# aleflabo/COSKAD

Measured on AMD Instinct MI355X. Metric: pose_clips_per_sec_fwd_bwd, higher is better.
Workload: dtype f32; 1 GPU; euclidean_encoder_dynamicCenter train step (fwd+mse-to-centre+L2 reg+bwd+Adam), synthetic clips B=4096/GPU T=12 V=17 C=2, channels 2-32-16-32-64, latent 16; clips_per_gpu=4096, global_batch=4096, head=euclidean, parallelism=dp1, hip_graph=False

## Files before the change

### coskad_amd/csrc/bottleneck.hip

```cpp
#include "tile_ops.h"
#include "layer_launch.h"

namespace coskad {

constexpr int kBtlBlock = 256;
constexpr int kBtlWaves = kBtlBlock / 64;
constexpr int kBtlFwdWaves = 8;

__global__ __launch_bounds__(64 * kBtlFwdWaves) void k_btlnk_fwd(const float* __restrict__ U,
                                                     const float* __restrict__ W,
                                                     const float* __restrict__ bias,
                                                     const float* __restrict__ slope,
                                                     float* __restrict__ z, int B, int K, int L) {
  __shared__ float red[kBtlFwdWaves][256];
  const int lane = threadIdx.x & 63, wave = threadIdx.x >> 6;
  const int i = lane & 15, kk = lane >> 4;
  const int n = blockIdx.x * 16 + i;
  const bool pre = slope != nullptr;
  const float a = pre ? slope[0] : 0.f;
  const bool rowok = n < B, colok = i < L;
  const float* up = U + (size_t)(rowok ? n : 0) * K;
  const float* wp = W + (size_t)(colok ? i : 0) * K;
  const int nsteps = ceil_div(K, 16);
  const int per = ceil_div(nsteps, kBtlFwdWaves);
  const int s0 = wave * per, s1 = min(nsteps, s0 + per);
  f32x4 acc = {0.f, 0.f, 0.f, 0.f};
  constexpr int UB = 4;
  for (int sb = s0; sb < s1; sb += UB) {
    float4 x[UB], w[UB];
#pragma unroll
    for (int u = 0; u < UB; ++u) {
      const int k = (sb + u) * 16 + 4 * kk;
      const bool ok = sb + u < s1 && k < K;
      x[u] = (ok && rowok) ? *reinterpret_cast<const float4*>(up + k) : float4{0.f, 0.f, 0.f, 0.f};
      w[u] = (ok && colok) ? *reinterpret_cast<const float4*>(wp + k) : float4{0.f, 0.f, 0.f, 0.f};
    }
#pragma unroll
    for (int u = 0; u < UB; ++u) {
      float4 xv = x[u];
      if (pre) { xv.x = prelu_f(xv.x, a); xv.y = prelu_f(xv.y, a); xv.z = prelu_f(xv.z, a); xv.w = prelu_f(xv.w, a); }
      acc = __builtin_amdgcn_mfma_f32_16x16x4f32(xv.x, w[u].x, acc, 0, 0, 0);
      acc = __builtin_amdgcn_mfma_f32_16x16x4f32(xv.y, w[u].y, acc, 0, 0, 0);
      acc = __builtin_amdgcn_mfma_f32_16x16x4f32(xv.z, w[u].z, acc, 0, 0, 0);
      acc = __builtin_amdgcn_mfma_f32_16x16x4f32(xv.w, w[u].w, acc, 0, 0, 0);
    }
  }
#pragma unroll
  for (int r = 0; r < 4; ++r) red[wave][(4 * (lane >> 4) + r) * 16 + (lane & 15)] = acc[r];
  __syncthreads();
  const int e = threadIdx.x, row = (e >> 4) & 15, col = e & 15;
  const int nn = blockIdx.x * 16 + row;
  if (e < 256 && nn < B && col < L) {
    float s = 0.f;
#pragma unroll
// ... 124 lines not shown
#pragma unroll
    for (int g = 0; g < 4; ++g) {
      const int nn = n0 + c, j = 4 * g + q;
      const float av = (nn < nend && j < L) ? dz[(size_t)nn * L + j] : 0.f;
      dx[0] = __builtin_amdgcn_mfma_f32_16x16x4f32(av, wf[g].x, dx[0], 0, 0, 0);
      dx[1] = __builtin_amdgcn_mfma_f32_16x16x4f32(av, wf[g].y, dx[1], 0, 0, 0);
      dx[2] = __builtin_amdgcn_mfma_f32_16x16x4f32(av, wf[g].z, dx[2], 0, 0, 0);
      dx[3] = __builtin_amdgcn_mfma_f32_16x16x4f32(av, wf[g].w, dx[3], 0, 0, 0);
    }
#pragma unroll
    for (int s = 0; s < 4; ++s) {
      const int nn = n0 + 4 * q + s;
      const bool ok = kok && nn < nend;
      const float4 u = ucur[s];
      float4 x = u;
      if (pre) { x.x = prelu_f(u.x, a); x.y = prelu_f(u.y, a); x.z = prelu_f(u.z, a); x.w = prelu_f(u.w, a); }
      const float dzv = (nn < nend && c < L) ? dz[(size_t)nn * L + c] : 0.f;
      dw[0] = __builtin_amdgcn_mfma_f32_16x16x4f32(dzv, x.x, dw[0], 0, 0, 0);
      dw[1] = __builtin_amdgcn_mfma_f32_16x16x4f32(dzv, x.y, dw[1], 0, 0, 0);
      dw[2] = __builtin_amdgcn_mfma_f32_16x16x4f32(dzv, x.z, dw[2], 0, 0, 0);
      dw[3] = __builtin_amdgcn_mfma_f32_16x16x4f32(dzv, x.w, dw[3], 0, 0, 0);
      float4 g = {dx[0][s], dx[1][s], dx[2][s], dx[3][s]};
      if (pre) {
        da += (u.x < 0.f ? g.x * u.x : 0.f) + (u.y < 0.f ? g.y * u.y : 0.f) +
              (u.z < 0.f ? g.z * u.z : 0.f) + (u.w < 0.f ? g.w * u.w : 0.f);
        g.x = u.x > 0.f ? g.x : a * g.x; g.y = u.y > 0.f ? g.y : a * g.y;
        g.z = u.z > 0.f ? g.z : a * g.z; g.w = u.w > 0.f ? g.w : a * g.w;
      }
      if (ok) *reinterpret_cast<float4*>(dU + (size_t)nn * K + kc) = g;
    }
#pragma unroll
    for (int s = 0; s < 4; ++s) ucur[s] = unext[s];
  }
  if (kok) {
    float* dst = dWp + (size_t)blockIdx.y * L * K;
#pragma unroll
    for (int r = 0; r < 4; ++r) {
      const int j = 4 * q + r;
      if (j < L) *reinterpret_cast<float4*>(dst + (size_t)j * K + kc) = float4{dw[0][r], dw[1][r], dw[2][r], dw[3][r]};
    }
  }
  da = wave_sum(da);
  if (lane == 0) sred[wave] = da;
  __syncthreads();
  if (threadIdx.x == 0) dap[blockIdx.y * gridDim.x + blockIdx.x] = (sred[0] + sred[1]) + (sred[2] + sred[3]);
}

__global__ __launch_bounds__(256) void k_btlnk_reduce(const float* __restrict__ partials, int P, size_t E,
                                                       float* __restrict__ out, const float* __restrict__ dz,
                                                       int B, int L, float* __restrict__ db,
                                                       const float* __restrict__ dap, int nda,
                                                       float* __restrict__ dslope, int accumulate,
                                                       const float* __restrict__ rows, int RP, int RE,
                                                       double* __restrict__ rsum) {
  __shared__ double sh[256];
  const unsigned nE = (unsigned)((E + 255) / 256);
  if (blockIdx.x > nE + L) {
    const int col = threadIdx.x & 15, slice = threadIdx.x >> 4;
    const int e = (int)(blockIdx.x - (nE + L + 1)) * 16 + col;
    double s = 0.0;
    if (e < RE) {
      const float* base = rows + e;
      int p = slice;
      for (; p + 7 * 16 < RP; p += 8 * 16) {
        float v[8];
#pragma unroll
        for (int u = 0; u < 8; ++u) v[u] = base[(size_t)(p + 16 * u) * RE];
#pragma unroll
        for (int u = 0; u < 8; ++u) s += (double)v[u];
      }
      for (; p < RP; p += 16) s += (double)base[(size_t)p * RE];
    }
    sh[threadIdx.x] = s;
    __syncthreads();
    if (slice == 0 && e < RE) {
      double t = 0.0;
#pragma unroll
      for (int k = 0; k < 16; ++k) t += sh[col + 16 * k];
      rsum[e] = t;
    }
    return;
  }
  if (blockIdx.x < nE) {
    const size_t e = (size_t)blockIdx.x * 256 + threadIdx.x;
    if (e >= E) return;
    double s = 0.0;
    int p = 0;
    for (; p + 8 <= P; p += 8) {
      float v[8];
#pragma unroll
      for (int u = 0; u < 8; ++u) v[u] = partials[(size_t)(p + u) * E + e];
#pragma unroll
      for (int u = 0; u < 8; ++u) s += (double)v[u];
    }
    for (; p < P; ++p) s += (double)partials[(size_t)p * E + e];
    out[e] = accumulate ? out[e] + (float)s : (float)s;
    return;
  }
  const int r = (int)(blockIdx.x - nE);
  double s = 0.0;
  if (r < L) {
    if (!db) return;
    for (int n = threadIdx.x; n < B; n += 256) s += (double)dz[(size_t)n * L + r];
  } else {
    if (!dslope) return;
    for (int i = threadIdx.x; i < nda; i += 256) s += (double)dap[i];
  }
  sh[threadIdx.x] = s;
  __syncthreads();
  for (int w = 128; w > 0; w >>= 1) {
    if ((int)threadIdx.x < w) sh[threadIdx.x] += sh[threadIdx.x + w];
    __syncthreads();
  }
  if (threadIdx.x == 0) {
    float* o = r < L ? db + r : dslope;
    o[0] = accumulate ? o[0] + (float)sh[0] : (float)sh[0];
  }
}

static int btl_chunks(int B, int K) {
  const int gx = ceil_div(K, 256);
  int s = (1024 + gx / 2) / gx;
  const int smax = ceil_div(B, 16);
  if (s > smax) s = smax;
  if (s > 64) s = 64;
  return s < 1 ? 1 : s;
}

int launch_btlnk_reduce(const float* partials, int P, size_t E, float* out, const float* dz, int B, int L, float* db,
                        const float* dap, int nda, float* dslope, int accumulate, hipStream_t stream, const float* rows,
                        int RP, int RE, double* rsum) {
  const unsigned extra = rows ? (unsigned)ceil_div(RE, 16) : 0u;
  hipLaunchKernelGGL(k_btlnk_reduce, dim3((unsigned)((E + 255) / 256) + L + 1 + extra), dim3(256), 0, stream, partials, P, E, out, dz,
                     B, L, db, dap, nda, dslope, accumulate, rows, RP, RE, rsum);
  return check_launch("btlnk_bwd_reduce");
}

constexpr int kBtlWideMax = 512;

}

using namespace coskad;

extern "C" {

int coskad_btlnk_fwd_f32(const float* U, const float* W, const float* bias, const float* slope, float* z,
                         int B, int K, int L, hipStream_t stream) {
  if (!U || !W || !z) return fail(COSKAD_ERR_ARG, "btlnk_fwd: null pointer");
  if (B <= 0 || K <= 0 || L <= 0) return fail(COSKAD_ERR_ARG, "btlnk_fwd: B=%d K=%d L=%d", B, K, L);
  if (L > 16) return fail(COSKAD_ERR_SHAPE, "btlnk_fwd: latent_dim=%d > 16 needs the workspace entry point coskad_btlnk_fwd_ws_f32", L);
  if (K % 4) return fail(COSKAD_ERR_SHAPE, "btlnk_fwd: K=%d must be a multiple of 4", K);
  hipLaunchKernelGGL(k_btlnk_fwd, dim3(ceil_div(B, 16)), dim3(64 * kBtlFwdWaves), 0, stream, U, W, bias, slope, z, B, K, L);
  return check_launch("btlnk_fwd");
}

size_t coskad_btlnk_fwd_ws_bytes(int B) { return (size_t)kBtlKS * (size_t)(B > 0 ? B : 0) * 16 * sizeof(float); }

size_t coskad_btlnk_fwd_ws_bytes_l(int B, int K, int L) {
  if (L > 16 && L <= kBtlWideMax) return wide_btlnk_fwd_ws_bytes(B, K, L);
  return coskad_btlnk_fwd_ws_bytes(B);
}

int coskad_btlnk_fwd_ws_f32(const float* U, const float* W, const float* bias, const float* slope, float* z, void* ws,
                            size_t ws_bytes, int B, int K, int L, hipStream_t stream) {
  if (!U || !W || !z || !ws) return fail(COSKAD_ERR_ARG, "btlnk_fwd_ws: null pointer");
  if (B <= 0 || K <= 0 || L <= 0) return fail(COSKAD_ERR_ARG, "btlnk_fwd_ws: B=%d K=%d L=%d", B, K, L);
  if (L > kBtlWideMax) return fail(COSKAD_ERR_SHAPE, "btlnk_fwd_ws: latent_dim=%d > %d not supported", L, kBtlWideMax);
  if (L > 16) {
    if (ws_bytes < wide_btlnk_fwd_ws_bytes(B, K, L)) return fail(COSKAD_ERR_WORKSPACE, "btlnk_fwd_ws: workspace too small");
    return wide_btlnk_fwd(U, W, bias, slope, z, ws, B, K, L, stream);
  }
  if (K % 16) return fail(COSKAD_ERR_SHAPE, "btlnk_fwd_ws: K=%d must be a multiple of 16", K);
  if (ws_bytes < coskad_btlnk_fwd_ws_bytes(B)) return fail(COSKAD_ERR_WORKSPACE, "btlnk_fwd_ws: workspace too small");
  float* part = reinterpret_cast<float*>(ws);
  hipLaunchKernelGGL(k_btlnk_fwd_t, dim3(ceil_div(B, 64), kBtlKS), dim3(256), 0, stream, U, W, slope, part, B, K, L);
  int rc;
  if ((rc = check_launch("btlnk_fwd_t"))) return rc;
  hipLaunchKernelGGL(k_btlnk_fwd_sum, dim3(ceil_div(B * 16, 256)), dim3(256), 0, stream, part, bias, z, B, L, kBtlKS);
  return check_launch("btlnk_fwd_sum");
}

size_t coskad_btlnk_bwd_ws_bytes(int B, int K, int L) {
  if (L > 16 && L <= kBtlWideMax) return wide_btlnk_bwd_ws_bytes(B, K, L);
  const int S = btl_chunks(B, K);
  return ((size_t)S * L * K + (size_t)S * ceil_div(K, 256) + 64) * sizeof(float);
}

int coskad_btlnk_bwd_f32(const float* U, const float* W, const float* dz, const float* slope, float* dU,
                         float* dW, float* db, float* dslope, void* ws, size_t ws_bytes, int accumulate,
                         int B, int K, int L, hipStream_t stream) {
  if (!U || !W || !dz || !dU || !dW || !ws) return fail(COSKAD_ERR_ARG, "btlnk_bwd: null pointer");
  if (B <= 0 || K <= 0 || L <= 0) return fail(COSKAD_ERR_ARG, "btlnk_bwd: B=%d K=%d L=%d", B, K, L);
  if (L > kBtlWideMax) return fail(COSKAD_ERR_SHAPE, "btlnk_bwd: latent_dim=%d > %d not supported", L, kBtlWideMax);
  if (ws_bytes < coskad_btlnk_bwd_ws_bytes(B, K, L)) return fail(COSKAD_ERR_WORKSPACE, "btlnk_bwd: workspace too small");
  if (L > 16) return wide_btlnk_bwd(U, W, dz, slope, dU, dW, db, dslope, ws, accumulate, B, K, L, stream);
  if (K % 4) return fail(COSKAD_ERR_SHAPE, "btlnk_bwd: K=%d must be a multiple of 4", K);
  const int S = btl_chunks(B, K);
  const int chunk = round_up(ceil_div(B, S), 16);
  const int gx = ceil_div(K, 256);
  float* dWp = reinterpret_cast<float*>(ws);
  float* dap = dWp + (size_t)S * L * K;
  {
    ProbeScope probe(KID_BTLNK_BWD, 0, L, stream);
    hipLaunchKernelGGL(k_btlnk_bwd, dim3(gx, S), dim3(kBtlBlock), 0, stream, U, W, dz, slope, dU, dWp, dap, B, K, L, chunk);
  }
  int rc = check_launch("btlnk_bwd");
  if (rc) return rc;
  return launch_btlnk_reduce(dWp, S, (size_t)L * K, dW, dz, B, L, db, dap, gx * S, (dslope && slope) ? dslope : nullptr, accumulate, stream,
                             nullptr, 0, 0, nullptr);
}

}
```

### coskad_amd/csrc/btlnk_chain.hip

```cpp
#include "fused_ops.h"
#include "layer_launch.h"

namespace coskad {
namespace bc {

using ff::f32x4; using ff::mfma; using ff::BufRes; using ff::make_res; using ff::buf_load4; using ff::buf_load1;
__device__ __forceinline__ void buf_store1(BufRes r, int voff, int soff, float v) {
  __builtin_amdgcn_raw_buffer_store_b32(__float_as_uint(v), r, voff, soff, 0);
}

constexpr int HID = 64;
constexpr int PT = 16;
constexpr int NCL = 16;
constexpr int RSTR = 17;
constexpr int kThreads = 512;
#ifndef BC_XCD
#define BC_XCD 1
#endif
#ifndef BC_PF
#define BC_PF 1
#endif
#ifndef BC_SKIP
#define BC_SKIP 0
#endif

template <int CT>
__global__ __launch_bounds__(kThreads, 1) void k_btlnk_bwd_stats(
    const float* __restrict__ U, const float* __restrict__ W, const float* __restrict__ dz, const float* __restrict__ slope,
    float* __restrict__ dU, float* __restrict__ dWp, float* __restrict__ dap, const float* __restrict__ xin,
    const float* __restrict__ Zg, const float* __restrict__ in_slope, float* __restrict__ prow, int B, int TV, int L, int chunk) {
  constexpr int Ci = 16 * CT, NR = 2 * Ci;
  constexpr int GCS = HID * RSTR + 4, ZCS = NR * RSTR + 4;
  constexpr int NL = NR * NCL * (PT / 4) / kThreads;
  constexpr int E = 2 * HID * Ci + HID;
  extern __shared__ __attribute__((aligned(16))) float lds[];
  float* G = lds;
  float* ZX = lds + NCL * GCS;
  const int tid = threadIdx.x, lane = tid & 63;
  const int wave = __builtin_amdgcn_readfirstlane(tid >> 6);
  const int wc = wave & 3, h = wave >> 2;
  const int c = lane & 15, q = lane >> 4;
  const int K = HID * TV;
  const int nwg = gridDim.x, npt = (TV + PT - 1) / PT;
  int wg = blockIdx.x;
  if (BC_XCD) {
    const int xq = nwg / 8, xr = nwg % 8, xcd = wg % 8;
    wg = (xcd < xr ? xcd * (xq + 1) : xr * (xq + 1) + (xcd - xr) * xq) + wg / 8;
  }
  const int ychunk = wg / npt;
  const int p0 = (wg - ychunk * npt) * PT;
  const int nbeg = ychunk * chunk, nend = min(B, nbeg + chunk);
  const bool pre = slope != nullptr;
  const float a = pre ? slope[0] : 0.f;
  const bool xact = in_slope != nullptr;
  const float a_in = xact ? in_slope[0] : 0.f;
  const int ch0 = 16 * wc + 8 * h;
  const bool pok = p0 + c < TV;
  constexpr int MASK = 0x7ffffff0;

  float wf[8][4];
#pragma unroll
  for (int i = 0; i < 8; ++i)
#pragma unroll
    for (int g = 0; g < 4; ++g) {
      const int j = 4 * g + q;
      wf[i][g] = (j < L && pok) ? W[(size_t)j * K + (ch0 + i) * TV + p0 + c] : 0.f;
    }

  f32x4 dw[8], pacc[CT], qacc[CT];
#pragma unroll
  for (int i = 0; i < 8; ++i) dw[i] = f32x4{0.f, 0.f, 0.f, 0.f};
#pragma unroll
  for (int t = 0; t < CT; ++t) pacc[t] = qacc[t] = f32x4{0.f, 0.f, 0.f, 0.f};
  float ssum = 0.f, da = 0.f;

  auto tile_res = [&](const float* base, int n0, int rowfloats) {
    const int left = nend - n0;
    return make_res(base + (size_t)(left > 0 ? n0 : 0) * rowfloats, left > 0 ? (unsigned)left * (unsigned)rowfloats * 4u : 0u);
  };
  const int zx_p4 = lane & 3, zx_row = lane >> 2;
  const int zx_voff = (p0 + 4 * zx_p4 < TV) ? (zx_row * TV + p0 + 4 * zx_p4) * 4 : MASK;
  auto zx_load = [&](int n0, float4 (&v)[NL]) {
    const BufRes rz = tile_res(Zg, n0, Ci * TV), rx = tile_res(xin, n0, Ci * TV);
#pragma unroll
    for (int i = 0; i < NL; ++i) {
      const int cl = wave + 8 * (i & 1), rb = i >> 1;
      v[i] = (BC_SKIP & 4) ? float4{0.f, 0.f, 0.f, 0.f} : buf_load4(rb < CT ? rz : rx, zx_voff, (cl * Ci + 16 * (rb % CT)) * TV * 4);
    }
  };
  auto zx_store = [&](const float4 (&v)[NL]) {
    if (BC_SKIP & 8) return;
#pragma unroll
    for (int i = 0; i < NL; ++i) {
      const int cl = wave + 8 * (i & 1), rb = i >> 1;
      float4 x = v[i];
      if (xact && rb >= CT) { x.x = prelu_f(x.x, a_in); x.y = prelu_f(x.y, a_in); x.z = prelu_f(x.z, a_in); x.w = prelu_f(x.w, a_in); }
      float* d = ZX + cl * ZCS + (16 * rb + zx_row) * RSTR + 4 * zx_p4;
      d[0] = x.x; d[1] = x.y; d[2] = x.z; d[3] = x.w;
    }
  };
  const int u_voff = pok ? (4 * q * K + p0 + c) * 4 : MASK;
  auto u_load = [&](int n0, float (&u)[8][4]) {
    const BufRes ru = tile_res(U, n0, K);
#pragma unroll
    for (int i = 0; i < 8; ++i)
#pragma unroll
      for (int r = 0; r < 4; ++r) u[i][r] = (BC_SKIP & 1) ? ((i + r) & 1 ? 1.f : -1.f) : buf_load1(ru, u_voff, (r * K + (ch0 + i) * TV) * 4);
  };
  const int dza_voff = (c * L + q) * 4, dzb_voff = (4 * q * L + c) * 4;
  auto dz_load = [&](int n0, float (&da_)[4], float (&db_)[4]) {
    const BufRes rd = tile_res(dz, n0, L);
#pragma unroll
    for (int g = 0; g < 4; ++g) {
      const float v = buf_load1(rd, dza_voff, 16 * g);
      da_[g] = 4 * g + q < L ? v : 0.f;
    }
#pragma unroll
    for (int r = 0; r < 4; ++r) {
      const float v = buf_load1(rd, dzb_voff, r * L * 4);
      db_[r] = c < L ? v : 0.f;
    }
  };

  float4 zx[NL];
  float ucur[8][4], dza[4], dzb[4];
  u_load(nbeg, ucur);
  dz_load(nbeg, dza, dzb);
  zx_load(nbeg, zx);

  float* gw = G + 4 * q * GCS + ch0 * RSTR + c;
  const float* ga = G + 4 * q * GCS + (16 * wc + c) * RSTR + 8 * h;
  const float* zb = ZX + 4 * q * ZCS + c * RSTR + 8 * h;

  for (int n0 = nbeg; n0 < nend; n0 += NCL) {
    float unext[8][4];
    if (BC_PF == 2) { zx_store(zx); zx_load(n0 + NCL, zx); }
    if (BC_PF) u_load(n0 + NCL, unext);
    {
      const BufRes rdu = tile_res(dU, n0, K);
      f32x4 dx[8];
#pragma unroll
      for (int i = 0; i < 8; ++i) dx[i] = f32x4{0.f, 0.f, 0.f, 0.f};
#pragma unroll
      for (int g = 0; g < 4; ++g)
#pragma unroll
        for (int i = 0; i < 8; ++i) dx[i] = mfma(dza[g], wf[i][g], dx[i]);
#pragma unroll
      for (int r = 0; r < 4; ++r)
#pragma unroll
        for (int i = 0; i < 8; ++i) {
          const float u = ucur[i][r];
          float g = dx[i][r], x = u;
          if (pre) {
            da += u < 0.f ? g * u : 0.f;
            g = u > 0.f ? g : a * g;
            x = prelu_f(u, a);
          }
          if (!(BC_SKIP & 32)) dw[i] = mfma(dzb[r], x, dw[i]);
          if (!(BC_SKIP & 64)) gw[r * GCS + i * RSTR] = g;
          if (!(BC_SKIP & 2) || g == 123.456f) buf_store1(rdu, u_voff, (r * K + (ch0 + i) * TV) * 4, g);
        }
    }
    if (BC_PF != 2) zx_store(zx);
    lds_barrier();
    if (BC_PF) {
#pragma unroll
      for (int i = 0; i < 8; ++i)
#pragma unroll
        for (int r = 0; r < 4; ++r) ucur[i][r] = unext[i][r];
    } else {
      u_load(n0 + NCL, ucur);
    }
    dz_load(n0 + NCL, dza, dzb);
    if (BC_PF != 2) zx_load(n0 + NCL, zx);
#pragma unroll
    for (int pl = 0; pl < 8; ++pl)
#pragma unroll
      for (int r = 0; r < 4; ++r) {
        const float av = (BC_SKIP & 64) ? 1.f : ga[r * GCS + pl];
        ssum += av;
        if (BC_SKIP & 16) continue;
#pragma unroll
        for (int t = 0; t < CT; ++t) {
          pacc[t] = mfma(av, zb[r * ZCS + (16 * t) * RSTR + pl], pacc[t]);
          qacc[t] = mfma(av, zb[r * ZCS + (Ci + 16 * t) * RSTR + pl], qacc[t]);
        }
      }
    lds_barrier();
  }

  {
    float* dst = dWp + (size_t)ychunk * L * K + p0 + c;
#pragma unroll
    for (int i = 0; i < 8; ++i)
#pragma unroll
      for (int r = 0; r < 4; ++r) {
        const int j = 4 * q + r;
        if (j < L && pok) dst[(size_t)j * K + (ch0 + i) * TV] = dw[i][r];
      }
  }
  float* row = lds;
  float* red = lds + E;
  const float s4 = ssum + __shfl_xor(ssum, 16, 64);
  const float sch = s4 + __shfl_xor(s4, 32, 64);
  da = wave_sum(da);
  for (int hh = 0; hh < 2; ++hh) {
    if (h == hh) {
#pragma unroll
      for (int t = 0; t < CT; ++t)
#pragma unroll
        for (int r = 0; r < 4; ++r) {
          const int o = 16 * wc + 4 * q + r, cc = 16 * t + c;
          float* p = row + o * Ci + cc;
          p[0] = (hh ? p[0] : 0.f) + pacc[t][r];
          p[HID * Ci] = (hh ? p[HID * Ci] : 0.f) + qacc[t][r];
        }
      if (q == 0) {
        float* p = row + 2 * HID * Ci + 16 * wc + c;
        p[0] = (hh ? p[0] : 0.f) + sch;
      }
      if (lane == 0) red[wave] = da;
    }
    __syncthreads();
  }
  float* dstrow = prow + (size_t)wg * E;
  for (int e = tid; e < E; e += kThreads) dstrow[e] = row[e];
  if (tid == 0) dap[wg] = ((red[0] + red[1]) + (red[2] + red[3])) + ((red[4] + red[5]) + (red[6] + red[7]));
}

struct Plan {
  int npt, S, chunk;
};
static Plan plan(int B, int TV) {
  Plan p;
  p.npt = ceil_div(TV, PT);
  int s = 256 / p.npt;
  const int smax = ceil_div(B, NCL);
  if (s > smax) s = smax;
  if (s < 1) s = 1;
  p.chunk = round_up(ceil_div(B, s), NCL);
  p.S = ceil_div(B, p.chunk);
  return p;
}
static inline size_t sums_offset(int rows, int E) { return ((size_t)rows * E + 1) / 2 * 2; }

}

}

using namespace coskad;

extern "C" {

int coskad_btlnk_bwd_chain_ok(int K, int TV, int below_Ci) {
  return TV > 0 && TV % 4 == 0 && K == bc::HID * TV && (below_Ci == 16 || below_Ci == 32);
}

int coskad_btlnk_bwd_chain_rows(int B, int TV) {
  if (B <= 0 || TV <= 0) return 0;
  const bc::Plan p = bc::plan(B, TV);
  return p.npt * p.S;
}

size_t coskad_btlnk_bwd_chain_floats(int B, int TV, int below_Ci) {
  const size_t E = 2 * (size_t)bc::HID * below_Ci + bc::HID;
  return bc::sums_offset(coskad_btlnk_bwd_chain_rows(B, TV), (int)E) + 2 * E;
}

size_t coskad_btlnk_bwd_chain_ws_bytes(int B, int K, int L, int TV) {
  if (B <= 0 || TV <= 0) return 0;
  const bc::Plan p = bc::plan(B, TV);
  return ((size_t)p.S * L * K + (size_t)p.S * p.npt + 64) * sizeof(float);
}

int coskad_btlnk_bwd_chain_f32(const float* U, const float* W, const float* dz, const float* slope, float* dU, float* dW,
                               float* db, float* dslope, void* ws, size_t ws_bytes, int accumulate, int B, int K, int L,
                               const float* below_in, const float* below_Z, const float* below_in_slope, int below_Ci, int TV,
                               float* stats_out, size_t stats_out_bytes, int* stats_rows, hipStream_t stream) {
  if (!U || !W || !dz || !dU || !dW || !ws || !below_in || !below_Z || !stats_out || !stats_rows)
    return fail(COSKAD_ERR_ARG, "btlnk_bwd_chain: null pointer");
  if (B <= 0 || K <= 0 || L <= 0) return fail(COSKAD_ERR_ARG, "btlnk_bwd_chain: B=%d K=%d L=%d", B, K, L);
  if (L > 16) return fail(COSKAD_ERR_SHAPE, "btlnk_bwd_chain: latent_dim=%d > 16 not supported", L);
  if (!coskad_btlnk_bwd_chain_ok(K, TV, below_Ci))
    return fail(COSKAD_ERR_SHAPE, "btlnk_bwd_chain: K=%d TV=%d below_Ci=%d (needs K = 64 TV, TV %% 4 == 0, 16 / 32 channels below)", K, TV, below_Ci);
  if ((size_t)stats_out & 7) return fail(COSKAD_ERR_ARG, "btlnk_bwd_chain: stats_out must be 8-byte aligned");
  if (ws_bytes < coskad_btlnk_bwd_chain_ws_bytes(B, K, L, TV)) return fail(COSKAD_ERR_WORKSPACE, "btlnk_bwd_chain: workspace too small");
  if (stats_out_bytes < coskad_btlnk_bwd_chain_floats(B, TV, below_Ci) * sizeof(float))
    return fail(COSKAD_ERR_WORKSPACE, "btlnk_bwd_chain: stats_out %zu bytes too small", stats_out_bytes);
  const bc::Plan p = bc::plan(B, TV);
  const int rows = p.npt * p.S;
  const int E = 2 * bc::HID * below_Ci + bc::HID;
  float* dWp = reinterpret_cast<float*>(ws);
  float* dap = dWp + (size_t)p.S * L * K;
  const size_t lds = (size_t)bc::NCL * ((bc::HID * bc::RSTR + 4) + (2 * below_Ci * bc::RSTR + 4)) * sizeof(float);
  int rc;
  {
  ProbeScope probe(KID_BTLNK_BWD, below_Ci, L, stream);
  if (below_Ci == 32) {
    auto k = bc::k_btlnk_bwd_stats<2>;
    (void)hipFuncSetAttribute((const void*)k, hipFuncAttributeMaxDynamicSharedMemorySize, (int)lds);
    hipLaunchKernelGGL(k, dim3(p.npt * p.S), dim3(bc::kThreads), lds, stream, U, W, dz, slope, dU, dWp, dap, below_in, below_Z,
                       below_in_slope, stats_out, B, TV, L, p.chunk);
  } else {
    auto k = bc::k_btlnk_bwd_stats<1>;
    (void)hipFuncSetAttribute((const void*)k, hipFuncAttributeMaxDynamicSharedMemorySize, (int)lds);
    hipLaunchKernelGGL(k, dim3(p.npt * p.S), dim3(bc::kThreads), lds, stream, U, W, dz, slope, dU, dWp, dap, below_in, below_Z,
                       below_in_slope, stats_out, B, TV, L, p.chunk);
  }
  }
  if ((rc = check_launch("btlnk_bwd_stats"))) return rc;
  *stats_rows = rows;
  return launch_btlnk_reduce(dWp, p.S, (size_t)L * K, dW, dz, B, L, db, dap, rows, (dslope && slope) ? dslope : nullptr, accumulate, stream,
                             stats_out, rows, E, reinterpret_cast<double*>(stats_out + bc::sums_offset(rows, E)));
}

}
```

### coskad_amd/csrc/first_layer.hip

```cpp
#include "mfma_ops.h"
#include "layer_launch.h"

namespace coskad {
namespace fl {

__device__ __forceinline__ float act(float x, bool pre, float a) { return (pre && x < 0.f) ? a * x : x; }
__device__ __forceinline__ float4 act4(float4 v, bool pre, float a) {
  return float4{act(v.x, pre, a), act(v.y, pre, a), act(v.z, pre, a), act(v.w, pre, a)};
}
__device__ __forceinline__ float dot4(const float4& a, const float4& b) { return (a.x * b.x + a.y * b.y) + (a.z * b.z + a.w * b.w); }

constexpr int NW = 4;
template <int CI, int RW>
__global__ __launch_bounds__(64 * NW, 4) void k_first_stats(const float* __restrict__ in, const float* __restrict__ Zg,
                                                           const float* __restrict__ dU, const float* __restrict__ in_slope,
                                                           float* __restrict__ partials, int B, int Co, int TVr, int need_q) {
  const int lane = threadIdx.x & 63;
  const int wave = uniform(threadIdx.x >> 6);
  const bool pre = in_slope != nullptr;
  const float a_in = pre ? in_slope[0] : 0.f;
  const int n4 = TVr >> 2;
  float pP[RW][CI], pQ[RW][CI], pS[RW];
#pragma unroll
  for (int k = 0; k < RW; ++k) {
    pS[k] = 0.f;
#pragma unroll
    for (int c = 0; c < CI; ++c) { pP[k][c] = 0.f; pQ[k][c] = 0.f; }
  }
  for (int clip = blockIdx.x; clip < B; clip += gridDim.x) {
    const float* gz = Zg + (size_t)clip * CI * TVr;
    const float* gx = in + (size_t)clip * CI * TVr;
    const float* gd = dU + ((size_t)clip * Co + (size_t)wave * RW) * TVr;
    for (int l = lane; l < n4; l += 64) {
      float4 z[CI], x[CI];
#pragma unroll
      for (int c = 0; c < CI; ++c) {
        z[c] = *reinterpret_cast<const float4*>(gz + c * TVr + 4 * l);
        x[c] = need_q ? act4(*reinterpret_cast<const float4*>(gx + c * TVr + 4 * l), pre, a_in) : float4{0.f, 0.f, 0.f, 0.f};
      }
      float4 d[RW];
#pragma unroll
      for (int k = 0; k < RW; ++k)
        d[k] = (wave * RW + k < Co) ? *reinterpret_cast<const float4*>(gd + (size_t)k * TVr + 4 * l) : float4{0.f, 0.f, 0.f, 0.f};
#pragma unroll
      for (int k = 0; k < RW; ++k) {
        pS[k] += (d[k].x + d[k].y) + (d[k].z + d[k].w);
#pragma unroll
        for (int c = 0; c < CI; ++c) {
          pP[k][c] += dot4(d[k], z[c]);
          pQ[k][c] += dot4(d[k], x[c]);
        }
      }
    }
  }
// ... 90 lines not shown
      }
#pragma unroll
      for (int c = 0; c < CI; ++c) *reinterpret_cast<float4*>(part + (wave * CI + c) * TV + 4 * l) = dz[c];
    }
    __syncthreads();
    for (int e = tid; e < CI * TV; e += NTH) {
      const int c = e / TV, p = e - c * TV;
      float v = kt[c];
#pragma unroll
      for (int c2 = 0; c2 < CI; ++c2) v = fmaf(Kt[c2 * CiP + c], Zg[((size_t)clip * CI + c2) * TV + p], v);
#pragma unroll
      for (int w = 0; w < NW; ++w) v += part[(w * CI + c) * TV + p];
      dZl[e] = v;
      Xl[e] = act(in[(size_t)clip * CI * TV + e], pre, a_in);
    }
    __syncthreads();
    for (int e = tid; e < CI * TV; e += NTH) {
      const int c = e / TV, p = e - c * TV, q = p / V, v = p - q * V;
      float y = 0.f, dy = 0.f;
#pragma unroll
      for (int t = 0; t < T; ++t) y = fmaf(Xl[c * TV + t * V + v], TwL[(t * T + q) * V + v], y);
#pragma unroll
      for (int w = 0; w < V; ++w) dy = fmaf(AwL[q * V * V + v * V + w], dZl[c * TV + q * V + w], dy);
      Yl[e] = y;
      dYl[e] = dy;
    }
    __syncthreads();
#pragma unroll
    for (int k = 0; k < KA; ++k) {
      float s = 0.f;
#pragma unroll
      for (int c = 0; c < CI; ++c) s = fmaf(Yl[c * TV + ya[k]], dZl[c * TV + za[k]], s);
      accA[k] += s;
    }
#pragma unroll
    for (int k = 0; k < KT; ++k) {
      float s = 0.f;
#pragma unroll
      for (int c = 0; c < CI; ++c) s = fmaf(Xl[c * TV + xt[k]], dYl[c * TV + yt[k]], s);
      accT[k] += s;
    }
  }
  float* dst = partials + (size_t)blockIdx.x * (NA + NT);
#pragma unroll
  for (int k = 0; k < KA; ++k)
    if (tid + NTH * k < NA) dst[tid + NTH * k] = accA[k];
#pragma unroll
  for (int k = 0; k < KT; ++k)
    if (tid + NTH * k < NT) dst[NA + tid + NTH * k] = accT[k];
}


constexpr int NWM = 8;
template <int T, int V, int CI>
__global__ __launch_bounds__(64 * NWM, 4) void k_first_moments(const float* __restrict__ in, const float* __restrict__ Aw,
                                                          const float* __restrict__ Tw, const float* __restrict__ in_slope,
                                                          float* __restrict__ partials, int B, float* __restrict__ Zout) {
  constexpr int TV = T * V, NA = T * V * V, NT = V * T * T, KP = (TV + 63) / 64;
  extern __shared__ __attribute__((aligned(16))) float lds[];
  float* AwL = lds;
  float* TwL = AwL + NA;
  const int tid = threadIdx.x, lane = tid & 63;
  const int wave = uniform(tid >> 6);
  float* Xl = TwL + NT + wave * 2 * CI * TV;
  float* Yl = Xl + CI * TV;
  const bool pre = in_slope != nullptr;
  const float a_in = pre ? in_slope[0] : 0.f;
  for (int e = tid; e < NA; e += 64 * NWM) AwL[e] = Aw[e];
  for (int e = tid; e < NT; e += 64 * NWM) {
    const int v = e / (T * T), tq = e - v * T * T;
    TwL[tq * V + v] = Tw[e];
  }
  float mx[CI][CI], mz[CI][CI], sx[CI], sz[CI];
#pragma unroll
  for (int a = 0; a < CI; ++a) {
    sx[a] = 0.f; sz[a] = 0.f;
#pragma unroll
    for (int b = 0; b < CI; ++b) { mx[a][b] = 0.f; mz[a][b] = 0.f; }
  }
  __syncthreads();
  const int rounds = (B + gridDim.x * NWM - 1) / (gridDim.x * NWM);
  for (int r = 0; r < rounds; ++r) {
    const int clip = (r * gridDim.x + blockIdx.x) * NWM + wave;
    const bool live = clip < B;
    const float* gx = in + (size_t)(live ? clip : 0) * CI * TV;
#pragma unroll
    for (int k = 0; k < KP; ++k) {
      const int p = lane + 64 * k;
      if (p < TV) {
        float x[CI];
#pragma unroll
        for (int c = 0; c < CI; ++c) {
          x[c] = live ? act(gx[c * TV + p], pre, a_in) : 0.f;
          Xl[c * TV + p] = x[c];
          sx[c] += x[c];
        }
#pragma unroll
        for (int a = 0; a < CI; ++a)
#pragma unroll
          for (int b = 0; b < CI; ++b) mx[a][b] = fmaf(x[a], x[b], mx[a][b]);
      }
    }
    __syncthreads();
#pragma unroll
    for (int k = 0; k < KP; ++k) {
      const int p = lane + 64 * k;
      if (p < TV) {
        const int q = p / V, v = p - q * V;
#pragma unroll
        for (int c = 0; c < CI; ++c) {
          float y = 0.f;
#pragma unroll
          for (int t = 0; t < T; ++t) y = fmaf(Xl[c * TV + t * V + v], TwL[(t * T + q) * V + v], y);
          Yl[c * TV + p] = y;
        }
      }
    }
    __syncthreads();
    float* gz = Zout + (size_t)(live ? clip : 0) * CI * TV;
#pragma unroll
    for (int k = 0; k < KP; ++k) {
      const int p = lane + 64 * k;
      if (p < TV) {
        const int t = p / V, w = p - t * V;
        float z[CI];
#pragma unroll
        for (int c = 0; c < CI; ++c) {
          float acc = 0.f;
#pragma unroll
          for (int v = 0; v < V; ++v) acc = fmaf(Yl[c * TV + t * V + v], AwL[t * V * V + v * V + w], acc);
          z[c] = acc;
          if (live) gz[c * TV + p] = acc;
          sz[c] += acc;
        }
#pragma unroll
        for (int a = 0; a < CI; ++a)
// ... 81 lines not shown
    else if (Ci == 2) LAUNCH_FS_C(2);
    else if (Ci == 3) LAUNCH_FS_C(3);
    else LAUNCH_FS_C(4);
  }
#undef LAUNCH_FS_C
#undef LAUNCH_FS
  return check_launch("first_stats");
}

template <int T, int V>
static int launch_first_bwd_tv(const float* in, const float* Zg, const float* dU, const float* Aw, const float* Tw, const float* coef,
                               const float* in_slope, float* partials, int B, int Ci, int Co, int max_rows, hipStream_t st,
                               int* rows_out) {
  constexpr int NWB = fl::first_bwd_waves<T, V>();
  int grid = B < 512 ? B : 512;
  if (grid > max_rows) grid = max_rows;
  *rows_out = grid;
  const int rw = ceil_div(Co, NWB);
  const size_t lds = ((size_t)T * V * V + (size_t)V * T * T + (4 + NWB) * (size_t)Ci * T * V) * sizeof(float);
#define LAUNCH_FB1(CI, RW)                                                                                              \
  do {                                                                                                                  \
    auto k = fl::k_first_bwd<T, V, CI, RW>;                                                                             \
    if (lds > 64 * 1024) (void)hipFuncSetAttribute((const void*)k, hipFuncAttributeMaxDynamicSharedMemorySize, (int)lds); \
    hipLaunchKernelGGL(k, dim3(grid), dim3(64 * NWB), lds, st, in, Zg, dU, Aw, Tw, coef, in_slope, partials, B, Co);             \
  } while (0)
#define LAUNCH_FB1_C(CI)                        \
  do {                                          \
    if (rw <= 4) LAUNCH_FB1(CI, 4);             \
    else if (rw <= 8) LAUNCH_FB1(CI, 8);        \
    else LAUNCH_FB1(CI, 16);                    \
  } while (0)
  {
    ProbeScope probe(KID_BWD_DATA, Ci, Co, st);
    if (Ci == 1) LAUNCH_FB1_C(1);
    else if (Ci == 2) LAUNCH_FB1_C(2);
    else if (Ci == 3) LAUNCH_FB1_C(3);
    else LAUNCH_FB1_C(4);
  }
#undef LAUNCH_FB1_C
#undef LAUNCH_FB1
  return check_launch("first_bwd");
}

int launch_first_bwd(const float* in, const float* Zg, const float* dU, const float* Aw, const float* Tw, const float* coef,
                     const float* in_slope, float* partials, int B, int Ci, int Co, int T, int V, int max_rows, hipStream_t st,
                     int* rows_out) {
#define CALL(T_, V_) return launch_first_bwd_tv<T_, V_>(in, Zg, dU, Aw, Tw, coef, in_slope, partials, B, Ci, Co, max_rows, st, rows_out)
  COSKAD_DISPATCH_TV(T, V, CALL);
#undef CALL
}

template <int T, int V>
static int launch_first_moments_tv(const float* in, const float* Aw, const float* Tw, const float* in_slope, float* partials, int B,
                                   int Ci, float* Zout, int max_rows, hipStream_t st, int* rows_out) {
  int grid = (B + fl::NWM - 1) / fl::NWM;
  if (grid > 512) grid = 512;
  if (grid > max_rows) grid = max_rows;
  *rows_out = grid;
  const size_t lds = ((size_t)T * V * V + (size_t)V * T * T + 2 * fl::NWM * (size_t)Ci * T * V) * sizeof(float);
#define LAUNCH_FM(CI)                                                                                                   \
  do {                                                                                                                  \
    auto k = fl::k_first_moments<T, V, CI>;                                                                             \
    if (lds > 64 * 1024) (void)hipFuncSetAttribute((const void*)k, hipFuncAttributeMaxDynamicSharedMemorySize, (int)lds); \
    hipLaunchKernelGGL(k, dim3(grid), dim3(64 * fl::NWM), lds, st, in, Aw, Tw, in_slope, partials, B, Zout);                    \
  } while (0)
  {
    ProbeScope probe(KID_FWD_MOMENTS, Ci, 0, st);
    if (Ci == 1) LAUNCH_FM(1);
    else if (Ci == 2) LAUNCH_FM(2);
    else if (Ci == 3) LAUNCH_FM(3);
    else LAUNCH_FM(4);
  }
#undef LAUNCH_FM
  return check_launch("first_moments");
}

int launch_first_moments(const float* in, const float* Aw, const float* Tw, const float* in_slope, float* partials, int B, int Ci,
                         int T, int V, float* Zout, int max_rows, hipStream_t st, int* rows_out) {
#define CALL(T_, V_) return launch_first_moments_tv<T_, V_>(in, Aw, Tw, in_slope, partials, B, Ci, Zout, max_rows, st, rows_out)
  COSKAD_DISPATCH_TV(T, V, CALL);
#undef CALL
}

int launch_first_apply(const float* Z, const float* in, float* out, const float* wfold, const float* bias, const float* in_slope,
                       int B, int Ci, int Co, int TVr, hipStream_t st) {
  const int grid = B < 2048 ? B : 2048;
  const size_t lds = 2 * (size_t)Ci * TVr * sizeof(float);
  const int CoP = round_up(Co, 16);
#define LAUNCH_FAP(CI) hipLaunchKernelGGL((fl::k_first_apply<CI>), dim3(grid), dim3(256), lds, st, Z, in, out, wfold, bias, in_slope, B, Co, CoP, TVr)
  {
    ProbeScope probe(KID_LAYER_APPLY, Ci, Co, st);
    if (Ci == 1) LAUNCH_FAP(1);
    else if (Ci == 2) LAUNCH_FAP(2);
    else if (Ci == 3) LAUNCH_FAP(3);
    else LAUNCH_FAP(4);
  }
#undef LAUNCH_FAP
  return check_launch("first_apply");
}

}
```

### coskad_amd/csrc/fused_apply_next.hip

```cpp
#include "fused_ops.h"
#include "layer_launch.h"

#ifndef FN_ABLATE
#define FN_ABLATE 0
#endif

namespace coskad {
namespace fn {

using namespace ff;

struct FtabArgs {
  const float* A[4];
  const float* Tm[4];
  float* tab[4];
};
__global__ void k_build_ftab(FtabArgs args) {
  const int layer = blockIdx.y;
  const float* __restrict__ Aw = args.A[layer];
  const float* __restrict__ Tw = args.Tm[layer];
  const int e = blockIdx.x * blockDim.x + threadIdx.x;
  if (e >= LAYER_F4 * 4) return;
  float val = 0.f;
  if (e < TEMP_F4 * 4) {
    const int v = e / 256, l = (e >> 2) & 63, s = e & 3, j = l & 15, q = l >> 4;
    if (s < 3 && j < T) val = Tw[v * T * T + (4 * s + q) * T + j];
  } else {
    const int r = e - TEMP_F4 * 4;
    const int t = r / (3 * 256), c = (r / 256) % 3, l = (r >> 2) & 63, k = 4 * c + (r & 3), j = l & 15, q = l >> 4;
    if (k < 10) {
      const int s = k < 5 ? k : k - 5, w = 4 * s + q;
      if (w < V) val = Aw[t * V * V + w * V + (k < 5 ? j : 16)];
    }
  }
  args.tab[layer][e] = val;
}

template <int CT, int OTP>
__global__ __launch_bounds__(256, 1) void k_layer_apply_next(const float* __restrict__ in, const float* __restrict__ Zg,
                                                            const float* __restrict__ wfold, const float* __restrict__ bias,
                                                            const float* __restrict__ in_slope, const float* __restrict__ out_slope,
                                                            const float* __restrict__ ftab, float* __restrict__ out,
                                                            float* __restrict__ Znext, float* __restrict__ partials, int B) {
  constexpr int Ci = CT ? 16 * CT : 2, Co = 16 * OTP, CoP = Co, NG = 2 * CT;
  constexpr int NACC = OTP == 1 ? 2 : 3;
  constexpr int E = 2 * (Co * Co + Co);
  static_assert(OTP == 1 || OTP == 2, "the 32-row image holds the whole output");
  extern __shared__ __attribute__((aligned(16))) float lds_all[];
  const int lane = threadIdx.x & 63;
  const int wave = __builtin_amdgcn_readfirstlane(threadIdx.x >> 6);
  float* lds = lds_all + wave * WAVE_LDS_W;
  float* r1 = lds + R1;
  float* r2 = lds + R2;
  auto geo = [&]() {
    int l = lane;
    asm volatile("" : "+v"(l));
    return Lane{l & 15, l >> 4};
  };
  auto olane = [&]() {
    int l = lane;
    asm volatile("" : "+v"(l));
    return l;
  };
  const bool pre = in_slope != nullptr;
  const float a_in = pre ? in_slope[0] : 0.f;
  const float a_out = out_slope[0];
  const int l16 = lane * 16;
  const BufRes wres = make_res(wfold, 2 * Ci * CoP * 4u);
  const BufRes bres = make_res(bias, CoP * 4u);
  const BufRes tabres = make_res(ftab, LAYER_F4 * 16u);
  const int nwaves = gridDim.x * 4;
  auto clip_res = [&](const float* base, int c, int rows) {
    const bool in_range = c < B;
#ifdef COSKAD_HOT
    return make_res(base + (size_t)(in_range ? (c & 63) : 0) * rows * TV, in_range ? rows * TV * 4u : 0u);
#else
    return make_res(base + (size_t)(in_range ? c : 0) * rows * TV, in_range ? rows * TV * 4u : 0u);
#endif
  };
  constexpr int QTAIL = 4 * (TV / 4) - 192;
  const int l16t = lane < QTAIL ? l16 : 0x7ffffff0;
  float4 gb[16];
  auto qload = [&](const BufRes& res, int row0, int q) {
#pragma unroll
    for (int c = 0; c < 4; ++c) gb[4 * q + c] = buf_load4(res, c < 3 ? l16 : l16t, ((row0 + 4 * q) * (TV / 4) + 64 * c) * 16);
  };
  auto qstore = [&](int q, bool act) {
    const int ln = olane();
// ... 202 lines not shown
  }

  float* row = lds_all;
  __syncthreads();
  const Lane L = geo();
  auto put = [&](int w, float* base, const f32x4 (&g)[NACC], const float (&s)[OTP]) {
#pragma unroll
    for (int r = 0; r < 4; ++r) {
      const int i = 4 * L.q + r, j = L.j;
      if constexpr (OTP == 1) {
        float* p = base + i * Co + j;
        p[0] = (w ? p[0] : 0.f) + (g[0][r] + g[1][r]);
      } else {
        float* p00 = base + i * Co + j;
        float* p01 = base + i * Co + 16 + j;
        float* p10 = base + (16 + j) * Co + i;
        float* p11 = base + (16 + i) * Co + 16 + j;
        p00[0] = (w ? p00[0] : 0.f) + g[0][r];
        p01[0] = (w ? p01[0] : 0.f) + g[1][r];
        p10[0] = (w ? p10[0] : 0.f) + g[1][r];
        p11[0] = (w ? p11[0] : 0.f) + g[2][r];
      }
    }
#pragma unroll
    for (int rt = 0; rt < OTP; ++rt) {
      const float t = quad_sum(s[rt]);
      if (L.q == 0) {
        float* p = base + Co * Co + 16 * rt + L.j;
        p[0] = (w ? p[0] : 0.f) + t;
      }
    }
  };
  for (int w = 0; w < 4; ++w) {
    if (wave == w) {
      put(w, row, gx, sx);
      put(w, row + Co * Co + Co, gz, sz);
    }
    __syncthreads();
  }
  float* dst = partials + (size_t)blockIdx.x * E;
  for (int e = threadIdx.x; e < E; e += 256) dst[e] = row[e];
}

}

bool layer_apply_next_ok(int T_, int V_, int Ci, int Co) {
  return T_ == ff::T && V_ == ff::V && (Ci == 2 || Ci == 16 || Ci == 32) && (Co == 16 || Co == 32);
}

int ftab_floats() { return ff::LAYER_F4 * 4; }

int launch_build_ftab(const float* const* A, const float* const* Tm, float* const* tab, int n, hipStream_t st) {
  if (n < 1 || n > 4) return fail(COSKAD_ERR_ARG, "build_ftab: 1..4 layers per launch, got %d", n);
  fn::FtabArgs args{};
  for (int i = 0; i < n; ++i) {
    if (!A[i] || !Tm[i] || !tab[i]) return fail(COSKAD_ERR_ARG, "build_ftab: null pointer (layer %d)", i);
    args.A[i] = A[i]; args.Tm[i] = Tm[i]; args.tab[i] = tab[i];
  }
  hipLaunchKernelGGL(fn::k_build_ftab, dim3(ceil_div(ff::LAYER_F4 * 4, 256), n), dim3(256), 0, st, args);
  return check_launch("build_ftab");
}

static bool apply_next_bpc_on(int Ci, int Co) { return (Ci == 2 && Co == 32) || (Ci == 32 && Co == 16) || (Ci == 16 && Co == 32); }
int layer_apply_next_rows(int B, int Ci, int Co) {
  if (apply_next_bpc_on(Ci, Co)) return apply_next_bpc_rows(B);
  const int nblk = (B + 3) / 4;
  return nblk < 256 ? nblk : 256;
}

int launch_layer_apply_next(const float* Z, const float* in, float* out, const float* wfold, const float* bias,
                            const float* in_slope, const float* out_slope, const float* ftab, float* Znext, float* partials,
                            int B, int Ci, int Co, hipStream_t st, int* rows_out) {
  const size_t lds = (size_t)4 * ff::WAVE_LDS_W * sizeof(float);
  const int grid = layer_apply_next_rows(B, Ci, Co);
  *rows_out = grid;
  if (apply_next_bpc_on(Ci, Co))
    return launch_layer_apply_next_bpc(Z, in, out, wfold, bias, in_slope, out_slope, ftab, Znext, partials, B, Ci, Co, st);
#define LAUNCH_FN(CT, OTP)                                                                                            \
  do {                                                                                                                \
    auto k = fn::k_layer_apply_next<CT, OTP>;                                                                         \
    (void)hipFuncSetAttribute((const void*)k, hipFuncAttributeMaxDynamicSharedMemorySize, (int)lds);                  \
    hipLaunchKernelGGL(k, dim3(grid), dim3(256), lds, st, in, Z, wfold, bias, in_slope, out_slope, ftab, out, Znext,  \
                       partials, B);                                                                                  \
  } while (0)
  {
    ProbeScope probe(KID_LAYER_APPLY, Ci, Co, st);
    if (Ci == 2 && Co == 16) LAUNCH_FN(0, 1);
    else if (Ci == 2 && Co == 32) LAUNCH_FN(0, 2);
    else if (Ci == 16 && Co == 16) LAUNCH_FN(1, 1);
    else if (Ci == 16 && Co == 32) LAUNCH_FN(1, 2);
    else if (Ci == 32 && Co == 16) LAUNCH_FN(2, 1);
    else if (Ci == 32 && Co == 32) LAUNCH_FN(2, 2);
    else return fail(COSKAD_ERR_SHAPE, "apply_next: unsupported channels (%d, %d)", Ci, Co);
  }
#undef LAUNCH_FN
  return check_launch("layer_apply_next");
}

}

using namespace coskad;
extern "C" {

int coskad_layer_apply_next_ok(int Ci, int Co, int T, int V) { return layer_apply_next_ok(T, V, Ci, Co) ? 1 : 0; }
int coskad_ftab_floats(void) { return ftab_floats(); }
int coskad_layer_apply_next_rows(int B, int Ci, int Co) { return layer_apply_next_rows(B, Ci, Co); }

// ... 24 lines not shown
```

### coskad_amd/csrc/heads.hip

```cpp
#include "tile_ops.h"
#include "heads_common.h"

namespace coskad {

struct Vec {
  float v[LMAX];
};

__device__ __forceinline__ Vec load_vec(const float* p, int L) {
  Vec r;
#pragma unroll
  for (int j = 0; j < LMAX; ++j) r.v[j] = j < L ? p[j] : 0.f;
  return r;
}
__device__ __forceinline__ void store_vec(float* p, const Vec& a, int L) {
#pragma unroll
  for (int j = 0; j < LMAX; ++j)
    if (j < L) p[j] = a.v[j];
}
__device__ __forceinline__ float dot(const Vec& a, const Vec& b) {
  float s = 0.f;
#pragma unroll
  for (int j = 0; j < LMAX; ++j) s = fmaf(a.v[j], b.v[j], s);
  return s;
}

struct Embed {
  Vec p;
  float un_raw, un, tn, en_raw;
  bool clamped;
};
__device__ __forceinline__ Embed hyp_embed(const Vec& u) {
  Embed r;
  r.un_raw = sqrtf(dot(u, u));
  r.un = fmaxf(r.un_raw, kMinNorm);
  r.tn = tanhf(fminf(fmaxf(r.un, -kTanhClamp), kTanhClamp));
  const float f = r.tn / r.un;
  Vec e;
#pragma unroll
  for (int j = 0; j < LMAX; ++j) e.v[j] = f * u.v[j];
  r.en_raw = sqrtf(dot(e, e));
  const float en = fmaxf(r.en_raw, kMinNorm);
  const float maxnorm = 1.f - kBallEps;
  r.clamped = en > maxnorm;
  const float s = r.clamped ? maxnorm / en : 1.f;
#pragma unroll
  for (int j = 0; j < LMAX; ++j) r.p.v[j] = r.clamped ? e.v[j] / en * maxnorm : e.v[j];
  (void)s;
  return r;
}

__device__ __forceinline__ float poincare_dist(const Vec& c, const Vec& p, Vec* gp) {
  const float x2 = dot(c, c), y2 = dot(p, p), xy = -dot(c, p);
  const float alpha = 1.f + 2.f * xy + y2, beta = 1.f - x2;
  const float den = 1.f + 2.f * xy + x2 * y2;
  const float D = den + kMobiusEps;
  Vec m;
#pragma unroll
  for (int j = 0; j < LMAX; ++j) m.v[j] = (alpha * (-c.v[j]) + beta * p.v[j]) / D;
  const float mn = sqrtf(dot(m, m));
  const float mc = fminf(fmaxf(mn, -1.f + kArtanhEps), 1.f - kArtanhEps);
  const float d = (log1pf(mc) - log1pf(-mc));
  if (gp) {
    const float gmn = 2.f / (1.f - mc * mc);
    const float inv = mn > 0.f ? gmn / mn : 0.f;
    Vec gm;
#pragma unroll
    for (int j = 0; j < LMAX; ++j) gm.v[j] = inv * m.v[j];
    const float gD = -dot(gm, m) / D;
    float galpha = 0.f;
#pragma unroll
    for (int j = 0; j < LMAX; ++j) galpha = fmaf(gm.v[j] / D, -c.v[j], galpha);
#pragma unroll
    for (int j = 0; j < LMAX; ++j) {
      const float x = -c.v[j], y = p.v[j];
      gp->v[j] = beta * gm.v[j] / D + galpha * (2.f * x + 2.f * y) + gD * (2.f * x + 2.f * x2 * y);
    }
  }
  return d;
}

__device__ __forceinline__ Vec hyp_embed_bwd(const Vec& u, const Embed& em, const Vec& gp) {
  const float f = em.tn / em.un;
  Vec ge;
  if (em.clamped) {
    const float maxnorm = 1.f - kBallEps;
    const float en = em.en_raw;
    float egp = 0.f;
#pragma unroll
    for (int j = 0; j < LMAX; ++j) egp = fmaf(f * u.v[j], gp.v[j], egp);
#pragma unroll
    for (int j = 0; j < LMAX; ++j) ge.v[j] = maxnorm * (gp.v[j] / en - f * u.v[j] * egp / (en * en * en));
  } else {
    ge = gp;
  }
  Vec gu;
  float gf = dot(ge, u);
  float coef = 0.f;
  if (em.un_raw > kMinNorm) {
    const float sech2 = em.un < kTanhClamp ? 1.f - em.tn * em.tn : 0.f;
    const float df = (sech2 * em.un - em.tn) / (em.un * em.un);
    coef = gf * df / em.un_raw;
  }
#pragma unroll
  for (int j = 0; j < LMAX; ++j) gu.v[j] = f * ge.v[j] + coef * u.v[j];
  return gu;
}

constexpr int kHeadSlots = LMAX + 3;

constexpr int kHeadSingleRows = kFlatBlock;
__host__ __device__ inline int head_blocks(int B) { return B <= kHeadSingleRows ? 1 : ceil_div(B, kFlatBlock); }

__device__ __forceinline__ void block_partials(const float (&vals)[kHeadSlots], float* partials, float scale0, float* stats,
                                               float* acc) {
  __shared__ float sh[kFlatBlock / 64][kHeadSlots];
  const int lane = threadIdx.x & 63, wave = threadIdx.x >> 6;
#pragma unroll
  for (int k = 0; k < kHeadSlots; ++k) {
    const float s = wave_sum(vals[k]);
    if (lane == 0) sh[wave][k] = s;
  }
  __syncthreads();
  if (threadIdx.x < kHeadSlots) {
    float s = 0.f;
    for (int w = 0; w < kFlatBlock / 64; ++w) s += sh[w][threadIdx.x];
    if (gridDim.x == 1) {
      if (stats) stats[threadIdx.x] = threadIdx.x == 0 ? s * scale0 : s;
      if (acc) acc[threadIdx.x] += s;
    } else {
      partials[blockIdx.x * kHeadSlots + threadIdx.x] = s;
    }
  }
}

__global__ __launch_bounds__(kFlatBlock) void k_mse_head(const float* __restrict__ z,
                                                    const float* __restrict__ cvec,
                                                    float* __restrict__ dz, float* __restrict__ score,
                                                    float* __restrict__ partials, int B, int L,
                                                    float gscale, float scale0, float* __restrict__ stats,
                                                    float* __restrict__ acc) {
  float vals[kHeadSlots];
#pragma unroll
  for (int k = 0; k < kHeadSlots; ++k) vals[k] = 0.f;
  const Vec c = load_vec(cvec, L);
#pragma unroll 4
  for (int n = blockIdx.x * kFlatBlock + threadIdx.x; n < B; n += gridDim.x * kFlatBlock) {
    const Vec u = load_vec(z + (size_t)n * L, L);
    Vec g;
    float sq = 0.f;
#pragma unroll
    for (int j = 0; j < LMAX; ++j) {
      const float d = j < L ? u.v[j] - c.v[j] : 0.f;
      sq = fmaf(d, d, sq);
      g.v[j] = 2.f * d * gscale;
      vals[1 + j] += u.v[j];
    }
    vals[0] += sq;
    vals[LMAX + 1] += 1.f;
    vals[LMAX + 2] += sqrtf(dot(u, u));
    if (dz) store_vec(dz + (size_t)n * L, g, L);
    if (score) score[n] = sq / (float)L;
  }
  block_partials(vals, partials, scale0, stats, acc);
}

__global__ __launch_bounds__(kFlatBlock) void k_mahalanobis_head(const float* __restrict__ z,
                                                            const float* __restrict__ cvec,
                                                            const float* __restrict__ VI,
                                                            float* __restrict__ dz, float* __restrict__ score,
                                                            float* __restrict__ partials, int B, int L,
                                                            float gscale, float scale0, float* __restrict__ stats,
                                                            float* __restrict__ acc) {
  __shared__ float vi[LMAX * LMAX];
  for (int e = threadIdx.x; e < LMAX * LMAX; e += kFlatBlock) {
    const int r = e / LMAX, q = e - r * LMAX;
    vi[e] = (r < L && q < L) ? VI[r * L + q] : 0.f;
  }
  __syncthreads();
  float vals[kHeadSlots];
#pragma unroll
  for (int k = 0; k < kHeadSlots; ++k) vals[k] = 0.f;
  const Vec c = load_vec(cvec, L);
  for (int n = blockIdx.x * kFlatBlock + threadIdx.x; n < B; n += gridDim.x * kFlatBlock) {
    const Vec u = load_vec(z + (size_t)n * L, L);
    Vec d, w, wt;
#pragma unroll
    for (int j = 0; j < LMAX; ++j) { d.v[j] = j < L ? u.v[j] - c.v[j] : 0.f; w.v[j] = 0.f; wt.v[j] = 0.f; }
#pragma unroll
    for (int r = 0; r < LMAX; ++r)
#pragma unroll
      for (int q = 0; q < LMAX; ++q) {
        const float a = vi[r * LMAX + q];
        w.v[r] = fmaf(a, d.v[q], w.v[r]);
        wt.v[q] = fmaf(a, d.v[r], wt.v[q]);
      }
    const float dist = sqrtf(dot(d, w));
    vals[0] += dist;
#pragma unroll
    for (int j = 0; j < LMAX; ++j) vals[1 + j] += u.v[j];
    vals[LMAX + 1] += 1.f;
    vals[LMAX + 2] += sqrtf(dot(u, u));
    if (score) score[n] = dist;
    if (dz) {
      Vec g;
      const float inv = gscale / (2.f * dist);
#pragma unroll
      for (int j = 0; j < LMAX; ++j) g.v[j] = (w.v[j] + wt.v[j]) * inv;
      store_vec(dz + (size_t)n * L, g, L);
    }
  }
  block_partials(vals, partials, scale0, stats, acc);
}

__global__ __launch_bounds__(LMAX * LMAX) void k_gram(const float* __restrict__ z, float* __restrict__ gram, int B,
                                                     int L, int accumulate) {
  constexpr int CH = 256;
  __shared__ float zs[CH * LMAX];
  const int i = threadIdx.x / LMAX, j = threadIdx.x % LMAX;
  float s = 0.f;
  for (int n0 = 0; n0 < B; n0 += CH) {
    const int nc = min(CH, B - n0);
    __syncthreads();
    for (int e = threadIdx.x; e < nc * L; e += LMAX * LMAX) {
      const int r = e / L, q = e - r * L;
      zs[r * LMAX + q] = z[(size_t)(n0 + r) * L + q];
    }
    __syncthreads();
    if (i < L && j < L)
      for (int r = 0; r < nc; ++r) s = fmaf(zs[r * LMAX + i], zs[r * LMAX + j], s);
  }
  if (i < L && j < L) gram[i * L + j] = accumulate ? gram[i * L + j] + s : s;
}

__global__ __launch_bounds__(kFlatBlock) void k_poincare_head(const float* __restrict__ z,
                                                         const float* __restrict__ cvec,
                                                         float* __restrict__ dz, float* __restrict__ zh,
                                                         float* __restrict__ score,
                                                         float* __restrict__ partials, int B, int L,
                                                         float gscale, float scale0, float* __restrict__ stats,
                                                         float* __restrict__ acc) {
  float vals[kHeadSlots];
#pragma unroll
  for (int k = 0; k < kHeadSlots; ++k) vals[k] = 0.f;
  for (int n = blockIdx.x * kFlatBlock + threadIdx.x; n < B; n += gridDim.x * kFlatBlock) {
    const Vec u = load_vec(z + (size_t)n * L, L);
    const Embed em = hyp_embed(u);
    if (zh) store_vec(zh + (size_t)n * L, em.p, L);
    const float y2 = dot(em.p, em.p);
    const float gamma = 2.f / (1.f - y2);
#pragma unroll
    for (int j = 0; j < LMAX; ++j) vals[1 + j] += gamma * em.p.v[j];
    vals[LMAX + 1] += gamma - 1.f;
    vals[LMAX + 2] += sqrtf(y2);
    if (cvec) {
      const Vec c = load_vec(cvec, L);
      Vec gp;
      const float d = poincare_dist(c, em.p, dz ? &gp : nullptr);
      vals[0] += d;
      if (score) score[n] = d;
      if (dz) {
#pragma unroll
        for (int j = 0; j < LMAX; ++j) gp.v[j] *= gscale;
        store_vec(dz + (size_t)n * L, hyp_embed_bwd(u, em, gp), L);
      }
    }
  }
  block_partials(vals, partials, scale0, stats, acc);
}

__global__ __launch_bounds__(64) void k_head_finalize(const float* __restrict__ partials, int P,
                                                       float scale0, float* __restrict__ stats,
                                                       float* __restrict__ acc) {
  const int k = threadIdx.x;
  if (k >= kHeadSlots) return;
  double s = 0.0;
  for (int p = 0; p < P; ++p) s += (double)partials[p * kHeadSlots + k];
  if (stats) stats[k] = (float)(k == 0 ? s * (double)scale0 : s);
  if (acc) acc[k] += (float)s;
}

__global__ __launch_bounds__(kFlatBlock) void k_poincare_dist(const float* __restrict__ zh,
                                                         const float* __restrict__ cvec,
                                                         float* __restrict__ score, int B, int L) {
  const int n = blockIdx.x * kFlatBlock + threadIdx.x;
  if (n >= B) return;
  const Vec p = load_vec(zh + (size_t)n * L, L), c = load_vec(cvec, L);
  score[n] = poincare_dist(c, p, nullptr);
}

__global__ __launch_bounds__(kFlatBlock) void k_poincare_logmap0(const float* __restrict__ y, float* __restrict__ out, int B, int L) {
  const int n = blockIdx.x * kFlatBlock + threadIdx.x;
  if (n >= B) return;
  const Vec p = load_vec(y + (size_t)n * L, L);
  const float yn = fmaxf(sqrtf(dot(p, p)), kMinNorm);
  const float yc = fminf(fmaxf(yn, -1.f + kArtanhEps), 1.f - kArtanhEps);
  const float at = 0.5f * (log1pf(yc) - log1pf(-yc));
  Vec o;
#pragma unroll
  for (int j = 0; j < LMAX; ++j) o.v[j] = p.v[j] / yn * at;
  store_vec(out + (size_t)n * L, o, L);
}

__global__ void k_midpoint_finalize(const float* __restrict__ acc, float* __restrict__ cvec, int L) {
  if (threadIdx.x != 0 || blockIdx.x != 0) return;
  const double s = fmax((double)acc[LMAX + 1], 1e-10);
  double m[LMAX], mn2 = 0.0;
  for (int j = 0; j < L; ++j) { m[j] = (double)acc[1 + j] / s; mn2 += m[j] * m[j]; }
  const double mn = fmax(sqrt(mn2), 1e-15);
  const double mc = fmin(mn, 1.0 - 1e-7);
  const double at = 0.5 * log((1.0 + mc) / (1.0 - mc));
  const double sc = tanh(0.5 * at) / mn;
  for (int j = 0; j < L; ++j) cvec[j] = (float)(sc * m[j]);
}

__global__ void k_center_finalize(const float* __restrict__ acc, float eps, float* __restrict__ cvec,
                                  int L) {
  const int j = threadIdx.x;
  if (j >= L || blockIdx.x != 0) return;
  float c = acc[1 + j] / acc[LMAX + 1];
  if (fabsf(c) < eps && c < 0.f) c = -eps;
  if (fabsf(c) < eps && c > 0.f) c = eps;
  cvec[j] = c;
}

__global__ __launch_bounds__(256) void k_sqnorm_masked(const float* __restrict__ p,
                                                        const float* __restrict__ mask, size_t n,
                                                        float* __restrict__ partials) {
  __shared__ float sh[4];
  float s = 0.f;
  for (size_t i = (size_t)blockIdx.x * 256 + threadIdx.x; i < n; i += (size_t)gridDim.x * 256) {
    const float v = p[i];
// ... 191 lines not shown
```

### coskad_amd/csrc/heads_common.h

```cpp
#pragma once
#include "common.h"

namespace coskad {

constexpr int LMAX = 16;
constexpr int kWideLMax = 512;
constexpr float kMinNorm = 1e-5f;
constexpr float kBallEps = 1e-3f;
constexpr float kArtanhEps = 1e-5f;
constexpr float kMobiusEps = 1e-5f;
constexpr float kTanhClamp = 15.f;

__host__ __device__ inline int head_lp(int L) { return L > LMAX ? L : LMAX; }
__host__ __device__ inline int head_slots_for(int L) { return head_lp(L) + 3; }

size_t wide_head_ws_floats(int B, int L);
int wide_mse_head(const float* z, const float* c, float* dz, float* score, float* stats, float* acc, float upstream, float* ws,
                  int B, int L, hipStream_t stream);
int wide_mahalanobis_head(const float* z, const float* c, const float* VI, float* dz, float* score, float* stats, float* acc,
                          float* gram, int gram_accumulate, float upstream, float* ws, int B, int L, hipStream_t stream);
int wide_poincare_head(const float* z, const float* c, float* dz, float* zh, float* score, float* stats, float* acc,
                       float upstream, float* ws, int B, int L, hipStream_t stream);
int wide_poincare_dist(const float* zh, const float* c, float* score, int B, int L, hipStream_t stream);
int wide_poincare_logmap0(const float* y, float* out, int B, int L, hipStream_t stream);
int wide_center_finalize(const float* acc, float* c, float eps, int L, hipStream_t stream);
int wide_midpoint_finalize(const float* acc, float* c, int L, hipStream_t stream);

}
```

### coskad_amd/csrc/layer_launch.h

```cpp
#pragma once
#include "common.h"
#include <cstdlib>
#include <type_traits>

extern "C" int coskad_window_ok(int T, int V);
extern "C" int coskad_layer_train_window_ok(int T, int V, int Ci, int Co);
extern "C" int coskad_layer_train_window_narrow_ok(int T, int V, int Ci, int Co);

namespace coskad {

#ifdef COSKAD_ABLATE
inline int ablate_env(const char* name, int dflt) {
  const char* e = getenv(name);
  return e ? atoi(e) : dflt;
}
#else
constexpr int ablate_env(const char*, int dflt) { return dflt; }
#endif

template <class F>
inline void with_tiles(int n, F&& f) {
  if (n == 1) f(std::integral_constant<int, 1>{});
  else if (n == 2) f(std::integral_constant<int, 2>{});
  else if (n == 3) f(std::integral_constant<int, 3>{});
// ... 26 lines not shown
  float* stats = nullptr;
};
struct StatsOnly {
  float* out = nullptr;
  int* rows_out = nullptr;
};
struct LayerBwdArgs {
  const float* in = nullptr;
  const float* dU = nullptr;
  const float* A = nullptr;
  const float* Tm = nullptr;
  const float* in_slope = nullptr;
  const float* stat = nullptr;
  const float* Wt = nullptr;
  const float* gt = nullptr;
  const float* Wr = nullptr;
  const float* gr = nullptr;
  const float* Z = nullptr;
  LayerGrads g;
  void* ws = nullptr;
  size_t ws_bytes = 0;
  int accumulate = 0;
  int B = 0, Ci = 0, Co = 0;
  hipStream_t stream = nullptr;
  ChainIn chain;
  double stats_count = 0.0;
  Below below;
  StatsOnly stats_only;
  float* dz_ext = nullptr;
};

struct BnConvParams {
  const float* Wt = nullptr;
  const float* bt = nullptr;
  const float* gt = nullptr;
  const float* bet = nullptr;
  float* rm_t = nullptr;
  float* rv_t = nullptr;
  long long* nbt_t = nullptr;
  const float* Wr = nullptr;
  const float* br = nullptr;
  const float* gr = nullptr;
  const float* ber = nullptr;
  float* rm_r = nullptr;
  float* rv_r = nullptr;
  long long* nbt_r = nullptr;
  float momentum = 0.f;
};
struct FoldOut {
  float* wfold = nullptr;
  float* bias = nullptr;
  float* stat = nullptr;
};
struct LayerStatsArgs {
  const float* in = nullptr;
  const float* A = nullptr;
  const float* Tm = nullptr;
  const float* in_slope = nullptr;
  const float* partials = nullptr;
  int rows = 0;
  BnConvParams p;
  FoldOut out;
  float* Zout = nullptr;
  double* sums = nullptr;
  void* ws = nullptr;
  size_t ws_bytes = 0;
  int B = 0, Ci = 0, Co = 0;
  hipStream_t stream = nullptr;
};

void launch_reduce_partials(const float* partials, int rows, int E, double* out, hipStream_t st);

int launch_window_gcn(const float* in, float* out, const float* Aw, const float* Tw, int rows, int T, int V, int adjoint,
                      hipStream_t st);
int launch_window_params(const float* x, const float* dZ, const float* Aw, const float* Tw, float* dA, float* dT, void* ws,
                         int accumulate, int rows, int T, int V, hipStream_t st, float* dX, const float* add,
                         const float* in_slope = nullptr, float* dap = nullptr, int* rows_out = nullptr);
size_t window_params_ws_bytes(int T, int V);

bool window_moments_ok(int T, int V, int Ci);
int launch_window_moments(const float* in, const float* Aw, const float* Tw, const float* in_slope, float* partials, int B, int Ci,
                          int T, int V, int need_x, float* Zout, hipStream_t st, int* rows_out);
bool window_flat_ok(int TV, int Ci, int Co);
int launch_window_apply(const float* Z, const float* in, float* out, const float* wfold, const float* bias, const float* in_slope,
                        int B, int Ci, int Co, int TV, hipStream_t st);
int launch_window_stats(const float* in, const float* Zg, const float* dU, const float* in_slope, float* partials, int B, int Ci, int Co,
                        int TV, int need_q, hipStream_t st, int* rows_out);
int launch_window_data(const float* in, const float* Z, const float* dU, const float* coef, const float* in_slope, float* dZ, float* dXr,
                       int B, int Ci, int Co, int TV, hipStream_t st);

int layer_bwd_below_rows(int T_, int V_, int B, int Ci, int Co, int below_Ci);
int launch_layer_bwd_bpc(const float* in, const float* Zg, const float* dU, const float* coef, const float* in_slope, float* dIn,
                         float* btab, float* partials, float* dap, int B, int Ci, int Co, hipStream_t st, int* rows_out,
                         const float* below_z, const float* below_x, const float* below_slope, int below_Ci, float* below_stats);
bool layer_bwd_fused_ok(int T_, int V_, int Ci, int Co);
int launch_reduce_fused(const float* partials, int rows, float* dA, float* dT, const float* dap, float* dslope, int accumulate,
                        hipStream_t st, const float* brows, int bE, double* bout);
bool bwd_stats_ring_ok(int T_, int V_, int Ci, int Co);
int launch_bwd_stats_ring(const float* in, const float* Zg, const float* dU, const float* in_slope, float* partials, int B,
                          int Ci, int Co, hipStream_t st, int* rows_out);
bool bwd_stats_bpc_ok(int T_, int V_, int Ci, int Co);
bool bwd_stats_flat_ok(int TV_, int Ci, int Co);
int launch_bwd_stats_flat(const float* in, const float* Zg, const float* dU, const float* in_slope, float* partials, int B,
                          int Ci, int Co, int TV_, hipStream_t st, int* rows_out);
int launch_bwd_stats_bpc(const float* in, const float* Zg, const float* dU, const float* in_slope, float* partials, int B,
                         int Ci, int Co, hipStream_t st, int* rows_out);
bool bwd_data_bpc_ok(int T_, int V_, int Ci, int Co);
int launch_bwd_data_bpc(const float* in, const float* Zg, const float* dU, const float* Aw, const float* Tw, const float* coef,
                        const float* in_slope, float* dIn, float* dZout, float* dap, int B, int Ci, int Co, int T_, int V_,
                        hipStream_t st, int* rows_out, float* gpart);
bool gcn_params_bpc_ok(int T_, int V_);
int launch_gcn_params_bpc(const float* in, const float* in_slope, const float* dz, const float* Aw, const float* Tw, float* partials,
                          int rows_total, int T_, int V_, hipStream_t st, int* rows_out);
bool first_layer_ok(int T_, int V_, int Ci, int Co);
int launch_first_stats(const float* in, const float* Zg, const float* dU, const float* in_slope, float* partials, int B, int Ci,
                       int Co, int TVr, int need_q, int max_rows, hipStream_t st, int* rows_out);
int launch_first_bwd(const float* in, const float* Zg, const float* dU, const float* Aw, const float* Tw, const float* coef,
                     const float* in_slope, float* partials, int B, int Ci, int Co, int T, int V, int max_rows, hipStream_t st,
                     int* rows_out);
int launch_first_moments(const float* in, const float* Aw, const float* Tw, const float* in_slope, float* partials, int B, int Ci,
                         int T, int V, float* Zout, int max_rows, hipStream_t st, int* rows_out);
int launch_first_apply(const float* Z, const float* in, float* out, const float* wfold, const float* bias, const float* in_slope,
                       int B, int Ci, int Co, int TVr, hipStream_t st);
bool fwd_moments_bpc_ok(int T_, int V_, int Ci);
int launch_fwd_moments_bpc(const float* in, const float* Aw, const float* Tw, const float* in_slope, float* partials, int B, int Ci,
                           int T_, int V_, int need_x, float* Zout, hipStream_t st, int* rows_out);
int launch_combine_moments_bpc(const float* Zy, const float* YR, const float* stat, float* U, const float* Aw, const float* Tw,
                               const float* slope, float* partials, int B, int T_, int V_, float* Zout, hipStream_t st, int* rows_out);
template <int T, int V>
int launch_layer_apply_m(const float* in, float* out, const float* Aw, const float* Tw, const float* wfold,
                         const float* bias, const float* in_slope, const float* out_slope, int B, int Ci,
                         int Co, hipStream_t st, const float* Zg);
bool eval_layer_clip_ok(int T_, int V_, int Ci, int Co);
int launch_eval_layer_clip(const float* in, float* out, const float* Aw, const float* Tw, const float* wfold, const float* bias,
                           const float* in_slope, const float* out_slope, int B, int Ci, int Co, int T_, int V_, hipStream_t st);
bool eval_first_pair_clip_ok(int T_, int V_, int Ci, int Cm, int Co);
int launch_eval_first_pair_clip(const float* x, float* out, const float* A1, const float* T1, const float* wfold1,
                                const float* bias1, const float* A2, const float* T2, const float* wfold2, const float* bias2,
                                const float* mid_slope, const float* out_slope, int B, int Co, int T_, int V_, hipStream_t st);
bool layer_apply_ring_ok(int T_, int V_, int Ci, int Co);
int launch_layer_apply_ring(const float* Z, const float* in, float* out, const float* wfold, const float* bias,
                            const float* in_slope, int B, int Ci, int Co, hipStream_t st);
int launch_layer_apply_bpc(const float* Z, const float* in, float* out, const float* wfold, const float* bias,
                           const float* in_slope, int B, int Ci, int Co, hipStream_t st);
bool layer_apply_flat_ok(int TV_, int Ci, int Co);
int launch_layer_apply_flat(const float* Z, const float* in, float* out, const float* wfold, const float* bias,
                            const float* in_slope, int B, int Ci, int Co, int TV_, hipStream_t st);
int launch_commute_apply_mix(const float* in, float* out, const float* wt, const float* wr, const float* in_slope, const float* Aw,
                             const float* Tw, float* zy, float* mixpart, int B, int Ci, int Jo, int TV_, hipStream_t st, int* rows_out);
int apply_next_bpc_rows(int B);
int launch_layer_apply_next_bpc(const float* Z, const float* in, float* out, const float* wfold, const float* bias,
                                const float* in_slope, const float* out_slope, const float* ftab, float* Znext, float* partials,
                                int B, int Ci, int Co, hipStream_t st);
int launch_btlnk_reduce(const float* partials, int P, size_t E, float* out, const float* dz, int B, int L, float* db,
                        const float* dap, int nda, float* dslope, int accumulate, hipStream_t stream, const float* rows,
                        int RP, int RE, double* rsum);
size_t wide_btlnk_fwd_ws_bytes(int B, int K, int L);
size_t wide_btlnk_bwd_ws_bytes(int B, int K, int L);
int wide_btlnk_fwd(const float* U, const float* W, const float* bias, const float* slope, float* z, void* ws, int B, int K, int L,
                   hipStream_t stream);
int wide_btlnk_bwd(const float* U, const float* W, const float* dz, const float* slope, float* dU, float* dW, float* db,
                   float* dslope, void* ws, int accumulate, int B, int K, int L, hipStream_t stream);
bool wide_rev_btlnk_ok(int N, int L);
size_t wide_rev_btlnk_ws_floats(int B, int N, int L);
int wide_rev_btlnk_fwd(const float* z, const float* W, const float* bias, float* H, int B, int N, int L, hipStream_t stream);
int wide_rev_btlnk_bwd(const float* dH, const float* z, const float* W, float* dz, int dz_accumulate, float* dW, float* db, int accumulate,
                       float* ws, int B, int N, int L, hipStream_t stream);

}
```

### coskad_amd/csrc/stsgcn_train.hip

```cpp
#include "mfma_ops.h"
#include "layer_launch.h"

namespace coskad {

constexpr int kMaxGrid = 768;

template <int T, int V, int NTC>
__global__ __launch_bounds__((Geo<T, V>::Block), (Geo<T, V>::Block <= 512 && NTC <= 2 ? 6 : 4)) void k_fwd_moments(const float* __restrict__ in,
                                                       const float* __restrict__ Aw,
                                                       const float* __restrict__ Tw,
                                                       const float* __restrict__ in_slope,
                                                       float* __restrict__ partials, int B, int Ci,
                                                       int NB, int need_x, float* __restrict__ Zout) {
  constexpr int kScratchFloats = Geo<T, V>::Scratch;
  constexpr int TV = Geo<T, V>::TV, LD = TV + 2;
  extern __shared__ __attribute__((aligned(16))) float lds[];
  float* scratch = lds;
  float* AwL = lds + max(NB * Ci * LD, kScratchFloats);
  float* TwL = AwL + T * V * V;
  copy_to_lds(AwL, Aw, T * V * V);
  copy_to_lds(TwL, Tw, V * T * T);
  const bool pre = in_slope != nullptr;
  const float a_in = pre ? in_slope[0] : 0.f;
  f32x4 mx[NTC][NTC], mz[NTC][NTC];
  float sx[NTC], sz[NTC];
  zero_acc(mx); zero_acc(mz);
#pragma unroll
  for (int t = 0; t < NTC; ++t) { sx[t] = 0.f; sz[t] = 0.f; }

  const int ntiles = ceil_div(B, NB);
  for (int tile = blockIdx.x; tile < ntiles; tile += gridDim.x) {
    const int clip0 = tile * NB;
    const int nb = min(NB, B - clip0);
    const int rows = nb * Ci;
    lds_barrier();
    stage_rows<T, V, LD>(in + (size_t)clip0 * Ci * TV, lds, rows * TV, pre, a_in);
    lds_barrier();
    if (need_x) {
      for (int n = 0; n < nb; ++n) moment_accum<T, V, NTC, LD>(lds + n * Ci * LD, Ci, mx, sx);
      lds_barrier();
    }
    gcn_mfma<T, V, false, LD>(lds, rows, AwL, TwL);
    lds_barrier();
    if (Zout) unstage_rows<T, V, LD>(Zout + (size_t)clip0 * Ci * TV, lds, rows * TV);
    for (int n = 0; n < nb; ++n) moment_accum<T, V, NTC, LD>(lds + n * Ci * LD, Ci, mz, sz);
  }
  float* dst = partials + (size_t)blockIdx.x * (2 * (Ci * Ci + Ci));
  store_moments<NTC>(mx, sx, scratch, dst, Ci, dst + Ci * Ci, Ci);
  store_moments<NTC>(mz, sz, scratch, dst + Ci * Ci + Ci, Ci, dst + 2 * Ci * Ci + Ci, Ci);
}

constexpr int kRedCols = 16;
__global__ __launch_bounds__(1024) void k_reduce_partials(const float* __restrict__ partials, int P, int E,
                                                           double* __restrict__ out) {
// ... 188 lines not shown

size_t train_stats_ws_bytes(int Ci) {
  const size_t E = 2 * ((size_t)Ci * Ci + Ci);
  return kMaxGrid * E * sizeof(float) + round_up((int)(E * sizeof(double)), 256) + 256;
}

void launch_reduce_partials(const float* partials, int rows, int E, double* out, hipStream_t st) {
  hipLaunchKernelGGL(k_reduce_partials, dim3(ceil_div(E, kRedCols)), dim3(1024), 0, st, partials, rows, E, out);
}

static int launch_reduce_fold(const float* partials, int rows, double* red, double npos, const BnConvParams& p, const FoldOut& o,
                              int Ci, int Co, hipStream_t st) {
  const int E = 2 * (Ci * Ci + Ci);
  int rc = 0;
  const bool self_sum = partials && p.Wt && E <= kFoldSelfSum;
  if (partials && !self_sum) {
    launch_reduce_partials(partials, rows, E, red, st);
    if ((rc = check_launch("reduce_partials"))) return rc;
  }
  if (!p.Wt) return 0;
  const size_t fold_lds = (2 * (size_t)Ci * Ci + 2 * Ci) * sizeof(double) + (4 * (size_t)Co * Ci + 4 * Co) * sizeof(float);
  if (fold_lds > 64 * 1024) (void)hipFuncSetAttribute((const void*)k_train_fold, hipFuncAttributeMaxDynamicSharedMemorySize, (int)fold_lds);
  const int fold_blocks = Co >= 32 ? 8 : (Co >= 16 ? 4 : 1);
  hipLaunchKernelGGL(k_train_fold, dim3(fold_blocks), dim3(1024), fold_lds, st, red, npos, p.Wt, p.bt, p.gt, p.bet, p.rm_t,
                     p.rv_t, p.nbt_t, p.Wr, p.br, p.gr, p.ber, p.rm_r, p.rv_r, p.nbt_r, p.momentum, o.wfold, o.bias, o.stat, Ci,
                     Co, round_up(Co, 16), self_sum ? partials : (const float*)nullptr, rows);
  return check_launch("train_fold");
}

template <int T, int V>
static int launch_train_stats(const LayerStatsArgs& a) {
  constexpr int kBlock = Geo<T, V>::Block;
  constexpr int kScratchFloats = Geo<T, V>::Scratch;
  constexpr int TV = Geo<T, V>::TV, LD = TV + 2;
  static_assert(TV % 4 == 0, "the moments kernel stages with float4 and needs TV + 2 == 2 (mod 4)");
  const int B = a.B, Ci = a.Ci, Co = a.Co;
  hipStream_t st = a.stream;
  if (Ci > 64) return fail(COSKAD_ERR_SHAPE, "train_stats: C_in=%d > 64 not supported", Ci);
  if (a.ws_bytes < train_stats_ws_bytes(Ci))
    return fail(COSKAD_ERR_WORKSPACE, "train_stats: workspace %zu < %zu bytes", a.ws_bytes, train_stats_ws_bytes(Ci));
  const int E = 2 * (Ci * Ci + Ci);
  int NB = Ci >= 32 ? 1 : 32 / Ci;
  if (NB > B) NB = B;
  const size_t img = (size_t)NB * Ci * LD > (size_t)kScratchFloats ? (size_t)NB * Ci * LD : (size_t)kScratchFloats;
  const size_t lds = (img + (size_t)T * V * V + (size_t)V * T * T) * sizeof(float);
  if (lds > (size_t)kMaxLdsBytes) return fail(COSKAD_ERR_SHAPE, "train_stats: LDS %zu too large", lds);
  const int ntiles = ceil_div(B, NB);
  const int per_cu = lds <= (size_t)52 * 1024 && Ci <= 32 && kBlock <= 512 ? 3 : (lds <= (size_t)80 * 1024 ? 2 : 1);
  const int grid = ntiles < 256 * per_cu ? ntiles : 256 * per_cu;
  float* partials = reinterpret_cast<float*>(a.ws);
  double* red = reinterpret_cast<double*>(reinterpret_cast<char*>(a.ws) + round_up((int)(kMaxGrid * (size_t)E * sizeof(float)), 256));
  const int need_x = a.sums ? 1 : (a.p.Wr != nullptr);
  int rows = grid;
  if (a.Zout && Ci <= 4 && TV % 4 == 0) {
    int rc1 = launch_first_moments(a.in, a.A, a.Tm, a.in_slope, partials, B, Ci, T, V, a.Zout, kMaxGrid, st, &rows);
    if (rc1) return rc1;
  } else if (a.Zout && fwd_moments_bpc_ok(T, V, Ci)) {
    ProbeScope probe(KID_FWD_MOMENTS, Ci, Co, st);
    int rc1 = launch_fwd_moments_bpc(a.in, a.A, a.Tm, a.in_slope, partials, B, Ci, T, V, need_x, a.Zout, st, &rows);
    if (rc1) return rc1;
  } else {
    ProbeScope probe(KID_FWD_MOMENTS, Ci, Co, st);
    with_tiles(ceil_div(Ci, 16), [&](auto NTC) {
      auto k = k_fwd_moments<T, V, decltype(NTC)::value>;
      if (lds > 64 * 1024) (void)hipFuncSetAttribute((const void*)k, hipFuncAttributeMaxDynamicSharedMemorySize, (int)lds);
      hipLaunchKernelGGL(k, dim3(grid), dim3(kBlock), lds, st, a.in, a.A, a.Tm, a.in_slope, partials, B, Ci, NB, need_x, a.Zout);
    });
  }
  int rc = check_launch("fwd_moments");
  if (rc) return rc;
  if (a.sums) return launch_reduce_fold(partials, rows, a.sums, 0.0, BnConvParams{}, FoldOut{}, Ci, Co, st);
  return launch_reduce_fold(partials, rows, red, (double)B * TV, a.p, a.out, Ci, Co, st);
}

enum : unsigned {
  kNeedInput = 1,
  kNeedPartials = 2,
  kNeedSums = 4,
  kNeedFold = 8,
  kNeedWs = 16,
};
static int check_layer_stats(const char* who, const LayerStatsArgs& a, unsigned need) {
  bool null = false;
  if (need & kNeedInput) null = null || !a.in || !a.A || !a.Tm;
  if (need & kNeedPartials) null = null || !a.partials;
  if (need & kNeedSums) null = null || !a.sums;
  if (need & kNeedFold) null = null || !a.p.Wt || !a.p.gt || !a.p.bet || !a.out.wfold || !a.out.bias || !a.out.stat;
  if (need & kNeedWs) null = null || !a.ws;
  if (null) return fail(COSKAD_ERR_ARG, "%s: null pointer", who);
  if (need & kNeedFold) {
    if (a.p.Wr && (!a.p.gr || !a.p.ber)) return fail(COSKAD_ERR_ARG, "%s: residual BN missing", who);
    if (!a.p.Wr && a.Ci != a.Co) return fail(COSKAD_ERR_ARG, "%s: identity residual needs Ci == Co", who);
  }
  return COSKAD_OK;
}

static int launch_train_stats_window(const LayerStatsArgs& a, int T, int V) {
  const int B = a.B, Ci = a.Ci, Co = a.Co;
  if (a.ws_bytes < train_stats_ws_bytes(Ci))
    return fail(COSKAD_ERR_WORKSPACE, "train_stats: workspace %zu < %zu bytes", a.ws_bytes, train_stats_ws_bytes(Ci));
  const int E = 2 * (Ci * Ci + Ci);
  float* partials = reinterpret_cast<float*>(a.ws);
  double* red = reinterpret_cast<double*>(reinterpret_cast<char*>(a.ws) + round_up((int)(kMaxGrid * (size_t)E * sizeof(float)), 256));
  const int need_x = a.sums ? 1 : (a.p.Wr != nullptr);
  int rows = 0;
  if (int rc = launch_window_moments(a.in, a.A, a.Tm, a.in_slope, partials, B, Ci, T, V, need_x, a.Zout, a.stream, &rows)) return rc;
  if (a.sums) return launch_reduce_fold(partials, rows, a.sums, 0.0, BnConvParams{}, FoldOut{}, Ci, Co, a.stream);
  return launch_reduce_fold(partials, rows, red, (double)B * T * V, a.p, a.out, Ci, Co, a.stream);
}

static int dispatch_train_stats(const char* who, const LayerStatsArgs& a, int T, int V, bool full) {
  if (coskad_window_ok(T, V)) {
    if ((size_t)a.in & 15) return fail(COSKAD_ERR_ARG, "%s: `in` must be 16-byte aligned at window lengths 8, 16 and 24", who);
    if ((size_t)a.Zout & 15) return fail(COSKAD_ERR_ARG, "%s: `Z` must be 16-byte aligned at window lengths 8, 16 and 24", who);
    if (full ? (coskad_layer_train_window_ok(T, V, a.Ci, a.Co) || coskad_layer_train_window_narrow_ok(T, V, a.Ci, a.Co))
             : window_moments_ok(T, V, a.Ci))
      return launch_train_stats_window(a, T, V);
  }
#define CALL(T_, V_) return launch_train_stats<T_, V_>(a)
  COSKAD_DISPATCH_TV(T, V, CALL);
#undef CALL
}

}

using namespace coskad;

extern "C" {

size_t coskad_train_stats_ws_bytes(int Ci) { return train_stats_ws_bytes(Ci); }
int coskad_stat_floats(int Ci, int Co) { return stat_floats(Ci, Co); }

int coskad_layer_train_stats_z_f32(const float* in, const float* A, const float* Tm, const float* in_slope,
                                 const float* Wt, const float* bt, const float* gamma_t,
                                 const float* beta_t, float* rmean_t, float* rvar_t, long long* nbt_t,
                                 const float* Wr, const float* br, const float* gamma_r,
                                 const float* beta_r, float* rmean_r, float* rvar_r, long long* nbt_r,
                                 float momentum, float* wfold, float* bias, float* stat, void* ws,
                                 size_t ws_bytes, int B, int Ci, int Co, int T, int V,
                                 hipStream_t stream, float* Z) {
  const LayerStatsArgs a{
      .in = in, .A = A, .Tm = Tm, .in_slope = in_slope,
      .p = {.Wt = Wt, .bt = bt, .gt = gamma_t, .bet = beta_t, .rm_t = rmean_t, .rv_t = rvar_t, .nbt_t = nbt_t, .Wr = Wr, .br = br,
            .gr = gamma_r, .ber = beta_r, .rm_r = rmean_r, .rv_r = rvar_r, .nbt_r = nbt_r, .momentum = momentum},
      .out = {.wfold = wfold, .bias = bias, .stat = stat},
      .Zout = Z, .ws = ws, .ws_bytes = ws_bytes, .B = B, .Ci = Ci, .Co = Co, .stream = stream};
  if (int rc = check_layer_stats("layer_train_stats", a, kNeedInput | kNeedFold | kNeedWs)) return rc;
  if (B <= 0 || Ci <= 0 || Co <= 0) return fail(COSKAD_ERR_ARG, "layer_train_stats: B=%d Ci=%d Co=%d", B, Ci, Co);
  return dispatch_train_stats("layer_train_stats", a, T, V, true);
}

int coskad_layer_train_stats_f32(const float* in, const float* A, const float* Tm, const float* in_slope,
                                 const float* Wt, const float* bt, const float* gamma_t,
                                 const float* beta_t, float* rmean_t, float* rvar_t, long long* nbt_t,
                                 const float* Wr, const float* br, const float* gamma_r,
                                 const float* beta_r, float* rmean_r, float* rvar_r, long long* nbt_r,
                                 float momentum, float* wfold, float* bias, float* stat, void* ws,
                                 size_t ws_bytes, int B, int Ci, int Co, int T, int V,
                                 hipStream_t stream) {
  return coskad_layer_train_stats_z_f32(in, A, Tm, in_slope, Wt, bt, gamma_t, beta_t, rmean_t, rvar_t, nbt_t, Wr, br, gamma_r, beta_r,
                                        rmean_r, rvar_r, nbt_r, momentum, wfold, bias, stat, ws, ws_bytes, B, Ci, Co, T, V, stream,
                                        nullptr);
}

int coskad_layer_train_fold_f32(const float* partials, int rows, const float* Wt, const float* bt, const float* gamma_t,
                                const float* beta_t, float* rmean_t, float* rvar_t, long long* nbt_t,
                                const float* Wr, const float* br, const float* gamma_r,
                                const float* beta_r, float* rmean_r, float* rvar_r, long long* nbt_r,
                                float momentum, float* wfold, float* bias, float* stat, void* ws,
                                size_t ws_bytes, int B, int Ci, int Co, int T, int V, hipStream_t stream) {
  const LayerStatsArgs a{
      .partials = partials, .rows = rows,
      .p = {.Wt = Wt, .bt = bt, .gt = gamma_t, .bet = beta_t, .rm_t = rmean_t, .rv_t = rvar_t, .nbt_t = nbt_t, .Wr = Wr, .br = br,
            .gr = gamma_r, .ber = beta_r, .rm_r = rmean_r, .rv_r = rvar_r, .nbt_r = nbt_r, .momentum = momentum},
      .out = {.wfold = wfold, .bias = bias, .stat = stat},
      .ws = ws, .ws_bytes = ws_bytes, .B = B, .Ci = Ci, .Co = Co, .stream = stream};
  if (int rc = check_layer_stats("layer_train_fold", a, kNeedPartials | kNeedFold | kNeedWs)) return rc;
  if (B <= 0 || Ci <= 0 || Co <= 0 || Ci > 64 || rows <= 0) return fail(COSKAD_ERR_ARG, "layer_train_fold: B=%d Ci=%d Co=%d rows=%d", B, Ci, Co, rows);
  const size_t E = 2 * ((size_t)Ci * Ci + Ci);
  if (ws_bytes < round_up((int)(E * sizeof(double)), 256)) return fail(COSKAD_ERR_WORKSPACE, "layer_train_fold: workspace %zu too small", ws_bytes);
  return launch_reduce_fold(partials, rows, reinterpret_cast<double*>(ws), (double)B * T * V, a.p, a.out, Ci, Co, stream);
}


int coskad_layer_train_moments_f32(const float* in, const float* A, const float* Tm, const float* in_slope, float* Z, double* sums,
                                   void* ws, size_t ws_bytes, int B, int Ci, int T, int V, hipStream_t stream) {
  const LayerStatsArgs a{.in = in, .A = A, .Tm = Tm, .in_slope = in_slope, .Zout = Z, .sums = sums, .ws = ws, .ws_bytes = ws_bytes,
                         .B = B, .Ci = Ci, .Co = Ci, .stream = stream};
  if (int rc = check_layer_stats("layer_train_moments", a, kNeedInput | kNeedSums | kNeedWs)) return rc;
  if (B <= 0 || Ci <= 0) return fail(COSKAD_ERR_ARG, "layer_train_moments: B=%d Ci=%d", B, Ci);
  if ((size_t)sums & 7) return fail(COSKAD_ERR_ARG, "layer_train_moments: sums must be 8-byte aligned");
  return dispatch_train_stats("layer_train_moments", a, T, V, false);
}

int coskad_layer_moment_sums_f32(const float* partials, int rows, int Ci, double* sums, hipStream_t stream) {
  if (!partials || !sums || rows <= 0 || Ci <= 0 || Ci > 64) return fail(COSKAD_ERR_ARG, "layer_moment_sums: bad argument");
  if ((size_t)sums & 7) return fail(COSKAD_ERR_ARG, "layer_moment_sums: sums must be 8-byte aligned");
  return launch_reduce_fold(partials, rows, sums, 0.0, BnConvParams{}, FoldOut{}, Ci, Ci, stream);
}

int coskad_layer_train_fold_sums_f32(const double* sums, double count, const float* Wt, const float* bt, const float* gamma_t,
                                     const float* beta_t, float* rmean_t, float* rvar_t, long long* nbt_t,
                                     const float* Wr, const float* br, const float* gamma_r,
                                     const float* beta_r, float* rmean_r, float* rvar_r, long long* nbt_r,
// ... 18 lines not shown
```

### coskad_amd/engine.py

```python
from __future__ import annotations

import os
from dataclasses import dataclass, field
from typing import Dict, List, Optional

import torch

from . import ops

Tensor = torch.Tensor


@dataclass
class LayerTensors:
    A: Tensor
    T: Tensor
    Wt: Tensor
    bt: Optional[Tensor]
    gt: Tensor
    bet: Tensor
    rm_t: Tensor
    rv_t: Tensor
    nbt_t: Tensor
    Wr: Optional[Tensor]
# ... 57 lines not shown

    def __init__(self) -> None:
        self.buf: Optional[Tensor] = None

    def get(self, nbytes: int, device) -> Tensor:
        if self.buf is None or self.buf.numel() < nbytes or self.buf.device != device:
            self.buf = torch.empty(int(nbytes), dtype=torch.uint8, device=device)
        return self.buf


@dataclass
class ChainCtx:
    inputs: List[Tensor] = field(default_factory=list)
    stats: List[Tensor] = field(default_factory=list)
    zs: List[Optional[Tensor]] = field(default_factory=list)
    in_slope: Optional[Tensor] = None
    sync: object = None
    sync_count: float = 0.0


EVAL_FIRST_PAIR = True
EVAL_WINDOW = True
EVAL_TAIL = True


def eval_fold(L: LayerTensors):
    key = L.fold_key() if L.cache is not None else None
    if key is not None and L.cache.get("key") == key:
        return L.cache["fold"]
    wb = ops.bn_fold(L.w2(L.Wt), L.bt, L.gt, L.bet, L.rm_t, L.rv_t, L.w2(L.Wr), L.br, L.gr, L.ber, L.rm_r, L.rv_r)
    if key is not None:
        L.cache["key"], L.cache["fold"] = key, wb
    return wb


def chain_forward(x: Tensor, layers: List[LayerTensors], training: bool, ws: Workspace,
                  in_slope: Optional[Tensor] = None, want_ctx: bool = False, sync=None, pending0=None):
    B, C, T, V = x.shape
    ctx = ChainCtx(in_slope=in_slope) if want_ctx else None
    sync_count = None
    batch_stats = [training or L.rm_t is None for L in layers]
    if sync is not None and training:
        import torch.distributed as dist
        if not STORE_Z:
            raise ValueError("SyncBN runs on the stored-Z training path")
        cnt = torch.tensor([float(B * T * V)], device=x.device, dtype=torch.float64)
        dist.all_reduce(cnt, group=sync)
        sync_count = float(cnt.item())
        if ctx is not None:
            ctx.sync, ctx.sync_count = sync, sync_count
    h, slope = x, in_slope
    n = len(layers)
    fuse = [False] * n
    ftab = None
    if all(batch_stats) and STORE_Z and FUSE_NEXT:
        for i in range(n - 1):
            fuse[i] = layers[i + 1].Ci == layers[i].Co and ops.layer_apply_next_ok(layers[i].Ci, layers[i].Co, T, V)
        nxt = [i + 1 for i in range(n - 1) if fuse[i]]
        if nxt:
            ftab = torch.empty(n, ops.ftab_floats(), device=x.device, dtype=torch.float32)
            for k in range(0, len(nxt), 4):
                grp = nxt[k:k + 4]
                ops.build_ftabs([layers[i].A for i in grp], [layers[i].T for i in grp], [ftab[i] for i in grp])
    fuse_flat = [False] * n
    if all(batch_stats) and STORE_Z and FUSE_NEXT and sync is None:
        for i in range(n - 1):
            fuse_flat[i] = (not fuse[i] and layers[i + 1].Ci == layers[i].Co and layers[i].Wr is not None
                            and ops.layer_apply_next_flat_ok(layers[i].Ci, layers[i].Co, T, V))
    skip = -1
    pending = pending0
    if pending0 is not None and not (batch_stats[0] and STORE_Z and sync is None):
        raise ValueError("chain_forward: pending0 is for the stored-Z training path without SyncBN")
    for i, L in enumerate(layers):
        if i == skip:
            continue
        if h.shape[1] != L.Ci:
            raise ValueError(f"layer expects {L.Ci} input channels, got {h.shape[1]}")
        Z = None
        if batch_stats[i]:
            buf = ws.get(ops.train_stats_ws_bytes(L.Ci), x.device)
            if sync_count is not None:
                if pending is not None:
                    Z, partials, rows = pending
                    sums = ops.layer_moment_sums(partials, rows, L.Ci)
                else:
                    Z = torch.empty_like(h)
                    sums = ops.layer_train_moments(h, L.A, L.T, slope, buf, Z=Z)
                dist.all_reduce(sums, group=sync)
                wfold, bias, stat = ops.layer_train_fold_sums(
                    sums, sync_count, L.w2(L.Wt), L.bt, L.gt, L.bet, L.rm_t, L.rv_t, L.nbt_t,
                    L.w2(L.Wr), L.br, L.gr, L.ber, L.rm_r, L.rv_r, L.nbt_r, momentum=L.step_momentum())
            elif pending is not None:
                Z, partials, rows = pending
                wfold, bias, stat = ops.layer_train_fold(
                    partials, rows, B, T, V, L.w2(L.Wt), L.bt, L.gt, L.bet, L.rm_t, L.rv_t, L.nbt_t,
                    L.w2(L.Wr), L.br, L.gr, L.ber, L.rm_r, L.rv_r, L.nbt_r, buf, momentum=L.step_momentum())
            else:
                if STORE_Z:
                    Z = torch.empty_like(h)
                wfold, bias, stat = ops.layer_train_stats(
                    h, L.A, L.T, slope, L.w2(L.Wt), L.bt, L.gt, L.bet, L.rm_t, L.rv_t, L.nbt_t,
                    L.w2(L.Wr), L.br, L.gr, L.ber, L.rm_r, L.rv_r, L.nbt_r, buf, momentum=L.step_momentum(), Z=Z)
        else:
            wfold, bias = eval_fold(L)
            stat = None
            if (EVAL_FIRST_PAIR and i == 0 and ctx is None and slope is None and n > 1 and not batch_stats[1] and layers[1].Ci == L.Co
                    and L.Wr is not None and wfold.shape[1] == L.Co
                    and ops.layer_first_pair_ok(L.Ci, L.Co, layers[1].Co, T, V)):
                N = layers[1]
                wf2, b2 = eval_fold(N)
                if wf2.shape[1] == N.Co:
                    h = ops.layer_first_pair_apply(h, L.A, L.T, wfold, bias, N.A, N.T, wf2, b2, L.Co, N.Co, L.slope)
                    slope, skip = N.slope, 1
                    continue
        pending = None
        if fuse[i]:
            rows_max = ops.layer_apply_next_rows(B, h.shape[1], L.Co)
            partials = torch.empty(rows_max * 2 * (L.Co * L.Co + L.Co), device=x.device, dtype=torch.float32)
            u, Zn, rows = ops.layer_apply_next(Z, h, wfold, bias, L.Co, slope, L.slope, ftab[i + 1], partials, T, V)
            pending = (Zn, partials, rows)
        elif fuse_flat[i] and Z is not None:
            u, Zn, partials, rows = ops.layer_apply_next_flat(Z, h, wfold, bias, L.Co, slope, L.slope, layers[i + 1].A, layers[i + 1].T)
            pending = (Zn, partials, rows)
        elif Z is not None:
            u = ops.layer_apply_z(Z, h, L.A, L.T, wfold, bias, L.Co, in_slope=slope)
        else:
            u = ops.layer_apply(h, L.A, L.T, wfold, bias, L.Co, in_slope=slope)
        if ctx is not None:
            ctx.inputs.append(h)
            ctx.stats.append(stat)
            ctx.zs.append(Z)
        h, slope = u, L.slope
    return h, ctx


STORE_Z = True
FUSE_BELOW = True
CHAIN_SKIP = frozenset()
FUSE_TOP = True
FUSE_NEXT = True


class SideStream:

    def __init__(self) -> None:
        self.stream: Optional[torch.cuda.Stream] = None
        self.dz = [None, None]
        self.ws = None
        self.done = [None, None]

    def ensure(self, nfloats: int, ws_bytes: int, device) -> None:
        if self.stream is None:
            self.stream = torch.cuda.Stream(device=device)
        for k in range(2):
            if self.dz[k] is None or self.dz[k].numel() < nfloats:
                self.dz[k] = torch.empty(nfloats, device=device, dtype=torch.float32)
        if self.ws is None or self.ws.numel() < ws_bytes:
            self.ws = torch.empty(ws_bytes, device=device, dtype=torch.uint8)


def btlnk_backward(ctx: Optional[ChainCtx], layers: List[LayerTensors], U: Tensor, W: Tensor, dz: Tensor, slope: Optional[Tensor],
                   dW: Tensor, db: Optional[Tensor], dslope: Optional[Tensor], ws: Workspace):
    B = U.shape[0]
    K, L = U.numel() // B, W.shape[0]
    i = len(layers) - 1 if layers else -1
    Z = ctx.zs[i] if (ctx is not None and ctx.zs and i >= 0) else None
    if (FUSE_TOP and Z is not None and U.dim() == 4 and layers[i].Wr is not None and L <= 16
            and ops.btlnk_bwd_chain_ok(K, U.shape[2] * U.shape[3], layers[i].Ci)):
        in_slope = layers[i - 1].slope if i > 0 else ctx.in_slope
        return ops.btlnk_bwd_chain(U, W, dz, slope, dW, db, dslope, ws, ctx.inputs[i], Z, in_slope)
    buf = ws.get(ops.btlnk_bwd_ws_bytes(B, K, L), U.device)
    return ops.btlnk_bwd(U, W, dz, slope, dW, db, dslope, buf), None


def chain_backward(ctx: ChainCtx, layers: List[LayerTensors], dU: Tensor, ws: Workspace,
                   grads: List[Dict[str, Tensor]], need_dx: bool, accumulate: bool = False,
                   side: Optional[SideStream] = None, stats_in=None, in_slope_grad: Optional[Tensor] = None) -> Optional[Tensor]:
    n = len(layers)
    if side is not None and stats_in is not None:
        raise ValueError("chain_backward: the side-stream path runs its own batch reductions (stats_in must be None)")
    if ctx.sync is not None and side is not None:
        raise ValueError("SyncBN runs on the main stream (side=None)")
    main = torch.cuda.current_stream() if side is not None else None
    if side is not None:
        side.done = [None, None]
    for i in range(n - 1, -1, -1):
        L = layers[i]
        x_in = ctx.inputs[i]
        B, Ci, T, V = x_in.shape
        in_slope = layers[i - 1].slope if i > 0 else ctx.in_slope
        g = dict(grads[i])
        g.pop("slope", None)
        if i > 0:
            g["slope_in"] = grads[i - 1]["slope"]
        elif in_slope_grad is not None and in_slope is not None:
            g["slope_in"] = in_slope_grad
        want_dx = need_dx or i > 0
        buf = ws.get(ops.layer_bwd_ws_bytes(B, Ci, L.Co, T, V), x_in.device)
        args = (x_in, dU, L.A, L.T, in_slope, ctx.stats[i], L.w2(L.Wt), L.gt, L.w2(L.Wr), L.gr, _as2d(g), buf)
        if side is None:
            sync = ctx.sync
            if sync is not None:
                import torch.distributed as dist
                if stats_in is None:
                    stats_in = ops.layer_bwd_stats(x_in, dU, L.A, L.T, in_slope, L.Wr is not None, buf, Z=ctx.zs[i])
                dist.all_reduce(ops.chain_sums(stats_in[0], stats_in[1], Ci, L.Co), group=sync)
            below = None
            Zi = ctx.zs[i] if ctx.zs else None
            if (FUSE_BELOW and i not in CHAIN_SKIP and Zi is not None and i > 0 and ctx.zs[i - 1] is not None
                    and in_slope is not None and layers[i - 1].Wr is not None):
                cb = ctx.inputs[i - 1].shape[1]
                rows = ops.layer_bwd_below_rows(B, Ci, L.Co, cb, T, V)
                if rows:
                    below = (ctx.inputs[i - 1], ctx.zs[i - 1], layers[i - 2].slope if i > 1 else ctx.in_slope,
                             torch.empty(ops.layer_bwd_below_floats(B, Ci, L.Co, cb, T, V), device=x_in.device, dtype=torch.float32))
            dIn = ops.layer_bwd(*args, need_dx=want_dx, accumulate=accumulate, Z=Zi,
                                stats_in=stats_in, below=below, stats_count=ctx.sync_count if sync is not None else 0.0)
            stats_in = (below[3], rows) if below is not None else None
        else:
            k = i & 1
            side.ensure(max(x.numel() for x in ctx.inputs), ops.layer_gcn_params_ws_bytes(T, V), x_in.device)
            if side.done[k] is not None:
                main.wait_event(side.done[k])
            dz = side.dz[k][:x_in.numel()].view(B, Ci, T, V)
            dIn = ops.layer_bwd_data(*args, dZ=dz, need_dx=want_dx, accumulate=accumulate, Z=ctx.zs[i] if ctx.zs else None)
# ... 64 lines not shown
```

### coskad_amd/ops.py

```python
from __future__ import annotations

import ctypes
from typing import Optional

import torch

from . import _lib
from ._lib import call

Tensor = torch.Tensor


def _stream() -> ctypes.c_void_p:
    return ctypes.c_void_p(torch.cuda.current_stream().cuda_stream)


def _chk(t: Optional[Tensor], name: str, shape=None, dtype=torch.float32, optional=False) -> None:
    if t is None:
        if optional:
            return
        raise ValueError(f"{name}: tensor required")
    if not t.is_cuda:
        raise _lib.CoskadHipError(f"{name}: expected a CUDA (ROCm) tensor, got device {t.device}; "
                                  "the COSKAD hot path runs only on the HIP extension (no CPU fallback)")
# ... 104 lines not shown
               out: Optional[Tensor] = None, score: Optional[Tensor] = None):
    B, Ci, T, V = x_in.shape
    _chk(x_in, "x_in"); _chk(A, "A", (T, V, V)); _chk(Tm, "T", (V, T, T))
    _chk(wfold, "wfold", (2 * Ci, cop(Co))); _chk(bias, "bias", (cop(Co),))
    _chk(in_slope, "in_slope", (1,), optional=True); _chk(out_slope, "out_slope", (1,), optional=True)
    if not (want_out or want_score):
        raise ValueError("layer_tail: neither the reconstruction nor the score asked for")
    if want_score:
        _chk(x, "x", (B, Co, T, V))
        if score is None:
            score = torch.empty(B, device=x_in.device, dtype=torch.float32)
        else:
            _chk(score, "score", (B,))
    if want_out:
        if out is None:
            out = torch.empty(B, Co, T, V, device=x_in.device, dtype=torch.float32)
        else:
            _chk(out, "out", (B, Co, T, V))
    out, score = (out if want_out else None), (score if want_score else None)
    call("coskad_layer_tail_f32", x_in, x if want_score else None, out, score, A, Tm, wfold, bias, in_slope, out_slope, B, Ci, Co, T, V,
         _stream(), tag=(Ci, Co))
    return out, score


def layer_first_pair_ok(Ci: int, Cm: int, Co: int, T: int, V: int) -> bool:
    return bool(_lib.lib().coskad_layer_first_pair_ok(T, V, Ci, Cm, Co))


def layer_first_pair_apply(x: Tensor, A1: Tensor, T1: Tensor, wfold1: Tensor, bias1: Tensor, A2: Tensor, T2: Tensor, wfold2: Tensor,
                           bias2: Tensor, Cm: int, Co: int, mid_slope: Tensor, out_slope: Optional[Tensor] = None) -> Tensor:
    B, Ci, T, V = x.shape
    _chk(x, "x", (B, 2, T, V)); _chk(A1, "A1", (T, V, V)); _chk(T1, "T1", (V, T, T)); _chk(A2, "A2", (T, V, V)); _chk(T2, "T2", (V, T, T))
    _chk(wfold1, "wfold1", (4, Cm)); _chk(bias1, "bias1", (Cm,)); _chk(wfold2, "wfold2", (2 * Cm, Co)); _chk(bias2, "bias2", (Co,))
    _chk(mid_slope, "mid_slope", (1,)); _chk(out_slope, "out_slope", (1,), optional=True)
    out = torch.empty(B, Co, T, V, device=x.device, dtype=torch.float32)
    call("coskad_layer_first_pair_apply_f32", x, out, A1, T1, wfold1, bias1, A2, T2, wfold2, bias2, mid_slope, out_slope, B, Cm, Co, T, V,
         _stream())
    return out


def layer_fits(Ci: int, Co: int, T: int, V: int) -> bool:
    return bool(_lib.lib().coskad_layer_fits(Ci, Co, T, V))


def stat_floats(Ci: int, Co: int) -> int:
    return _lib.lib().coskad_stat_floats(Ci, Co)


def train_stats_ws_bytes(Ci: int) -> int:
    return _lib.lib().coskad_train_stats_ws_bytes(Ci)


def layer_train_stats(x, A, Tm, in_slope, Wt, bt, gt, bet, rm_t, rv_t, nbt_t,
                      Wr, br, gr, ber, rm_r, rv_r, nbt_r, ws, momentum: float = 0.1, Z: Optional[Tensor] = None):
    B, Ci, T, V = x.shape
    Co = Wt.shape[0]
    _chk(x, "x"); _chk(A, "A", (T, V, V)); _chk(Tm, "T", (V, T, T))
    _chk(Wt, "Wt", (Co, Ci)); _chk(gt, "gamma_t", (Co,)); _chk(bet, "beta_t", (Co,))
    for n, t in (("bt", bt), ("rm_t", rm_t), ("rv_t", rv_t), ("br", br), ("gamma_r", gr), ("beta_r", ber),
                 ("rm_r", rm_r), ("rv_r", rv_r)):
        _chk(t, n, (Co,), optional=True)
    _chk(Wr, "Wr", (Co, Ci), optional=True)
    _chk(in_slope, "in_slope", (1,), optional=True)
    _chk(nbt_t, "nbt_t", (), dtype=torch.int64, optional=True)
    _chk(nbt_r, "nbt_r", (), dtype=torch.int64, optional=True)
    need = train_stats_ws_bytes(Ci)
    if ws is None or ws.numel() * ws.element_size() < need:
        raise ValueError(f"workspace too small: need {need} bytes")
    wfold = torch.empty(2 * Ci, cop(Co), device=x.device, dtype=torch.float32)
    bias = torch.empty(cop(Co), device=x.device, dtype=torch.float32)
    stat = torch.empty(stat_floats(Ci, Co), device=x.device, dtype=torch.float32)
    _chk(Z, "Z", tuple(x.shape), optional=True)
    args = (x, A, Tm, in_slope, Wt, bt, gt, bet, rm_t, rv_t, nbt_t, Wr, br, gr, ber, rm_r, rv_r, nbt_r, momentum, wfold, bias, stat, ws,
            ws.numel() * ws.element_size(), B, Ci, Co, T, V, _stream())
    note_raw_write()
    if Z is None:
        call("coskad_layer_train_stats_f32", *args)
    else:
        call("coskad_layer_train_stats_z_f32", *args, Z)
    return wfold, bias, stat


def layer_train_moments(x, A, Tm, in_slope, ws, Z: Optional[Tensor] = None) -> Tensor:
    B, Ci, T, V = x.shape
    _chk(x, "x"); _chk(A, "A", (T, V, V)); _chk(Tm, "T", (V, T, T)); _chk(in_slope, "in_slope", (1,), optional=True)
    _chk(Z, "Z", tuple(x.shape), optional=True)
    need = train_stats_ws_bytes(Ci)
    if ws is None or _bytes(ws) < need:
        raise ValueError(f"workspace too small: need {need} bytes")
    sums = torch.empty(2 * (Ci * Ci + Ci), device=x.device, dtype=torch.float64)
    call("coskad_layer_train_moments_f32", x, A, Tm, in_slope, Z, sums, ws, _bytes(ws), B, Ci, T, V, _stream())
    return sums


def layer_moment_sums(partials: Tensor, rows: int, Ci: int) -> Tensor:
    _chk(partials, "partials")
    if partials.numel() < rows * 2 * (Ci * Ci + Ci):
        raise ValueError("layer_moment_sums: partials smaller than rows x 2 (Ci^2 + Ci)")
    sums = torch.empty(2 * (Ci * Ci + Ci), device=partials.device, dtype=torch.float64)
    call("coskad_layer_moment_sums_f32", partials, rows, Ci, sums, _stream())
    return sums


def layer_train_fold_sums(sums, count, Wt, bt, gt, bet, rm_t, rv_t, nbt_t, Wr, br, gr, ber, rm_r, rv_r, nbt_r, momentum: float = 0.1):
    Co, Ci = Wt.shape
    _chk(sums, "sums", (2 * (Ci * Ci + Ci),), dtype=torch.float64); _chk(Wt, "Wt", (Co, Ci)); _chk(gt, "gamma_t", (Co,)); _chk(bet, "beta_t", (Co,))
    for n, t in (("bt", bt), ("rm_t", rm_t), ("rv_t", rv_t), ("br", br), ("gamma_r", gr), ("beta_r", ber), ("rm_r", rm_r), ("rv_r", rv_r)):
        _chk(t, n, (Co,), optional=True)
    _chk(Wr, "Wr", (Co, Ci), optional=True)
    _chk(nbt_t, "nbt_t", (), dtype=torch.int64, optional=True); _chk(nbt_r, "nbt_r", (), dtype=torch.int64, optional=True)
    wfold = torch.empty(2 * Ci, cop(Co), device=Wt.device, dtype=torch.float32)
    bias = torch.empty(cop(Co), device=Wt.device, dtype=torch.float32)
    stat = torch.empty(stat_floats(Ci, Co), device=Wt.device, dtype=torch.float32)
    note_raw_write()
    call("coskad_layer_train_fold_sums_f32", sums, float(count), Wt, bt, gt, bet, rm_t, rv_t, nbt_t, Wr, br, gr, ber, rm_r, rv_r, nbt_r,
         momentum, wfold, bias, stat, Ci, Co, _stream())
    return wfold, bias, stat


def layer_bwd_stats(x_in, dU, A, Tm, in_slope, has_residual: bool, ws, Z=None):
    B, Ci, T, V = x_in.shape
    Co = dU.shape[1]
    _chk(x_in, "x_in"); _chk(dU, "dU", (B, Co, T, V)); _chk(A, "A", (T, V, V)); _chk(Tm, "T", (V, T, T))
    _chk(in_slope, "in_slope", (1,), optional=True); _chk(Z, "Z", (B, Ci, T, V), optional=True)
    need = layer_bwd_ws_bytes(B, Ci, Co, T, V)
    if ws is None or _bytes(ws) < need:
        raise ValueError(f"workspace too small: need {need} bytes")
    buf = torch.empty(_lib.lib().coskad_layer_bwd_stats_floats(B, Ci, Co, T, V), device=x_in.device, dtype=torch.float32)
    rows = ctypes.c_int(0)
    call("coskad_layer_bwd_stats_f32", x_in, dU, A, Tm, in_slope, 1 if has_residual else 0, buf, _bytes(buf), ctypes.byref(rows), ws,
         _bytes(ws), B, Ci, Co, T, V, _stream(), Z)
    return buf, rows.value


def chain_sums(buf: Tensor, rows: int, Ci: int, Co: int) -> Tensor:
    off = _lib.lib().coskad_layer_bwd_sums_offset(rows, Ci, Co)
    E = 2 * Co * Ci + Co
    return buf[off:off + 2 * E].view(torch.float64)


def layer_apply_z(Z, x, A, Tm, wfold, bias, Co, in_slope=None, out_slope=None, out=None):
    B, Ci, T, V = x.shape
    _chk(x, "x"); _chk(Z, "Z", (B, Ci, T, V)); _chk(wfold, "wfold", (2 * Ci, cop(Co))); _chk(bias, "bias", (cop(Co),))
    _chk(in_slope, "in_slope", (1,), optional=True); _chk(out_slope, "out_slope", (1,), optional=True)
    if out is None:
        out = torch.empty(B, Co, T, V, device=x.device, dtype=torch.float32)
    _chk(A, "A", (T, V, V)); _chk(Tm, "T", (V, T, T))
    call("coskad_layer_apply_z_f32", Z, x, out, A, Tm, wfold, bias, in_slope, out_slope, B, Ci, Co, T, V, _stream())
    return out


def layer_apply_next_ok(Ci: int, Co: int, T: int, V: int) -> bool:
    return bool(_lib.lib().coskad_layer_apply_next_ok(Ci, Co, T, V))


def layer_apply_next_rows(B: int, Ci: int, Co: int) -> int:
    return _lib.lib().coskad_layer_apply_next_rows(B, Ci, Co)


def ftab_floats() -> int:
    return _lib.lib().coskad_ftab_floats()


def build_ftabs(As, Ts, tabs) -> None:
    n = len(As)
    if not (1 <= n <= 4) or len(Ts) != n or len(tabs) != n:
        raise ValueError("build_ftabs: 1..4 layers, equal list lengths")
    T, V = As[0].shape[0], As[0].shape[1]
    nf = ftab_floats()
    for A, Tm, tab in zip(As, Ts, tabs):
        _chk(A, "A", (T, V, V)); _chk(Tm, "T", (V, T, T)); _chk(tab, "tab", (nf,))
    arr = ctypes.c_void_p * n
    call("coskad_build_ftab_f32", arr(*[t.data_ptr() for t in As]), arr(*[t.data_ptr() for t in Ts]),
         arr(*[t.data_ptr() for t in tabs]), n, T, V, _stream())


def layer_apply_next(Z, x, wfold, bias, Co, in_slope, out_slope, ftab_next, partials, T, V, out=None, Z_next=None):
    B, Ci = x.shape[0], x.shape[1]
    _chk(x, "x", (B, Ci, T, V)); _chk(Z, "Z", (B, Ci, T, V)); _chk(wfold, "wfold", (2 * Ci, cop(Co))); _chk(bias, "bias", (cop(Co),))
    _chk(in_slope, "in_slope", (1,), optional=True); _chk(out_slope, "out_slope", (1,)); _chk(ftab_next, "ftab_next", (ftab_floats(),))
    _chk(partials, "partials")
    if out is None:
        out = torch.empty(B, Co, T, V, device=x.device, dtype=torch.float32)
    if Z_next is None:
        Z_next = torch.empty(B, Co, T, V, device=x.device, dtype=torch.float32)
    _chk(out, "out", (B, Co, T, V)); _chk(Z_next, "Z_next", (B, Co, T, V))
    rows = layer_apply_next_rows(B, Ci, Co)
    call("coskad_layer_apply_next_f32", Z, x, out, wfold, bias, in_slope, out_slope, ftab_next, Z_next, partials, _bytes(partials), B, Ci,
         Co, T, V, _stream(), tag=(Ci, Co))
    return out, Z_next, rows


def layer_apply_next_flat_ok(Ci: int, Co: int, T: int, V: int) -> bool:
    return bool(_lib.lib().coskad_layer_apply_next_flat_ok(Ci, Co, T, V))


def layer_apply_next_flat(Z, x, wfold, bias, Co, in_slope, out_slope, A_next, T_next):
    B, Ci, T, V = x.shape
    _chk(x, "x"); _chk(Z, "Z", (B, Ci, T, V)); _chk(wfold, "wfold", (2 * Ci, cop(Co))); _chk(bias, "bias", (cop(Co),))
    _chk(in_slope, "in_slope", (1,), optional=True); _chk(out_slope, "out_slope", (1,))
    _chk(A_next, "A_next", (T, V, V)); _chk(T_next, "T_next", (V, T, T))
    rows = int(_lib.lib().coskad_layer_apply_next_flat_rows(B))
    out = torch.empty(B, Co, T, V, device=x.device, dtype=torch.float32)
    Zn = torch.empty(B, Co, T, V, device=x.device, dtype=torch.float32)
    partials = torch.empty(rows * 2 * (Co * Co + Co), device=x.device, dtype=torch.float32)
    call("coskad_layer_apply_next_flat_f32", Z, x, out, wfold, bias, in_slope, out_slope, A_next, T_next, Zn, partials, _bytes(partials), B,
         Ci, Co, T, V, _stream(), tag=(Ci, Co))
    return out, Zn, partials, rows


def layer_train_fold(partials, rows, B, T, V, Wt, bt, gt, bet, rm_t, rv_t, nbt_t, Wr, br, gr, ber, rm_r, rv_r, nbt_r, ws,
                     momentum: float = 0.1):
    Co, Ci = Wt.shape
    _chk(partials, "partials"); _chk(Wt, "Wt", (Co, Ci)); _chk(gt, "gamma_t", (Co,)); _chk(bet, "beta_t", (Co,))
    for n, t in (("bt", bt), ("rm_t", rm_t), ("rv_t", rv_t), ("br", br), ("gamma_r", gr), ("beta_r", ber),
                 ("rm_r", rm_r), ("rv_r", rv_r)):
        _chk(t, n, (Co,), optional=True)
    _chk(Wr, "Wr", (Co, Ci), optional=True)
    _chk(nbt_t, "nbt_t", (), dtype=torch.int64, optional=True)
    _chk(nbt_r, "nbt_r", (), dtype=torch.int64, optional=True)
    if partials.numel() < rows * 2 * (Ci * Ci + Ci):
        raise ValueError("layer_train_fold: partials smaller than rows x 2 (Ci^2 + Ci)")
    need = train_stats_ws_bytes(Ci)
    if ws is None or _bytes(ws) < need:
        raise ValueError(f"workspace too small: need {need} bytes")
    wfold = torch.empty(2 * Ci, cop(Co), device=Wt.device, dtype=torch.float32)
    bias = torch.empty(cop(Co), device=Wt.device, dtype=torch.float32)
# ... 138 lines not shown
    return z


BTLNK_SPLITK_MIN_B = 1
BTLNK_LMAX = 512


def btlnk_bwd_ws_bytes(B, K, L) -> int:
    return _lib.lib().coskad_btlnk_bwd_ws_bytes(B, K, L)


def btlnk_bwd(U, W, dz, slope, dW, db, dslope, ws, dU=None, accumulate=False):
    B = U.shape[0]
    K = U.numel() // B
    L = W.shape[0]
    _chk(U, "U"); _chk(W, "W", (L, K)); _chk(dz, "dz", (B, L)); _chk(dW, "dW", (L, K))
    _chk(db, "db", (L,), optional=True); _chk(dslope, "dslope", (1,), optional=True); _chk(slope, "slope", (1,), optional=True)
    need = btlnk_bwd_ws_bytes(B, K, L)
    if ws is None or _bytes(ws) < need:
        raise ValueError(f"workspace too small: need {need} bytes")
    if dU is None:
        dU = torch.empty_like(U)
    call("coskad_btlnk_bwd_f32", U, W, dz, slope, dU, dW, db, dslope, ws, _bytes(ws), 1 if accumulate else 0, B, K, L, _stream())
    return dU


def btlnk_bwd_chain_ok(K: int, TV: int, below_Ci: int) -> bool:
    return bool(_lib.lib().coskad_btlnk_bwd_chain_ok(K, TV, below_Ci))


def btlnk_bwd_chain(U, W, dz, slope, dW, db, dslope, ws, below_in, below_Z, below_in_slope, dU=None, accumulate=False):
    B, Ch, T, V = U.shape
    TV = T * V
    K = Ch * TV
    L = W.shape[0]
    Ci = below_in.shape[1]
    _chk(U, "U"); _chk(W, "W", (L, K)); _chk(dz, "dz", (B, L)); _chk(dW, "dW", (L, K))
    _chk(db, "db", (L,), optional=True); _chk(dslope, "dslope", (1,), optional=True); _chk(slope, "slope", (1,), optional=True)
    _chk(below_in, "below_in", (B, Ci, T, V)); _chk(below_Z, "below_Z", (B, Ci, T, V)); _chk(below_in_slope, "below_in_slope", (1,), optional=True)
    if not btlnk_bwd_chain_ok(K, TV, Ci):
        raise ValueError(f"btlnk_bwd_chain: shape K={K} TV={TV} Ci={Ci} not supported")
    lib = _lib.lib()
    need = lib.coskad_btlnk_bwd_chain_ws_bytes(B, K, L, TV)
    buf = ws.get(need, U.device)
    stats = torch.empty(lib.coskad_btlnk_bwd_chain_floats(B, TV, Ci), device=U.device, dtype=torch.float32)
    if dU is None:
        dU = torch.empty_like(U)
    rows = ctypes.c_int(0)
    call("coskad_btlnk_bwd_chain_f32", U, W, dz, slope, dU, dW, db, dslope, buf, _bytes(buf), 1 if accumulate else 0, B, K, L, below_in,
         below_Z, below_in_slope, Ci, TV, stats, _bytes(stats), ctypes.byref(rows), _stream())
    return dU, (stats, rows.value)


def _cuda_f32(t: Tensor, name: str) -> None:
    if not t.is_cuda:
        raise _lib.CoskadHipError(f"{name}: expected a CUDA (ROCm) tensor, got device {t.device}; no CPU fallback")
    if t.dtype != torch.float32:
        raise TypeError(f"{name}: expected float32, got {t.dtype}")


def _b3(t: Tensor):
    if t.dim() == 2:
        return 1, t.shape[0], t.shape[1], 0, t.stride(0), t.stride(1)
    if t.dim() == 3:
        return t.shape[0], t.shape[1], t.shape[2], t.stride(0), t.stride(1), t.stride(2)
    raise ValueError("gemm operands are 2-D or 3-D")


def gemm(A: Tensor, B: Tensor, out: Optional[Tensor] = None, bias: Optional[Tensor] = None, bias_mode: int = 0,
         bias_mod: int = 1, relu: bool = False, accumulate: bool = False) -> Tensor:
    _cuda_f32(A, "A"); _cuda_f32(B, "B")
    ba, M, K, sab, sam, sak = _b3(A)
    bb, K2, N, sbb, sbk, sbn = _b3(B)
    if K != K2:
        raise ValueError(f"gemm: inner sizes differ ({K} vs {K2})")
    batch = max(ba, bb)
    if ba not in (1, batch) or bb not in (1, batch):
        raise ValueError("gemm: batch sizes do not broadcast")
    if ba == 1:
        sab = 0
    if bb == 1:
        sbb = 0
    if out is None:
        out = torch.empty((batch, M, N) if (A.dim() == 3 or B.dim() == 3) else (M, N), device=A.device, dtype=torch.float32)
    _cuda_f32(out, "out")
    bc, Mc, Nc, scb, scm, scn = _b3(out)
    if (Mc, Nc) != (M, N) or bc != batch:
        raise ValueError(f"gemm: out has shape {tuple(out.shape)}, expected batch {batch} x {M} x {N}")
    _chk(bias, "bias", optional=True)
    call("coskad_gemm_f32", A, B, out, bias, sab, sam, sak, sbb, sbk, sbn, scb, scm, scn, M, N, K, batch, bias_mode, bias_mod,
         1 if relu else 0, 0, 0, 0, 1 if accumulate else 0, _stream())
    return out


def gemm_reduce(A: Tensor, B: Tensor, out: Tensor, target_chunks: int = 64, ktotal: int = 0, accumulate: bool = False) -> Tensor:
    _cuda_f32(A, "A"); _cuda_f32(B, "B"); _chk(out, "out")
    ba, M, K, sab, sam, sak = _b3(A)
    bb, K2, N, sbb, sbk, sbn = _b3(B)
    if K != K2 or ba != bb or tuple(out.shape) != (M, N):
        raise ValueError("gemm_reduce: shape mismatch")
    chunk = max(1, (ba + target_chunks - 1) // target_chunks)
    chunks = (ba + chunk - 1) // chunk
    part = torch.empty(chunks, M, N, device=A.device, dtype=torch.float32)
    call("coskad_gemm_f32", A, B, part, None, sab, sam, sak, sbb, sbk, sbn, 0, 0, 0, M, N, K, ba, 0, 1, 0, 1, chunk, ktotal, 0, _stream())
    call("coskad_gemm_sum_f32", part, chunks, M * N, out, 1 if accumulate else 0, _stream())
    return out
# ... 769 lines not shown
```

### coskad_amd/trainer.py

```python
from __future__ import annotations

from typing import Dict, List, Optional

import torch
import torch.distributed as dist

from . import engine, ops, parallel
from .models.graph_layers.stsgcn import layer_tensors

Tensor = torch.Tensor


class FlatParams:

    def __init__(self, module: torch.nn.Module) -> None:
        named = [(n, p) for n, p in module.named_parameters()]
        self.names = [n for n, _ in named]
        al = lambda k: (k + 3) // 4 * 4
        total = sum(al(p.numel()) for _, p in named)
        dev = named[0][1].device
        self.flat = torch.zeros(total, device=dev, dtype=torch.float32)
        self.grad = torch.zeros(total, device=dev, dtype=torch.float32)
        self.reg_mask = torch.zeros(total, device=dev, dtype=torch.float32)
        self.views: Dict[str, Tensor] = {}
# ... 373 lines not shown


class _OneClassHead:

    def _head(self, z: Tensor):
        m = self.model
        if self.head == 'euclidean':
            return ops.mse_head(z, m.c, acc=self.center_acc)[:2]
        if self.head == 'poincare':
            return ops.poincare_head(z, m.c, acc=self.center_acc)[:2]
        if self.head == 'mahalanobis':
            return ops.mahalanobis_head(z, m.c, m.inv_cov_matrix, acc=self.center_acc, gram=self.gram_acc)[:2]
        raise ValueError(f"unknown head {self.head}")

    def refresh_center(self, eps: float = 1e-3) -> Tensor:
        parallel.allreduce_sum_(self.center_acc, self.pg)
        L = self.model.latent_dim
        c = ops.center_finalize(self.center_acc, eps, L) if self.head != 'poincare' else ops.midpoint_finalize(self.center_acc, L)
        self.model.c.copy_(c)
        self.center_acc.zero_()
        return self.model.c

    def refresh_inv_cov(self, mu: Tensor, reset: bool = True) -> Tensor:
        parallel.allreduce_sum_(self.gram_acc, self.pg)
        acc = self.center_acc.clone()
        parallel.allreduce_sum_(acc, self.pg)
        self.model.inv_cov_matrix.copy_(inv_cov_from_moments(self.gram_acc, acc, mu, self.model.latent_dim))
        if reset:
            self.gram_acc.zero_()
        return self.model.inv_cov_matrix


def _stacked_heads(m):
    return torch.cat([m.fc_mean.weight, m.fc_var.weight], 0), torch.cat([m.fc_mean.bias, m.fc_var.bias], 0)


def _unstack_head_grads(gv: Dict[str, Tensor], L: int, gW: Tensor, gb: Tensor) -> None:
    gv["fc_mean.weight"].copy_(gW[:L]); gv["fc_var.weight"].copy_(gW[L:])
    gv["fc_mean.bias"].copy_(gb[:L]); gv["fc_var.bias"].copy_(gb[L:])


class _LinearProjector:

    def __init__(self, lin, fp: "FlatParams", ws: engine.Workspace, wname: str = "btlnk.") -> None:
        self.lin, self.ws = lin, ws
        self.gW, self.gb = fp.gviews[wname + "weight"], fp.gviews.get(wname + "bias")

    def forward(self, U: Tensor, slope):
        W = self.lin.weight
        return ops.btlnk_fwd(U, W, self.lin.bias, slope, ws=self.ws), W

    def backward(self, W, dy, U, slope, ctx, top_layers, last_slope_grad):
        return engine.btlnk_backward(ctx, top_layers or [], U, W, dy, slope, self.gW, self.gb, last_slope_grad, self.ws)


class _MLPProjector(_LinearProjector):

    def __init__(self, mlp, fp: "FlatParams", ws: engine.Workspace) -> None:
        super().__init__(mlp.net[0], fp, ws, "btlnk.net.0.")
        gv = fp.gviews
        self.blocks = [(bn, lin, {"gamma": gv[f"btlnk.net.{3 * i + 1}.weight"], "beta": gv[f"btlnk.net.{3 * i + 1}.bias"],
                                  "W2": gv[f"btlnk.net.{3 * i + 3}.weight"], "b2": gv.get(f"btlnk.net.{3 * i + 3}.bias")})
                       for i, (bn, lin) in enumerate(mlp.blocks())]

    def forward(self, U: Tensor, slope):
        if U.shape[0] == 1:
            raise ValueError("Expected more than 1 value per channel when training (BatchNorm1d of the mlp projector)")
        y, W = super().forward(U, slope)
        saved = []
        for bn, lin, _ in self.blocks:
            z, stat = ops.mlp_head_fwd(y, bn.weight, bn.bias, bn.running_mean, bn.running_var, bn.num_batches_tracked,
                                       lin.weight, lin.bias, True, momentum=ops.bn_momentum(bn), eps=bn.eps)
            saved.append((y, stat))
            y = z
        return y, (W, saved)

    def backward(self, saved, dy, *top):
        W, block_saved = saved
        for (bn, lin, g), (y_in, stat) in zip(reversed(self.blocks), reversed(block_saved)):
            dy = ops.mlp_head_bwd(y_in, stat, bn.weight, bn.bias, lin.weight, dy, g, True)
        return super().backward(W, dy, *top)


class _StackedHeads:

    def __init__(self, model, fp: "FlatParams", ws: engine.Workspace) -> None:
        self.model, self.ws, self.gv = model, ws, fp.gviews

    def forward(self, U: Tensor, slope):
        W, b = _stacked_heads(self.model)
        return ops.btlnk_fwd(U, W, b, slope, ws=self.ws), (W, b)

    def backward(self, saved, dy, U, slope, ctx, top_layers, last_slope_grad):
        W, b = saved
        gW, gb = torch.empty_like(W), torch.empty_like(b)
        res = engine.btlnk_backward(ctx, top_layers or [], U, W, dy, slope, gW, gb, last_slope_grad, self.ws)
        _unstack_head_grads(self.gv, self.model.latent_dim, gW, gb)
        return res


def _projector(model, fp: "FlatParams", ws: engine.Workspace):
    from .models.common.components import MLP
    if isinstance(model.btlnk, MLP):
        return _MLPProjector(model.btlnk, fp, ws)
    if isinstance(model.btlnk, torch.nn.Linear):
        return _LinearProjector(model.btlnk, fp, ws)
# ... 44 lines not shown
        from .models.sts.ae import STSE
        from .models.common.components import MLP
        mlp = isinstance(model.btlnk, MLP)
        if not isinstance(model, STSE) or not (isinstance(model.btlnk, torch.nn.Linear) or (mlp and model.btlnk.hip_ok)):
            raise TypeError("STSETrainStep drives an STSE with projector='linear' or an 'mlp' within the kernels' widths")
        super().__init__(model, lr, alpha, betas, eps, process_group)
        self.head = head
        dev = self.fp.flat.device
        self.hyper = torch.tensor([lr, 1.0, 1.0, 0.0], device=dev, dtype=torch.float32)
        L = model.latent_dim
        self.center_acc = torch.zeros(ops.head_slots(L), device=dev, dtype=torch.float32)
        self.gram_acc = torch.zeros(L, L, device=dev, dtype=torch.float32) if head == 'mahalanobis' else None
        plain_gcn = _is_plain_gcn(model.encoder)
        wide = plain_gcn or any(l.is_wide for l in model.encoder.model)
        if plain_gcn and (side_stream or use_graph):
            raise ValueError("a plain-GCN encoder runs on the main stream, outside hipGraph capture")
        if wide and (side_stream or use_graph):
            raise ValueError("an encoder with wide layers runs on the main stream, outside hipGraph capture")
        self.side = engine.SideStream() if side_stream else None
        self.sync_group = None
        if sync_bn and self.world > 1:
            if mlp or side_stream or use_graph or wide:
                raise ValueError("sync_bn: encoder BatchNorm only (STS-GCN encoder within the tile kernels, linear projector), on the "
                                 "main stream, outside hipGraph capture")
            self.sync_group = process_group if process_group is not None else dist.group.WORLD
        if plain_gcn:
            self.stack = _PlainGCNStack(model.encoder, self.fp)
        else:
            plain = not wide and (use_graph or side_stream or sync_bn or not any(_is_commute(l) for l in model.encoder.model))
            self.stack = _FlatStack(list(model.encoder.model), self.fp, "encoder.model.", plain=plain, side=self.side,
                                    sync=self.sync_group, window=fused_window)
        names = self.fp.names
        first_tail = next((i for i, n in enumerate(names) if n.startswith("btlnk.")), None)
        tail = first_tail is not None and all(n.startswith("btlnk.") for n in names[first_tail:])
        self.tail_off = self.fp.offsets[names[first_tail]] if tail else None
        if use_graph and any(isinstance(b, torch.nn.modules.batchnorm._BatchNorm) and b.momentum is None for b in model.modules()):
            raise ValueError("use_graph: BatchNorm with momentum=None changes its averaging factor every step (a launch argument here); "
                             "capture needs a fixed momentum")
        self.use_graph = use_graph
        self._graph = self._x_static = self._stats_static = None

    @property
    def layers(self) -> List[engine.LayerTensors]:
        segs = self.stack.segs
        return segs[0].layers if len(segs) == 1 and segs[0].kind == 'tile' else []

    def set_lr(self, lr: float) -> None:
        self.hyper[0] = lr
        self.lr = float(lr)

    def _body(self, x: Tensor) -> Tensor:
        U, slope, saved_stack = self.stack.forward(x, self.ws)
        ctx, top_layers = self.stack.top(saved_stack)
        z, saved = self.projector.forward(U, slope)
        stats, dz = self._head(z)
        dU, top_stats = self.projector.backward(saved, dz, U, slope, ctx if self.side is None else None, top_layers,
                                                self.stack.last_slope_grad)
        work = None
        if self.world > 1 and self.tail_off is not None:
            work = dist.all_reduce(self.fp.grad[self.tail_off:], group=self.pg, async_op=True)
        self.stack.backward(saved_stack, dU, self.ws, need_dx=False, top_stats=top_stats)
        if self.world > 1:
            head = self.fp.grad if work is None else self.fp.grad[:self.tail_off]
            dist.all_reduce(head, group=self.pg)
            if work is not None:
                work.wait()
        self._adam()
        return stats

    def step(self, x: Tensor) -> Tensor:
        self.steps += 1
        x = x.contiguous()
        if not self.use_graph:
            return self._body(x)
        if self._graph is None or self._x_static.shape != x.shape:
            self._x_static = x.clone()
            s = torch.cuda.Stream()
            s.wait_stream(torch.cuda.current_stream())
            with torch.cuda.stream(s):
                self._body(self._x_static)
            torch.cuda.current_stream().wait_stream(s)
            self.steps += 1
            self._graph = torch.cuda.CUDAGraph()
            with torch.cuda.graph(self._graph):
                self._stats_static = self._body(self._x_static)
        self._x_static.copy_(x)
        self._graph.replay()
        ops.note_raw_write()
        return self._stats_static


class _LatentHead:

    def __init__(self, step: "STSAETrainStep", heads: bool = False) -> None:
        self.model, self.acc, self.gv, self.heads = step.model, step.center_acc, step.fp.gviews, heads
        self.beta, self.gamma = step.beta, step.gamma


class _CentreLatent(_LatentHead):

    def forward(self, y: Tensor):
        stats, dz, _ = ops.mse_head(y, self.model.c, acc=self.acc)
        return y, dz, {'head': stats[0:1]}, None

    def backward(self, saved, dz: Tensor) -> Tensor:
        return dz


class _PowerSphericalLatent(_LatentHead):

# ... 264 lines not shown
```

### include/coskad_hip.h

```cpp
#ifndef COSKAD_HIP_H
#define COSKAD_HIP_H
#include <hip/hip_runtime_api.h>

#ifdef __cplusplus
extern "C" {
#endif

int coskad_abi_version(void);
const char* coskad_last_error(void);

int coskad_probe_begin(int kernel, int Ci, int Co);
int coskad_probe_stride(int n);
int coskad_probe_end(float* avg_ms, int* launches);


int coskad_window_ok(int T, int V);

int coskad_gcn_f32(const float* in, float* out, const float* A, const float* Tm, int rows, int T, int V,
                   int adjoint, hipStream_t stream);

int coskad_bn_fold_f32(const float* Wt, const float* bt, const float* gamma_t, const float* beta_t,
                       const float* mean_t, const float* var_t, const float* Wr, const float* br,
                       const float* gamma_r, const float* beta_r, const float* mean_r,
                       const float* var_r, float* wfold, float* bias, int Ci, int Co,
// ... 9 lines not shown
int coskad_layer_tail_max_grid(int T, int V, int Ci);
int coskad_layer_tail_f32(const float* in, const float* x, float* out, float* score,
                          const float* A, const float* Tm, const float* wfold, const float* bias,
                          const float* in_slope, const float* out_slope,
                          int B, int Ci, int Co, int T, int V, hipStream_t stream);

int coskad_prelu_fwd_f32(const float* u, const float* slope, float* out, size_t n, hipStream_t stream);
int coskad_prelu_bwd_f32(const float* u, const float* dout, const float* slope, float* du, float* dslope,
                         float* ws, int accumulate, size_t n, hipStream_t stream);

int coskad_rec_head_f32(const float* U, const float* x, const float* slope, float* xrec, float* dU, float* loss, float* dslope,
                        float upstream, float* ws, int accumulate, size_t n, hipStream_t stream);

size_t coskad_rev_btlnk_ws_floats(int B, int N, int L);
int coskad_rev_btlnk_wide_ok(int N, int L);
int coskad_rev_btlnk_fwd_f32(const float* z, const float* W, const float* bias, float* H, int B, int N, int L, hipStream_t stream);
int coskad_rev_btlnk_bwd_f32(const float* dH, const float* z, const float* W, float* dz, int dz_accumulate, float* dW, float* db,
                             int accumulate, float* ws, int B, int N, int L, hipStream_t stream);


size_t coskad_train_stats_ws_bytes(int Ci);
int coskad_stat_floats(int Ci, int Co);

int coskad_layer_train_stats_f32(const float* in, const float* A, const float* Tm, const float* in_slope,
                                 const float* Wt, const float* bt, const float* gamma_t,
                                 const float* beta_t, float* rmean_t, float* rvar_t, long long* nbt_t,
                                 const float* Wr, const float* br, const float* gamma_r,
                                 const float* beta_r, float* rmean_r, float* rvar_r, long long* nbt_r,
                                 float momentum, float* wfold, float* bias, float* stat, void* ws,
                                 size_t ws_bytes, int B, int Ci, int Co, int T, int V,
                                 hipStream_t stream);

int coskad_layer_train_window_ok(int T, int V, int Ci, int Co);

int coskad_layer_train_window_narrow_ok(int T, int V, int Ci, int Co);

int coskad_layer_train_stats_z_f32(const float* in, const float* A, const float* Tm, const float* in_slope,
                                   const float* Wt, const float* bt, const float* gamma_t,
                                   const float* beta_t, float* rmean_t, float* rvar_t, long long* nbt_t,
                                   const float* Wr, const float* br, const float* gamma_r,
                                   const float* beta_r, float* rmean_r, float* rvar_r, long long* nbt_r,
                                   float momentum, float* wfold, float* bias, float* stat, void* ws,
                                   size_t ws_bytes, int B, int Ci, int Co, int T, int V,
                                   hipStream_t stream, float* Z);
int coskad_layer_apply_z_f32(const float* Z, const float* in, float* out, const float* A, const float* Tm,
                             const float* wfold, const float* bias, const float* in_slope, const float* out_slope,
                             int B, int Ci, int Co, int T, int V, hipStream_t stream);

int coskad_layer_apply_next_ok(int Ci, int Co, int T, int V);
int coskad_ftab_floats(void);
int coskad_layer_apply_next_rows(int B, int Ci, int Co);
int coskad_build_ftab_f32(const float* const* A, const float* const* Tm, float* const* tab, int n, int T, int V,
                          hipStream_t stream);
int coskad_layer_apply_next_f32(const float* Z, const float* in, float* out, const float* wfold, const float* bias,
                                const float* in_slope, const float* out_slope, const float* ftab_next, float* Z_next,
                                float* partials, size_t partials_bytes, int B, int Ci, int Co, int T, int V,
                                hipStream_t stream);
int coskad_layer_train_fold_f32(const float* partials, int rows, const float* Wt, const float* bt, const float* gamma_t,
                                const float* beta_t, float* rmean_t, float* rvar_t, long long* nbt_t,
                                const float* Wr, const float* br, const float* gamma_r,
                                const float* beta_r, float* rmean_r, float* rvar_r, long long* nbt_r,
                                float momentum, float* wfold, float* bias, float* stat, void* ws,
                                size_t ws_bytes, int B, int Ci, int Co, int T, int V, hipStream_t stream);

int coskad_gather_f32(const float* src, const int* idx, float* out, size_t n, hipStream_t stream);
int coskad_fused_encoder_out_floats(void);
int coskad_fused_encoder_f32(const float* x, float* out, const float* tab, const float* wreg, const float* slopes, int B,
                             int T, int V, hipStream_t stream);

int coskad_gemm_f32(const float* A, const float* B, float* C, const float* bias, long long sa_b, long long sa_m,
                    long long sa_k, long long sb_b, long long sb_k, long long sb_n, long long sc_b, long long sc_m,
                    long long sc_n, int M, int N, int K, int batch, int bias_mode, int bias_mod, int relu, int reduce,
                    int chunk, long long ktotal, int accum, hipStream_t stream);
int coskad_gemm_sum_f32(const float* partials, int chunks, size_t E, float* out, int accumulate, hipStream_t stream);
int coskad_relu_bwd_f32(const float* out, const float* dout, float* g, float* part, int Nb, int C, int P, int slices,
                        hipStream_t stream);
int coskad_softmax_rows_f32(const float* x, float* y, int n, hipStream_t stream);
int coskad_softmax_rows_bwd_f32(const float* y, const float* dy, float* dx, int n, hipStream_t stream);

int coskad_plain_gcn_ok(int Ci, int Co, int P);
size_t coskad_plain_gcn_ws_bytes(int B, int Ci, int Co, int P, int grid_cap);
int coskad_plain_gcn_fwd_f32(const float* X, const float* W, const float* Ap, const float* bias, float* O, float* save, int B,
                             int Ci, int Co, int P, int grid_cap, hipStream_t stream);
int coskad_plain_gcn_bwd_f32(const float* X, const float* S, const float* O, const float* dO, const float* W, const float* Ap,
                             float* dX, float* dW, float* db, float* D, void* ws, size_t ws_bytes, int B, int Ci, int Co, int P,
                             int need_dx, int need_da, int accumulate, int grid_cap, hipStream_t stream);

int coskad_conv1x1_ok(int M, int K, int P);
int coskad_conv1x1_stat_rows(int M, int K, int P, int batch);
int coskad_conv1x1_f32(const float* A, long long sa_m, long long sa_k, const float* In, float* Out, const float* bias, double* stats,
                       int M, int K, int P, int batch, int accumulate, hipStream_t stream);
int coskad_bn2_stats_parts_f32(const double* parts, int rows, float* stat, float* running_mean, float* running_var,
                               long long* num_batches_tracked, float momentum, float eps, double count, int C, hipStream_t stream);
int coskad_conv1x1_wgrad_ok(int M, int K, int P);
int coskad_conv1x1_wgrad_f32(const float* G, const float* X, float* partials, int M, int K, int P, int batch, int chunk,
                             hipStream_t stream);

size_t coskad_bn2_ws_bytes(int Nb, int C);
size_t coskad_bn2_bwd_ws_bytes(int Nb, int C);
int coskad_bn2_stats_f32(const float* x, float* stat, float* running_mean, float* running_var, long long* num_batches_tracked,
                         float momentum, float eps, int training, void* ws, size_t ws_bytes, int Nb, int C, int P,
                         hipStream_t stream);
int coskad_bn2_apply_prelu_f32(const float* Ct, const float* Cr, const float* stat_t, const float* gamma_t, const float* beta_t,
                               const float* stat_r, const float* gamma_r, const float* beta_r, const float* slope, float* out,
                               int Nb, int C, int P, hipStream_t stream, float drop_p, unsigned long long drop_seed);
int coskad_bn2_bwd_f32(const float* Ct, const float* Cr, const float* dOut, const float* stat_t, const float* gamma_t,
// ... 48 lines not shown
                         const float* Wr, const float* gamma_r, float* dIn, float* dA, float* dT, float* dWt,
                         float* dbt, float* dgamma_t, float* dbeta_t, float* dWr, float* dbr,
                         float* dgamma_r, float* dbeta_r, float* dslope_in, void* ws, size_t ws_bytes,
                         int accumulate, int B, int Ci, int Co, int T, int V, hipStream_t stream);

int coskad_layer_bwd_z_f32(const float* in, const float* dU, const float* A, const float* Tm,
                           const float* in_slope, const float* stat, const float* Wt, const float* gamma_t,
                           const float* Wr, const float* gamma_r, float* dIn, float* dA, float* dT, float* dWt,
                           float* dbt, float* dgamma_t, float* dbeta_t, float* dWr, float* dbr,
                           float* dgamma_r, float* dbeta_r, float* dslope_in, void* ws, size_t ws_bytes,
                           int accumulate, int B, int Ci, int Co, int T, int V, hipStream_t stream, const float* Z);

int coskad_layer_bwd_data_f32(const float* in, const float* dU, const float* A, const float* Tm,
                              const float* in_slope, const float* stat, const float* Wt, const float* gamma_t,
                              const float* Wr, const float* gamma_r, float* dIn, float* dZ, float* dWt, float* dbt,
                              float* dgamma_t, float* dbeta_t, float* dWr, float* dbr, float* dgamma_r,
                              float* dbeta_r, float* dslope_in, void* ws, size_t ws_bytes, int accumulate, int B,
                              int Ci, int Co, int T, int V, hipStream_t stream, const float* Z );
size_t coskad_layer_gcn_params_ws_bytes(int T, int V);
int coskad_layer_gcn_params_f32(const float* in, const float* in_slope, const float* dZ, const float* A,
                                const float* Tm, float* dA, float* dT, void* ws, size_t ws_bytes, int accumulate,
                                int B, int Ci, int T, int V, hipStream_t stream);

size_t coskad_gcn_bwd_params_ws_bytes(int T, int V);
int coskad_gcn_bwd_params_f32(const float* x, const float* dZ, const float* A, const float* Tm, float* dA,
                              float* dT, void* ws, size_t ws_bytes, int accumulate, int rows, int T, int V,
                              hipStream_t stream);

int coskad_gcn_bwd_params_dx_f32(const float* x, const float* dZ, const float* A, const float* Tm, float* dA, float* dT,
                                 float* dX, const float* dX_add, void* ws, size_t ws_bytes, int accumulate, int rows, int T,
                                 int V, hipStream_t stream);


int coskad_btlnk_fwd_f32(const float* U, const float* W, const float* bias, const float* slope, float* z,
                         int B, int K, int L, hipStream_t stream);

size_t coskad_btlnk_fwd_ws_bytes(int B);
size_t coskad_btlnk_fwd_ws_bytes_l(int B, int K, int L);
int coskad_btlnk_fwd_ws_f32(const float* U, const float* W, const float* bias, const float* slope, float* z, void* ws,
                            size_t ws_bytes, int B, int K, int L, hipStream_t stream);
size_t coskad_btlnk_bwd_ws_bytes(int B, int K, int L);
int coskad_btlnk_bwd_f32(const float* U, const float* W, const float* dz, const float* slope, float* dU,
                         float* dW, float* db, float* dslope, void* ws, size_t ws_bytes, int accumulate,
                         int B, int K, int L, hipStream_t stream);

int coskad_btlnk_bwd_chain_ok(int K, int TV, int below_Ci);
int coskad_btlnk_bwd_chain_rows(int B, int TV);
size_t coskad_btlnk_bwd_chain_floats(int B, int TV, int below_Ci);
size_t coskad_btlnk_bwd_chain_ws_bytes(int B, int K, int L, int TV);
int coskad_btlnk_bwd_chain_f32(const float* U, const float* W, const float* dz, const float* slope, float* dU, float* dW,
                               float* db, float* dslope, void* ws, size_t ws_bytes, int accumulate, int B, int K, int L,
                               const float* below_in, const float* below_Z, const float* below_in_slope, int below_Ci, int TV,
                               float* stats_out, size_t stats_out_bytes, int* stats_rows, hipStream_t stream);


int coskad_gather_transform_f32(const float* xy, const long long* index, const float* mats, float* out, int B, int N,
                                int ntrans, int TV, hipStream_t stream);


int coskad_score_pad_row_max(void);
int coskad_score_tile(void);
int coskad_score_auc_ws(int F);
int coskad_score_person_frames_f64(const void* scores, int scores_f64, const int* win_ptr, const int* win_idx, double* pf,
                                   int n_scores, int n_rows, hipStream_t stream);
int coskad_score_pad_f64(double* pf, const int* row_ptr, int n_persons, int pad_size, int n_max, hipStream_t stream);
int coskad_score_clip_max_f64(const double* pf, const int* row_ptr, const int* pc_ptr, const int* out_clip, const int* out_frame,
                              double* raw, int n_clips, int n_transform, int F, hipStream_t stream);
int coskad_score_smooth_f64(const double* raw, const int* tiles, const double* taps, int n_taps, double* per_t, double* mean,
                            int n_tiles, int n_transform, int F, hipStream_t stream);
int coskad_score_auc_f64(const double* sorted_scores, const int* gt_sorted, const long long* cum_neg, double* out, long long* ws,
                         size_t ws_elems, int F, hipStream_t stream);


int coskad_head_slots(void);
size_t coskad_head_ws_floats(int B);
int coskad_head_slots_l(int L);
size_t coskad_head_ws_floats_l(int B, int L);

int coskad_mse_head_f32(const float* z, const float* c, float* dz, float* score, float* stats, float* acc,
                        float upstream, float* ws, int B, int L, hipStream_t stream);

int coskad_mahalanobis_head_f32(const float* z, const float* c, const float* VI, float* dz, float* score,
                                float* stats, float* acc, float* gram, int gram_accumulate, float upstream,
                                float* ws, int B, int L, hipStream_t stream);

int coskad_poincare_head_f32(const float* z, const float* c, float* dz, float* zh, float* score,
                             float* stats, float* acc, float upstream, float* ws, int B, int L,
                             hipStream_t stream);
int coskad_poincare_dist_f32(const float* zh, const float* c, float* score, int B, int L, hipStream_t stream);
int coskad_poincare_logmap0_f32(const float* y, float* out, int B, int L, hipStream_t stream);

int coskad_lowrank_fold_ok(int latent, int TV);
int coskad_lowrank_fold_fwd_f32(const float* X, const double* G, const float* gamma0, const float* beta0, const float* cbias0,
                                float* rmean0, float* rvar0, long long* nbt0, float momentum0, float eps0, const float* gamma1,
                                const float* beta1, const float* cbias1, float* rmean1, float* rvar1, long long* nbt1, float momentum1,
                                float eps1, double n_pos, float* Mw, float* Mb, double* saved, double* xbar, double* xx, int Co, int TV,
                                hipStream_t stream);
int coskad_lowrank_fold_bwd_f32(const float* X, const double* G, const float* dMw, const float* dMb, const double* saved,
                                const double* xbar, const double* xx, const float* gamma0, const float* gamma1, double n_pos, float* dX,
                                float* dgamma, float* dbeta, double* dGc, int Co, int TV, hipStream_t stream);

int coskad_narrow_conv_rows(int B, int TV);
int coskad_narrow_conv_fwd_f32(const float* U, const float* in_slope, const float* W, float* out, int B, int Ci, int J, int TV,
                               hipStream_t stream);
int coskad_narrow_conv_bwd_f32(const float* U, const float* in_slope, const float* W, const float* dOut, float* dU, float* partials,
                               size_t partials_floats, int B, int Ci, int J, int TV, hipStream_t stream);
// ... 66 lines not shown
```

Before: 3.004 million clips/s.

## Fuse bottleneck forward sum and MSE head into bottleneck backward chain kernel

For the euclidean linear-projector path, the forward split-K partials are no longer summed by a separate kernel. The backward chain kernel recomputes dz from the partials inside its main loop through LDS, and extra blocks in the same grid write z, dz and the head partials. The head finalize moves into a spare block of the reduce kernel, and the first-layer moments kernel also gains extra blocks that build the ftab. This removes several small launches and the dz round trip through memory, at the cost of extra LDS, more kernel template variants and more per-iteration work in the backward loop.

```diff
diff --git a/coskad_amd/csrc/bottleneck.hip b/coskad_amd/csrc/bottleneck.hip
--- a/coskad_amd/csrc/bottleneck.hip
+++ b/coskad_amd/csrc/bottleneck.hip
@@ -1,5 +1,6 @@
 #include "tile_ops.h"
 #include "layer_launch.h"
+#include "heads_common.h"
 
 namespace coskad {
 
@@ -230,9 +231,13 @@
                                                        const float* __restrict__ dap, int nda,
                                                        float* __restrict__ dslope, int accumulate,
                                                        const float* __restrict__ rows, int RP, int RE,
-                                                       double* __restrict__ rsum) {
+                                                       double* __restrict__ rsum, HeadFin fin) {
   __shared__ double sh[256];
   const unsigned nE = (unsigned)((E + 255) / 256);
+  if (fin.part && blockIdx.x == fin.block) {
+    head_finalize_slot(fin.part, fin.P, fin.scale0, fin.stats, fin.acc, threadIdx.x);
+    return;
+  }
   if (blockIdx.x > nE + L) {
     const int col = threadIdx.x & 15, slice = threadIdx.x >> 4;
     const int e = (int)(blockIdx.x - (nE + L + 1)) * 16 + col;
@@ -307,10 +312,12 @@
 
 int launch_btlnk_reduce(const float* partials, int P, size_t E, float* out, const float* dz, int B, int L, float* db,
                         const float* dap, int nda, float* dslope, int accumulate, hipStream_t stream, const float* rows,
-                        int RP, int RE, double* rsum) {
+                        int RP, int RE, double* rsum, HeadFin fin) {
   const unsigned extra = rows ? (unsigned)ceil_div(RE, 16) : 0u;
-  hipLaunchKernelGGL(k_btlnk_reduce, dim3((unsigned)((E + 255) / 256) + L + 1 + extra), dim3(256), 0, stream, partials, P, E, out, dz,
-                     B, L, db, dap, nda, dslope, accumulate, rows, RP, RE, rsum);
+  unsigned blocks = (unsigned)((E + 255) / 256) + L + 1 + extra;
+  if (fin.part) fin.block = blocks++;
+  hipLaunchKernelGGL(k_btlnk_reduce, dim3(blocks), dim3(256), 0, stream, partials, P, E, out, dz,
+                     B, L, db, dap, nda, dslope, accumulate, rows, RP, RE, rsum, fin);
   return check_launch("btlnk_bwd_reduce");
 }
 
@@ -356,6 +363,19 @@
   if ((rc = check_launch("btlnk_fwd_t"))) return rc;
   hipLaunchKernelGGL(k_btlnk_fwd_sum, dim3(ceil_div(B * 16, 256)), dim3(256), 0, stream, part, bias, z, B, L, kBtlKS);
   return check_launch("btlnk_fwd_sum");
+}
+
+int coskad_btlnk_fwd_ks(void) { return kBtlKS; }
+
+int coskad_btlnk_fwd_parts_f32(const float* U, const float* W, const float* slope, float* part, size_t part_bytes, int B, int K,
+                               int L, hipStream_t stream) {
+  if (!U || !W || !part) return fail(COSKAD_ERR_ARG, "btlnk_fwd_parts: null pointer");
+  if (B <= 0 || K <= 0 || L <= 0) return fail(COSKAD_ERR_ARG, "btlnk_fwd_parts: B=%d K=%d L=%d", B, K, L);
+  if (L > 16) return fail(COSKAD_ERR_SHAPE, "btlnk_fwd_parts: latent_dim=%d > 16 not supported", L);
+  if (K % 16) return fail(COSKAD_ERR_SHAPE, "btlnk_fwd_parts: K=%d must be a multiple of 16", K);
+  if (part_bytes < coskad_btlnk_fwd_ws_bytes(B)) return fail(COSKAD_ERR_WORKSPACE, "btlnk_fwd_parts: partials buffer too small");
+  hipLaunchKernelGGL(k_btlnk_fwd_t, dim3(ceil_div(B, 64), kBtlKS), dim3(256), 0, stream, U, W, slope, part, B, K, L);
+  return check_launch("btlnk_fwd_t");
 }
 
 size_t coskad_btlnk_bwd_ws_bytes(int B, int K, int L) {
diff --git a/coskad_amd/csrc/btlnk_chain.hip b/coskad_amd/csrc/btlnk_chain.hip
--- a/coskad_amd/csrc/btlnk_chain.hip
+++ b/coskad_amd/csrc/btlnk_chain.hip
@@ -1,5 +1,6 @@
 #include "fused_ops.h"
 #include "layer_launch.h"
+#include "heads_common.h"
 
 namespace coskad {
 namespace bc {
@@ -24,11 +25,52 @@
 #define BC_SKIP 0
 #endif
 
-template <int CT>
+struct HeadRide {
+  const float *part, *bias, *c;
+  float gscale, scale0;
+  float *z, *dz, *score, *hpart, *stats, *acc;
+  int KS, nbwd, nhead;
+};
+constexpr int kDzStr = 20;
+constexpr int kMaxKS = 8;
+
+__device__ __forceinline__ void head_ride_block(const HeadRide& hr, int B, int L) {
+  float vals[kHeadSlots];
+#pragma unroll
+  for (int k = 0; k < kHeadSlots; ++k) vals[k] = 0.f;
+  const Vec c = load_vec(hr.c, L);
+  const int bid = (int)blockIdx.x - hr.nbwd;
+  const int n = bid * kFlatBlock + (int)threadIdx.x;
+  if (n < B) {
+    Vec u, g;
+#pragma unroll
+    for (int j = 0; j < LMAX; ++j) {
+      float z = 0.f;
+      if (j < L) {
+        float sum = 0.f;
+        for (int k = 0; k < hr.KS; ++k) sum += hr.part[((size_t)k * B + n) * 16 + j];
+        z = sum + (hr.bias ? hr.bias[j] : 0.f);
+      }
+      u.v[j] = z;
+    }
+    store_vec(hr.z + (size_t)n * L, u, L);
+    const float sq = mse_head_row(u, c, L, hr.gscale, vals, g);
+    store_vec(hr.dz + (size_t)n * L, g, L);
+    if (hr.score) hr.score[n] = sq / (float)L;
+  }
+  block_partials(vals, hr.hpart, hr.scale0, hr.stats, hr.acc, bid, hr.nhead);
+}
+
+template <int CT, bool HD>
 __global__ __launch_bounds__(kThreads, 1) void k_btlnk_bwd_stats(
     const float* __restrict__ U, const float* __restrict__ W, const float* __restrict__ dz, const float* __restrict__ slope,
     float* __restrict__ dU, float* __restrict__ dWp, float* __restrict__ dap, const float* __restrict__ xin,
-    const float* __restrict__ Zg, const float* __restrict__ in_slope, float* __restrict__ prow, int B, int TV, int L, int chunk) {
+    const float* __restrict__ Zg, const float* __restrict__ in_slope, float* __restrict__ prow, int B, int TV, int L, int chunk, HeadRide hr) {
+  static_assert(kFlatBlock == kThreads, "the riding head blocks are k_mse_head's");
+  if (HD && (int)blockIdx.x >= hr.nbwd) {
+    head_ride_block(hr, B, L);
+    return;
+  }
   constexpr int Ci = 16 * CT, NR = 2 * Ci;
   constexpr int GCS = HID * RSTR + 4, ZCS = NR * RSTR + 4;
   constexpr int NL = NR * NCL * (PT / 4) / kThreads;
@@ -36,12 +78,13 @@
   extern __shared__ __attribute__((aligned(16))) float lds[];
   float* G = lds;
   float* ZX = lds + NCL * GCS;
+  float* DZ = ZX + NCL * ZCS;
   const int tid = threadIdx.x, lane = tid & 63;
   const int wave = __builtin_amdgcn_readfirstlane(tid >> 6);
   const int wc = wave & 3, h = wave >> 2;
   const int c = lane & 15, q = lane >> 4;
   const int K = HID * TV;
-  const int nwg = gridDim.x, npt = (TV + PT - 1) / PT;
+  const int nwg = HD ? hr.nbwd : (int)gridDim.x, npt = (TV + PT - 1) / PT;
   int wg = blockIdx.x;
   if (BC_XCD) {
     const int xq = nwg / 8, xr = nwg % 8, xcd = wg % 8;
@@ -122,11 +165,48 @@
     }
   };
 
+  const bool dz_maker = HD && wave < 4;
+  const int mk_cl = tid >> 4, mk_l = tid & 15;
+  const bool mk_ok = dz_maker && mk_l < L;
+  const float mk_c = mk_ok ? hr.c[mk_l] : 0.f, mk_b = (mk_ok && hr.bias) ? hr.bias[mk_l] : 0.f;
+  auto dz_fetch = [&](int n0, float (&pv)[kMaxKS]) {
+    const int n = n0 + mk_cl;
+#pragma unroll
+    for (int k = 0; k < kMaxKS; ++k) pv[k] = (mk_ok && n < nend && k < hr.KS) ? hr.part[((size_t)k * B + n) * 16 + mk_l] : 0.f;
+  };
+  auto dz_put = [&](int n0, const float (&pv)[kMaxKS]) {
+    if (!dz_maker) return;
+    float g = 0.f;
+    if (mk_ok && n0 + mk_cl < nend) {
+      float sum = 0.f;
+#pragma unroll
+      for (int k = 0; k < kMaxKS; ++k)
+        if (k < hr.KS) sum += pv[k];
+      const float d = (sum + mk_b) - mk_c;
+      g = 2.f * d * hr.gscale;
+    }
+    DZ[mk_cl * kDzStr + mk_l] = g;
+  };
+  auto dz_read = [&](float (&da_)[4], float (&db_)[4]) {
+#pragma unroll
+    for (int g = 0; g < 4; ++g) da_[g] = DZ[c * kDzStr + 4 * g + q];
+#pragma unroll
+    for (int r = 0; r < 4; ++r) db_[r] = DZ[(4 * q + r) * kDzStr + c];
+  };
+
   float4 zx[NL];
-  float ucur[8][4], dza[4], dzb[4];
+  float ucur[8][4], dza[4], dzb[4], pv[kMaxKS];
   u_load(nbeg, ucur);
-  dz_load(nbeg, dza, dzb);
+  if (HD) {
+    dz_fetch(nbeg, pv);
+  } else {
+    dz_load(nbeg, dza, dzb);
+  }
   zx_load(nbeg, zx);
+  if (HD) {
+    dz_put(nbeg, pv);
+    lds_barrier();
+  }
 
   float* gw = G + 4 * q * GCS + ch0 * RSTR + c;
   const float* ga = G + 4 * q * GCS + (16 * wc + c) * RSTR + 8 * h;
@@ -134,6 +214,7 @@
 
   for (int n0 = nbeg; n0 < nend; n0 += NCL) {
     float unext[8][4];
+    if (HD) dz_read(dza, dzb);
     if (BC_PF == 2) { zx_store(zx); zx_load(n0 + NCL, zx); }
     if (BC_PF) u_load(n0 + NCL, unext);
     {
@@ -171,7 +252,11 @@
     } else {
       u_load(n0 + NCL, ucur);
     }
-    dz_load(n0 + NCL, dza, dzb);
+    if (HD) {
+      dz_fetch(n0 + NCL, pv);
+    } else {
+      dz_load(n0 + NCL, dza, dzb);
+    }
     if (BC_PF != 2) zx_load(n0 + NCL, zx);
 #pragma unroll
     for (int pl = 0; pl < 8; ++pl)
@@ -186,6 +271,7 @@
           qacc[t] = mfma(av, zb[r * ZCS + (Ci + 16 * t) * RSTR + pl], qacc[t]);
         }
       }
+    if (HD) dz_put(n0 + NCL, pv);
     lds_barrier();
   }
 
@@ -273,10 +359,10 @@
   return ((size_t)p.S * L * K + (size_t)p.S * p.npt + 64) * sizeof(float);
 }
 
-int coskad_btlnk_bwd_chain_f32(const float* U, const float* W, const float* dz, const float* slope, float* dU, float* dW,
-                               float* db, float* dslope, void* ws, size_t ws_bytes, int accumulate, int B, int K, int L,
-                               const float* below_in, const float* below_Z, const float* below_in_slope, int below_Ci, int TV,
-                               float* stats_out, size_t stats_out_bytes, int* stats_rows, hipStream_t stream) {
+static int btlnk_bwd_chain_run(const float* U, const float* W, const float* dz, const float* slope, float* dU, float* dW, float* db,
+                               float* dslope, void* ws, size_t ws_bytes, int accumulate, int B, int K, int L, const float* below_in,
+                               const float* below_Z, const float* below_in_slope, int below_Ci, int TV, float* stats_out,
+                               size_t stats_out_bytes, int* stats_rows, bc::HeadRide* hr, hipStream_t stream) {
   if (!U || !W || !dz || !dU || !dW || !ws || !below_in || !below_Z || !stats_out || !stats_rows)
     return fail(COSKAD_ERR_ARG, "btlnk_bwd_chain: null pointer");
   if (B <= 0 || K <= 0 || L <= 0) return fail(COSKAD_ERR_ARG, "btlnk_bwd_chain: B=%d K=%d L=%d", B, K, L);
@@ -292,26 +378,68 @@
   const int E = 2 * bc::HID * below_Ci + bc::HID;
   float* dWp = reinterpret_cast<float*>(ws);
   float* dap = dWp + (size_t)p.S * L * K;
-  const size_t lds = (size_t)bc::NCL * ((bc::HID * bc::RSTR + 4) + (2 * below_Ci * bc::RSTR + 4)) * sizeof(float);
+  size_t lds = (size_t)bc::NCL * ((bc::HID * bc::RSTR + 4) + (2 * below_Ci * bc::RSTR + 4)) * sizeof(float);
+  bc::HeadRide ride = {};
+  int grid = rows;
+  if (hr) {
+    hr->nbwd = rows;
+    hr->nhead = head_blocks(B);
+    ride = *hr;
+    grid += hr->nhead;
+    lds += (size_t)bc::NCL * bc::kDzStr * sizeof(float);
+  }
   int rc;
   {
   ProbeScope probe(KID_BTLNK_BWD, below_Ci, L, stream);
+#define BC_LAUNCH(CT_, HD_)                                                                                                          \
+  do {                                                                                                                               \
+    auto k = bc::k_btlnk_bwd_stats<CT_, HD_>;                                                                                        \
+    (void)hipFuncSetAttribute((const void*)k, hipFuncAttributeMaxDynamicSharedMemorySize, (int)lds);                                 \
+    hipLaunchKernelGGL(k, dim3(grid), dim3(bc::kThreads), lds, stream, U, W, dz, slope, dU, dWp, dap, below_in, below_Z,             \
+                       below_in_slope, stats_out, B, TV, L, p.chunk, ride);                                                          \
+  } while (0)
   if (below_Ci == 32) {
-    auto k = bc::k_btlnk_bwd_stats<2>;
-    (void)hipFuncSetAttribute((const void*)k, hipFuncAttributeMaxDynamicSharedMemorySize, (int)lds);
-    hipLaunchKernelGGL(k, dim3(p.npt * p.S), dim3(bc::kThreads), lds, stream, U, W, dz, slope, dU, dWp, dap, below_in, below_Z,
-                       below_in_slope, stats_out, B, TV, L, p.chunk);
+    if (hr) BC_LAUNCH(2, true); else BC_LAUNCH(2, false);
   } else {
-    auto k = bc::k_btlnk_bwd_stats<1>;
-    (void)hipFuncSetAttribute((const void*)k, hipFuncAttributeMaxDynamicSharedMemorySize, (int)lds);
-    hipLaunchKernelGGL(k, dim3(p.npt * p.S), dim3(bc::kThreads), lds, stream, U, W, dz, slope, dU, dWp, dap, below_in, below_Z,
-                       below_in_slope, stats_out, B, TV, L, p.chunk);
-  }
+    if (hr) BC_LAUNCH(1, true); else BC_LAUNCH(1, false);
+  }
+#undef BC_LAUNCH
   }
   if ((rc = check_launch("btlnk_bwd_stats"))) return rc;
   *stats_rows = rows;
+  HeadFin fin;
+  if (hr && hr->nhead > 1 && (hr->stats || hr->acc)) {
+    fin.part = hr->hpart; fin.P = hr->nhead; fin.scale0 = hr->scale0; fin.stats = hr->stats; fin.acc = hr->acc;
+  }
   return launch_btlnk_reduce(dWp, p.S, (size_t)L * K, dW, dz, B, L, db, dap, rows, (dslope && slope) ? dslope : nullptr, accumulate, stream,
-                             stats_out, rows, E, reinterpret_cast<double*>(stats_out + bc::sums_offset(rows, E)));
-}
-
-}
+                             stats_out, rows, E, reinterpret_cast<double*>(stats_out + bc::sums_offset(rows, E)), fin);
+}
+
+int coskad_btlnk_bwd_chain_f32(const float* U, const float* W, const float* dz, const float* slope, float* dU, float* dW,
+                               float* db, float* dslope, void* ws, size_t ws_bytes, int accumulate, int B, int K, int L,
+                               const float* below_in, const float* below_Z, const float* below_in_slope, int below_Ci, int TV,
+                               float* stats_out, size_t stats_out_bytes, int* stats_rows, hipStream_t stream) {
+  return btlnk_bwd_chain_run(U, W, dz, slope, dU, dW, db, dslope, ws, ws_bytes, accumulate, B, K, L, below_in, below_Z, below_in_slope,
+                             below_Ci, TV, stats_out, stats_out_bytes, stats_rows, nullptr, stream);
+}
+
+int coskad_btlnk_bwd_chain_head_f32(const float* U, const float* W, const float* part, int KS, const float* bias, const float* c,
+                                    float upstream, float* z, float* dz, float* score, float* stats, float* acc, float* head_ws,
+                                    const float* slope, float* dU, float* dW, float* db, float* dslope, void* ws, size_t ws_bytes,
+                                    int accumulate, int B, int K, int L, const float* below_in, const float* below_Z,
+                                    const float* below_in_slope, int below_Ci, int TV, float* stats_out, size_t stats_out_bytes,
+                                    int* stats_rows, hipStream_t stream) {
+  if (!part || !c || !z || !dz || !head_ws) return fail(COSKAD_ERR_ARG, "btlnk_bwd_chain_head: null pointer");
+  if (KS <= 0 || KS > bc::kMaxKS) return fail(COSKAD_ERR_SHAPE, "btlnk_bwd_chain_head: %d K slices (1 .. %d)", KS, bc::kMaxKS);
+  if (B <= 0 || L <= 0 || L > 16) return fail(COSKAD_ERR_SHAPE, "btlnk_bwd_chain_head: B=%d latent_dim=%d (1 .. 16)", B, L);
+  bc::HeadRide hr = {};
+  hr.part = part; hr.bias = bias; hr.c = c;
+  hr.gscale = upstream / ((float)B * (float)L);
+  hr.scale0 = 1.f / ((float)B * (float)L);
+  hr.z = z; hr.dz = dz; hr.score = score; hr.hpart = head_ws; hr.stats = stats; hr.acc = acc;
+  hr.KS = KS;
+  return btlnk_bwd_chain_run(U, W, dz, slope, dU, dW, db, dslope, ws, ws_bytes, accumulate, B, K, L, below_in, below_Z, below_in_slope,
+                             below_Ci, TV, stats_out, stats_out_bytes, stats_rows, &hr, stream);
+}
+
+}
diff --git a/coskad_amd/csrc/first_layer.hip b/coskad_amd/csrc/first_layer.hip
--- a/coskad_amd/csrc/first_layer.hip
+++ b/coskad_amd/csrc/first_layer.hip
@@ -1,5 +1,6 @@
 #include "mfma_ops.h"
 #include "layer_launch.h"
+#include "ftab_ops.h"
 
 namespace coskad {
 namespace fl {
@@ -196,11 +197,20 @@
 
 
 constexpr int NWM = 8;
+constexpr int kFtabBlocks = (ftab_elems<12, 17>() + 64 * NWM - 1) / (64 * NWM);
 template <int T, int V, int CI>
 __global__ __launch_bounds__(64 * NWM, 4) void k_first_moments(const float* __restrict__ in, const float* __restrict__ Aw,
                                                           const float* __restrict__ Tw, const float* __restrict__ in_slope,
-                                                          float* __restrict__ partials, int B, float* __restrict__ Zout) {
+                                                          float* __restrict__ partials, int B, float* __restrict__ Zout, int nmom,
+                                                          FtabArgs tabs) {
   constexpr int TV = T * V, NA = T * V * V, NT = V * T * T, KP = (TV + 63) / 64;
+  if ((int)blockIdx.x >= nmom) {
+    if constexpr (T == 12 && V == 17) {
+      const int b = (int)blockIdx.x - nmom;
+      ftab_store<T, V>(tabs, b / kFtabBlocks, (b % kFtabBlocks) * 64 * NWM + (int)threadIdx.x);
+    }
+    return;
+  }
   extern __shared__ __attribute__((aligned(16))) float lds[];
   float* AwL = lds;
   float* TwL = AwL + NA;
@@ -223,9 +233,9 @@
     for (int b = 0; b < CI; ++b) { mx[a][b] = 0.f; mz[a][b] = 0.f; }
   }
   __syncthreads();
-  const int rounds = (B + gridDim.x * NWM - 1) / (gridDim.x * NWM);
+  const int rounds = (B + nmom * NWM - 1) / (nmom * NWM);
   for (int r = 0; r < rounds; ++r) {
-    const int clip = (r * gridDim.x + blockIdx.x) * NWM + wave;
+    const int clip = (r * nmom + blockIdx.x) * NWM + wave;
     const bool live = clip < B;
     const float* gx = in + (size_t)(live ? clip : 0) * CI * TV;
 #pragma unroll
@@ -413,17 +423,23 @@
 
 template <int T, int V>
 static int launch_first_moments_tv(const float* in, const float* Aw, const float* Tw, const float* in_slope, float* partials, int B,
-                                   int Ci, float* Zout, int max_rows, hipStream_t st, int* rows_out) {
+                                   int Ci, float* Zout, int max_rows, hipStream_t st, int* rows_out, const FtabArgs* ride) {
   int grid = (B + fl::NWM - 1) / fl::NWM;
   if (grid > 512) grid = 512;
   if (grid > max_rows) grid = max_rows;
   *rows_out = grid;
+  FtabArgs tabs{};
+  if (ride && ride->n > 0) {
+    if (T != 12 || V != 17 || ride->n > 4) return fail(COSKAD_ERR_SHAPE, "first_moments: operand tables ride at T=12, V=17, 1..4 layers");
+    tabs = *ride;
+  }
+  const int nmom = grid, ntab = tabs.n * fl::kFtabBlocks;
   const size_t lds = ((size_t)T * V * V + (size_t)V * T * T + 2 * fl::NWM * (size_t)Ci * T * V) * sizeof(float);
 #define LAUNCH_FM(CI)                                                                                                   \
   do {                                                                                                                  \
     auto k = fl::k_first_moments<T, V, CI>;                                                                             \
     if (lds > 64 * 1024) (void)hipFuncSetAttribute((const void*)k, hipFuncAttributeMaxDynamicSharedMemorySize, (int)lds); \
-    hipLaunchKernelGGL(k, dim3(grid), dim3(64 * fl::NWM), lds, st, in, Aw, Tw, in_slope, partials, B, Zout);                    \
+    hipLaunchKernelGGL(k, dim3(nmom + ntab), dim3(64 * fl::NWM), lds, st, in, Aw, Tw, in_slope, partials, B, Zout, nmom, tabs); \
   } while (0)
   {
     ProbeScope probe(KID_FWD_MOMENTS, Ci, 0, st);
@@ -437,8 +453,8 @@
 }
 
 int launch_first_moments(const float* in, const float* Aw, const float* Tw, const float* in_slope, float* partials, int B, int Ci,
-                         int T, int V, float* Zout, int max_rows, hipStream_t st, int* rows_out) {
-#define CALL(T_, V_) return launch_first_moments_tv<T_, V_>(in, Aw, Tw, in_slope, partials, B, Ci, Zout, max_rows, st, rows_out)
+                         int T, int V, float* Zout, int max_rows, hipStream_t st, int* rows_out, const FtabArgs* ride) {
+#define CALL(T_, V_) return launch_first_moments_tv<T_, V_>(in, Aw, Tw, in_slope, partials, B, Ci, Zout, max_rows, st, rows_out, ride)
   COSKAD_DISPATCH_TV(T, V, CALL);
 #undef CALL
 }
diff --git a/coskad_amd/csrc/ftab_ops.h b/coskad_amd/csrc/ftab_ops.h
--- /dev/null
+++ b/coskad_amd/csrc/ftab_ops.h
@@ -0,0 +1,37 @@
+#pragma once
+#include "common.h"
+
+namespace coskad {
+
+struct FtabArgs {
+  const float* A[4];
+  const float* Tm[4];
+  float* tab[4];
+  int n;
+};
+
+template <int T, int V>
+constexpr int ftab_elems() { return (V * 64 + T * 3 * 64) * 4; }
+
+template <int T, int V>
+__device__ __forceinline__ void ftab_store(const FtabArgs& args, int layer, int e) {
+  constexpr int TEMP_F4 = V * 64;
+  const float* __restrict__ Aw = args.A[layer];
+  const float* __restrict__ Tw = args.Tm[layer];
+  if (e >= ftab_elems<T, V>()) return;
+  float val = 0.f;
+  if (e < TEMP_F4 * 4) {
+    const int v = e / 256, l = (e >> 2) & 63, s = e & 3, j = l & 15, q = l >> 4;
+    if (s < 3 && j < T) val = Tw[v * T * T + (4 * s + q) * T + j];
+  } else {
+    const int r = e - TEMP_F4 * 4;
+    const int t = r / (3 * 256), c = (r / 256) % 3, l = (r >> 2) & 63, k = 4 * c + (r & 3), j = l & 15, q = l >> 4;
+    if (k < 10) {
+      const int s = k < 5 ? k : k - 5, w = 4 * s + q;
+      if (w < V) val = Aw[t * V * V + w * V + (k < 5 ? j : 16)];
+    }
+  }
+  args.tab[layer][e] = val;
+}
+
+}
diff --git a/coskad_amd/csrc/fused_apply_next.hip b/coskad_amd/csrc/fused_apply_next.hip
--- a/coskad_amd/csrc/fused_apply_next.hip
+++ b/coskad_amd/csrc/fused_apply_next.hip
@@ -1,5 +1,6 @@
 #include "fused_ops.h"
 #include "layer_launch.h"
+#include "ftab_ops.h"
 
 #ifndef FN_ABLATE
 #define FN_ABLATE 0
@@ -10,30 +11,9 @@
 
 using namespace ff;
 
-struct FtabArgs {
-  const float* A[4];
-  const float* Tm[4];
-  float* tab[4];
-};
+static_assert(ftab_elems<T, V>() == LAYER_F4 * 4, "the table layout of ftab_ops.h is this file's");
 __global__ void k_build_ftab(FtabArgs args) {
-  const int layer = blockIdx.y;
-  const float* __restrict__ Aw = args.A[layer];
-  const float* __restrict__ Tw = args.Tm[layer];
-  const int e = blockIdx.x * blockDim.x + threadIdx.x;
-  if (e >= LAYER_F4 * 4) return;
-  float val = 0.f;
-  if (e < TEMP_F4 * 4) {
-    const int v = e / 256, l = (e >> 2) & 63, s = e & 3, j = l & 15, q = l >> 4;
-    if (s < 3 && j < T) val = Tw[v * T * T + (4 * s + q) * T + j];
-  } else {
-    const int r = e - TEMP_F4 * 4;
-    const int t = r / (3 * 256), c = (r / 256) % 3, l = (r >> 2) & 63, k = 4 * c + (r & 3), j = l & 15, q = l >> 4;
-    if (k < 10) {
-      const int s = k < 5 ? k : k - 5, w = 4 * s + q;
-      if (w < V) val = Aw[t * V * V + w * V + (k < 5 ? j : 16)];
-    }
-  }
-  args.tab[layer][e] = val;
+  ftab_store<T, V>(args, blockIdx.y, blockIdx.x * blockDim.x + threadIdx.x);
 }
 
 template <int CT, int OTP>
@@ -342,7 +322,8 @@
 
 int launch_build_ftab(const float* const* A, const float* const* Tm, float* const* tab, int n, hipStream_t st) {
   if (n < 1 || n > 4) return fail(COSKAD_ERR_ARG, "build_ftab: 1..4 layers per launch, got %d", n);
-  fn::FtabArgs args{};
+  FtabArgs args{};
+  args.n = n;
   for (int i = 0; i < n; ++i) {
     if (!A[i] || !Tm[i] || !tab[i]) return fail(COSKAD_ERR_ARG, "build_ftab: null pointer (layer %d)", i);
     args.A[i] = A[i]; args.Tm[i] = Tm[i]; args.tab[i] = tab[i];
diff --git a/coskad_amd/csrc/heads.hip b/coskad_amd/csrc/heads.hip
--- a/coskad_amd/csrc/heads.hip
+++ b/coskad_amd/csrc/heads.hip
@@ -2,28 +2,6 @@
 #include "heads_common.h"
 
 namespace coskad {
-
-struct Vec {
-  float v[LMAX];
-};
-
-__device__ __forceinline__ Vec load_vec(const float* p, int L) {
-  Vec r;
-#pragma unroll
-  for (int j = 0; j < LMAX; ++j) r.v[j] = j < L ? p[j] : 0.f;
-  return r;
-}
-__device__ __forceinline__ void store_vec(float* p, const Vec& a, int L) {
-#pragma unroll
-  for (int j = 0; j < LMAX; ++j)
-    if (j < L) p[j] = a.v[j];
-}
-__device__ __forceinline__ float dot(const Vec& a, const Vec& b) {
-  float s = 0.f;
-#pragma unroll
-  for (int j = 0; j < LMAX; ++j) s = fmaf(a.v[j], b.v[j], s);
-  return s;
-}
 
 struct Embed {
   Vec p;
@@ -107,33 +85,6 @@
   return gu;
 }
 
-constexpr int kHeadSlots = LMAX + 3;
-
-constexpr int kHeadSingleRows = kFlatBlock;
-__host__ __device__ inline int head_blocks(int B) { return B <= kHeadSingleRows ? 1 : ceil_div(B, kFlatBlock); }
-
-__device__ __forceinline__ void block_partials(const float (&vals)[kHeadSlots], float* partials, float scale0, float* stats,
-                                               float* acc) {
-  __shared__ float sh[kFlatBlock / 64][kHeadSlots];
-  const int lane = threadIdx.x & 63, wave = threadIdx.x >> 6;
-#pragma unroll
-  for (int k = 0; k < kHeadSlots; ++k) {
-    const float s = wave_sum(vals[k]);
-    if (lane == 0) sh[wave][k] = s;
-  }
-  __syncthreads();
-  if (threadIdx.x < kHeadSlots) {
-    float s = 0.f;
-    for (int w = 0; w < kFlatBlock / 64; ++w) s += sh[w][threadIdx.x];
-    if (gridDim.x == 1) {
-      if (stats) stats[threadIdx.x] = threadIdx.x == 0 ? s * scale0 : s;
-      if (acc) acc[threadIdx.x] += s;
-    } else {
-      partials[blockIdx.x * kHeadSlots + threadIdx.x] = s;
-    }
-  }
-}
-
 __global__ __launch_bounds__(kFlatBlock) void k_mse_head(const float* __restrict__ z,
                                                     const float* __restrict__ cvec,
                                                     float* __restrict__ dz, float* __restrict__ score,
@@ -148,21 +99,11 @@
   for (int n = blockIdx.x * kFlatBlock + threadIdx.x; n < B; n += gridDim.x * kFlatBlock) {
     const Vec u = load_vec(z + (size_t)n * L, L);
     Vec g;
-    float sq = 0.f;
-#pragma unroll
-    for (int j = 0; j < LMAX; ++j) {
-      const float d = j < L ? u.v[j] - c.v[j] : 0.f;
-      sq = fmaf(d, d, sq);
-      g.v[j] = 2.f * d * gscale;
-      vals[1 + j] += u.v[j];
-    }
-    vals[0] += sq;
-    vals[LMAX + 1] += 1.f;
-    vals[LMAX + 2] += sqrtf(dot(u, u));
+    const float sq = mse_head_row(u, c, L, gscale, vals, g);
     if (dz) store_vec(dz + (size_t)n * L, g, L);
     if (score) score[n] = sq / (float)L;
   }
-  block_partials(vals, partials, scale0, stats, acc);
+  block_partials(vals, partials, scale0, stats, acc, blockIdx.x, gridDim.x);
 }
 
 __global__ __launch_bounds__(kFlatBlock) void k_mahalanobis_head(const float* __restrict__ z,
@@ -210,7 +151,7 @@
       store_vec(dz + (size_t)n * L, g, L);
     }
   }
-  block_partials(vals, partials, scale0, stats, acc);
+  block_partials(vals, partials, scale0, stats, acc, blockIdx.x, gridDim.x);
 }
 
 __global__ __launch_bounds__(LMAX * LMAX) void k_gram(const float* __restrict__ z, float* __restrict__ gram, int B,
@@ -266,18 +207,13 @@
       }
     }
   }
-  block_partials(vals, partials, scale0, stats, acc);
+  block_partials(vals, partials, scale0, stats, acc, blockIdx.x, gridDim.x);
 }
 
 __global__ __launch_bounds__(64) void k_head_finalize(const float* __restrict__ partials, int P,
                                                        float scale0, float* __restrict__ stats,
                                                        float* __restrict__ acc) {
-  const int k = threadIdx.x;
-  if (k >= kHeadSlots) return;
-  double s = 0.0;
-  for (int p = 0; p < P; ++p) s += (double)partials[p * kHeadSlots + k];
-  if (stats) stats[k] = (float)(k == 0 ? s * (double)scale0 : s);
-  if (acc) acc[k] += (float)s;
+  head_finalize_slot(partials, P, scale0, stats, acc, threadIdx.x);
 }
 
 __global__ __launch_bounds__(kFlatBlock) void k_poincare_dist(const float* __restrict__ zh,
diff --git a/coskad_amd/csrc/heads_common.h b/coskad_amd/csrc/heads_common.h
--- a/coskad_amd/csrc/heads_common.h
+++ b/coskad_amd/csrc/heads_common.h
@@ -14,6 +14,79 @@
 __host__ __device__ inline int head_lp(int L) { return L > LMAX ? L : LMAX; }
 __host__ __device__ inline int head_slots_for(int L) { return head_lp(L) + 3; }
 
+struct Vec {
+  float v[LMAX];
+};
+
+__device__ __forceinline__ Vec load_vec(const float* p, int L) {
+  Vec r;
+#pragma unroll
+  for (int j = 0; j < LMAX; ++j) r.v[j] = j < L ? p[j] : 0.f;
+  return r;
+}
+__device__ __forceinline__ void store_vec(float* p, const Vec& a, int L) {
+#pragma unroll
+  for (int j = 0; j < LMAX; ++j)
+    if (j < L) p[j] = a.v[j];
+}
+__device__ __forceinline__ float dot(const Vec& a, const Vec& b) {
+  float s = 0.f;
+#pragma unroll
+  for (int j = 0; j < LMAX; ++j) s = fmaf(a.v[j], b.v[j], s);
+  return s;
+}
+
+constexpr int kHeadSlots = LMAX + 3;
+
+constexpr int kHeadSingleRows = kFlatBlock;
+__host__ __device__ inline int head_blocks(int B) { return B <= kHeadSingleRows ? 1 : ceil_div(B, kFlatBlock); }
+
+__device__ __forceinline__ void block_partials(const float (&vals)[kHeadSlots], float* partials, float scale0, float* stats,
+                                               float* acc, int bid, int nb) {
+  __shared__ float sh[kFlatBlock / 64][kHeadSlots];
+  const int lane = threadIdx.x & 63, wave = threadIdx.x >> 6;
+#pragma unroll
+  for (int k = 0; k < kHeadSlots; ++k) {
+    const float s = wave_sum(vals[k]);
+    if (lane == 0) sh[wave][k] = s;
+  }
+  __syncthreads();
+  if (threadIdx.x < kHeadSlots) {
+    float s = 0.f;
+    for (int w = 0; w < kFlatBlock / 64; ++w) s += sh[w][threadIdx.x];
+    if (nb == 1) {
+      if (stats) stats[threadIdx.x] = threadIdx.x == 0 ? s * scale0 : s;
+      if (acc) acc[threadIdx.x] += s;
+    } else {
+      partials[bid * kHeadSlots + threadIdx.x] = s;
+    }
+  }
+}
+
+__device__ __forceinline__ float mse_head_row(const Vec& u, const Vec& c, int L, float gscale, float (&vals)[kHeadSlots], Vec& g) {
+  float sq = 0.f;
+#pragma unroll
+  for (int j = 0; j < LMAX; ++j) {
+    const float d = j < L ? u.v[j] - c.v[j] : 0.f;
+    sq = fmaf(d, d, sq);
+    g.v[j] = 2.f * d * gscale;
+    vals[1 + j] += u.v[j];
+  }
+  vals[0] += sq;
+  vals[LMAX + 1] += 1.f;
+  vals[LMAX + 2] += sqrtf(dot(u, u));
+  return sq;
+}
+
+__device__ __forceinline__ void head_finalize_slot(const float* __restrict__ partials, int P, float scale0,
+                                                   float* __restrict__ stats, float* __restrict__ acc, int k) {
+  if (k >= kHeadSlots) return;
+  double s = 0.0;
+  for (int p = 0; p < P; ++p) s += (double)partials[p * kHeadSlots + k];
+  if (stats) stats[k] = (float)(k == 0 ? s * (double)scale0 : s);
+  if (acc) acc[k] += (float)s;
+}
+
 size_t wide_head_ws_floats(int B, int L);
 int wide_mse_head(const float* z, const float* c, float* dz, float* score, float* stats, float* acc, float upstream, float* ws,
                   int B, int L, hipStream_t stream);
diff --git a/coskad_amd/csrc/layer_launch.h b/coskad_amd/csrc/layer_launch.h
--- a/coskad_amd/csrc/layer_launch.h
+++ b/coskad_amd/csrc/layer_launch.h
@@ -102,7 +102,9 @@
   float* bias = nullptr;
   float* stat = nullptr;
 };
+struct FtabArgs;
 struct LayerStatsArgs {
+  const FtabArgs* ftab = nullptr;
   const float* in = nullptr;
   const float* A = nullptr;
   const float* Tm = nullptr;
@@ -169,7 +171,7 @@
                      const float* in_slope, float* partials, int B, int Ci, int Co, int T, int V, int max_rows, hipStream_t st,
                      int* rows_out);
 int launch_first_moments(const float* in, const float* Aw, const float* Tw, const float* in_slope, float* partials, int B, int Ci,
-                         int T, int V, float* Zout, int max_rows, hipStream_t st, int* rows_out);
+                         int T, int V, float* Zout, int max_rows, hipStream_t st, int* rows_out, const FtabArgs* ride = nullptr);
 int launch_first_apply(const float* Z, const float* in, float* out, const float* wfold, const float* bias, const float* in_slope,
                        int B, int Ci, int Co, int TVr, hipStream_t st);
 bool fwd_moments_bpc_ok(int T_, int V_, int Ci);
@@ -202,9 +204,17 @@
 int launch_layer_apply_next_bpc(const float* Z, const float* in, float* out, const float* wfold, const float* bias,
                                 const float* in_slope, const float* out_slope, const float* ftab, float* Znext, float* partials,
                                 int B, int Ci, int Co, hipStream_t st);
+struct HeadFin {
+  const float* part = nullptr;
+  int P = 0;
+  float scale0 = 0.f;
+  float* stats = nullptr;
+  float* acc = nullptr;
+  unsigned block = 0;
+};
 int launch_btlnk_reduce(const float* partials, int P, size_t E, float* out, const float* dz, int B, int L, float* db,
                         const float* dap, int nda, float* dslope, int accumulate, hipStream_t stream, const float* rows,
-                        int RP, int RE, double* rsum);
+                        int RP, int RE, double* rsum, HeadFin fin = HeadFin());
 size_t wide_btlnk_fwd_ws_bytes(int B, int K, int L);
 size_t wide_btlnk_bwd_ws_bytes(int B, int K, int L);
 int wide_btlnk_fwd(const float* U, const float* W, const float* bias, const float* slope, float* z, void* ws, int B, int K, int L,
diff --git a/coskad_amd/csrc/stsgcn_train.hip b/coskad_amd/csrc/stsgcn_train.hip
--- a/coskad_amd/csrc/stsgcn_train.hip
+++ b/coskad_amd/csrc/stsgcn_train.hip
@@ -1,5 +1,6 @@
 #include "mfma_ops.h"
 #include "layer_launch.h"
+#include "ftab_ops.h"
 
 namespace coskad {
 
@@ -294,8 +295,10 @@
   double* red = reinterpret_cast<double*>(reinterpret_cast<char*>(a.ws) + round_up((int)(kMaxGrid * (size_t)E * sizeof(float)), 256));
   const int need_x = a.sums ? 1 : (a.p.Wr != nullptr);
   int rows = grid;
+  if (a.ftab && !(a.Zout && Ci <= 4 && T == 12 && V == 17))
+    return fail(COSKAD_ERR_SHAPE, "train_stats: operand tables ride only in the first layer's moments launch (stored Z, C_in <= 4, T=12, V=17)");
   if (a.Zout && Ci <= 4 && TV % 4 == 0) {
-    int rc1 = launch_first_moments(a.in, a.A, a.Tm, a.in_slope, partials, B, Ci, T, V, a.Zout, kMaxGrid, st, &rows);
+    int rc1 = launch_first_moments(a.in, a.A, a.Tm, a.in_slope, partials, B, Ci, T, V, a.Zout, kMaxGrid, st, &rows, a.ftab);
     if (rc1) return rc1;
   } else if (a.Zout && fwd_moments_bpc_ok(T, V, Ci)) {
     ProbeScope probe(KID_FWD_MOMENTS, Ci, Co, st);
@@ -357,7 +360,7 @@
     if ((size_t)a.Zout & 15) return fail(COSKAD_ERR_ARG, "%s: `Z` must be 16-byte aligned at window lengths 8, 16 and 24", who);
     if (full ? (coskad_layer_train_window_ok(T, V, a.Ci, a.Co) || coskad_layer_train_window_narrow_ok(T, V, a.Ci, a.Co))
              : window_moments_ok(T, V, a.Ci))
-      return launch_train_stats_window(a, T, V);
+      return a.ftab ? fail(COSKAD_ERR_SHAPE, "%s: no operand tables ride at window lengths 8, 16 and 24", who) : launch_train_stats_window(a, T, V);
   }
 #define CALL(T_, V_) return launch_train_stats<T_, V_>(a)
   COSKAD_DISPATCH_TV(T, V, CALL);
@@ -392,6 +395,34 @@
   return dispatch_train_stats("layer_train_stats", a, T, V, true);
 }
 
+int coskad_layer_train_stats_z_ftab_f32(const float* in, const float* A, const float* Tm, const float* in_slope,
+                                        const float* Wt, const float* bt, const float* gamma_t,
+                                        const float* beta_t, float* rmean_t, float* rvar_t, long long* nbt_t,
+                                        const float* Wr, const float* br, const float* gamma_r,
+                                        const float* beta_r, float* rmean_r, float* rvar_r, long long* nbt_r,
+                                        float momentum, float* wfold, float* bias, float* stat, void* ws,
+                                        size_t ws_bytes, int B, int Ci, int Co, int T, int V,
+                                        hipStream_t stream, float* Z, const float* const* tab_A, const float* const* tab_Tm,
+                                        float* const* tab, int ntab) {
+  if (!tab_A || !tab_Tm || !tab || !Z) return fail(COSKAD_ERR_ARG, "layer_train_stats_ftab: null pointer");
+  if (ntab < 1 || ntab > 4) return fail(COSKAD_ERR_ARG, "layer_train_stats_ftab: 1..4 operand tables, got %d", ntab);
+  FtabArgs tabs{};
+  tabs.n = ntab;
+  for (int i = 0; i < ntab; ++i) {
+    if (!tab_A[i] || !tab_Tm[i] || !tab[i]) return fail(COSKAD_ERR_ARG, "layer_train_stats_ftab: null pointer (table %d)", i);
+    tabs.A[i] = tab_A[i]; tabs.Tm[i] = tab_Tm[i]; tabs.tab[i] = tab[i];
+  }
+  const LayerStatsArgs a{
+      .ftab = &tabs, .in = in, .A = A, .Tm = Tm, .in_slope = in_slope,
+      .p = {.Wt = Wt, .bt = bt, .gt = gamma_t, .bet = beta_t, .rm_t = rmean_t, .rv_t = rvar_t, .nbt_t = nbt_t, .Wr = Wr, .br = br,
+            .gr = gamma_r, .ber = beta_r, .rm_r = rmean_r, .rv_r = rvar_r, .nbt_r = nbt_r, .momentum = momentum},
+      .out = {.wfold = wfold, .bias = bias, .stat = stat},
+      .Zout = Z, .ws = ws, .ws_bytes = ws_bytes, .B = B, .Ci = Ci, .Co = Co, .stream = stream};
+  if (int rc = check_layer_stats("layer_train_stats_ftab", a, kNeedInput | kNeedFold | kNeedWs)) return rc;
+  if (B <= 0 || Ci <= 0 || Co <= 0) return fail(COSKAD_ERR_ARG, "layer_train_stats_ftab: B=%d Ci=%d Co=%d", B, Ci, Co);
+  return dispatch_train_stats("layer_train_stats_ftab", a, T, V, true);
+}
+
 int coskad_layer_train_stats_f32(const float* in, const float* A, const float* Tm, const float* in_slope,
                                  const float* Wt, const float* bt, const float* gamma_t,
                                  const float* beta_t, float* rmean_t, float* rvar_t, long long* nbt_t,
diff --git a/coskad_amd/engine.py b/coskad_amd/engine.py
--- a/coskad_amd/engine.py
+++ b/coskad_amd/engine.py
@@ -133,16 +133,19 @@
     h, slope = x, in_slope
     n = len(layers)
     fuse = [False] * n
-    ftab = None
+    ftab = ftab_ride = None
     if all(batch_stats) and STORE_Z and FUSE_NEXT:
         for i in range(n - 1):
             fuse[i] = layers[i + 1].Ci == layers[i].Co and ops.layer_apply_next_ok(layers[i].Ci, layers[i].Co, T, V)
         nxt = [i + 1 for i in range(n - 1) if fuse[i]]
         if nxt:
             ftab = torch.empty(n, ops.ftab_floats(), device=x.device, dtype=torch.float32)
-            for k in range(0, len(nxt), 4):
-                grp = nxt[k:k + 4]
-                ops.build_ftabs([layers[i].A for i in grp], [layers[i].T for i in grp], [ftab[i] for i in grp])
+            if FTAB_RIDES and len(nxt) <= 4 and pending0 is None and sync_count is None and layers[0].Ci <= 4 and fuse[0]:
+                ftab_ride = ([layers[i].A for i in nxt], [layers[i].T for i in nxt], [ftab[i] for i in nxt])
+            else:
+                for k in range(0, len(nxt), 4):
+                    grp = nxt[k:k + 4]
+                    ops.build_ftabs([layers[i].A for i in grp], [layers[i].T for i in grp], [ftab[i] for i in grp])
     fuse_flat = [False] * n
     if all(batch_stats) and STORE_Z and FUSE_NEXT and sync is None:
         for i in range(n - 1):
@@ -181,7 +184,8 @@
                     Z = torch.empty_like(h)
                 wfold, bias, stat = ops.layer_train_stats(
                     h, L.A, L.T, slope, L.w2(L.Wt), L.bt, L.gt, L.bet, L.rm_t, L.rv_t, L.nbt_t,
-                    L.w2(L.Wr), L.br, L.gr, L.ber, L.rm_r, L.rv_r, L.nbt_r, buf, momentum=L.step_momentum(), Z=Z)
+                    L.w2(L.Wr), L.br, L.gr, L.ber, L.rm_r, L.rv_r, L.nbt_r, buf, momentum=L.step_momentum(), Z=Z,
+                    ftabs=ftab_ride if i == 0 else None)
         else:
             wfold, bias = eval_fold(L)
             stat = None
@@ -220,6 +224,8 @@
 CHAIN_SKIP = frozenset()
 FUSE_TOP = True
 FUSE_NEXT = True
+FTAB_RIDES = False
+HEAD_RIDES = True
 
 
 class SideStream:
@@ -240,18 +246,40 @@
             self.ws = torch.empty(ws_bytes, device=device, dtype=torch.uint8)
 
 
+def _chain_top(ctx: Optional[ChainCtx], layers: List[LayerTensors], U: Tensor, L: int):
+    i = len(layers) - 1 if layers else -1
+    Z = ctx.zs[i] if (ctx is not None and ctx.zs and i >= 0) else None
+    if (FUSE_TOP and Z is not None and U.dim() == 4 and layers[i].Wr is not None and L <= 16
+            and ops.btlnk_bwd_chain_ok(U.numel() // U.shape[0], U.shape[2] * U.shape[3], layers[i].Ci)):
+        return i, Z
+    return None
+
+
 def btlnk_backward(ctx: Optional[ChainCtx], layers: List[LayerTensors], U: Tensor, W: Tensor, dz: Tensor, slope: Optional[Tensor],
                    dW: Tensor, db: Optional[Tensor], dslope: Optional[Tensor], ws: Workspace):
     B = U.shape[0]
     K, L = U.numel() // B, W.shape[0]
-    i = len(layers) - 1 if layers else -1
-    Z = ctx.zs[i] if (ctx is not None and ctx.zs and i >= 0) else None
-    if (FUSE_TOP and Z is not None and U.dim() == 4 and layers[i].Wr is not None and L <= 16
-            and ops.btlnk_bwd_chain_ok(K, U.shape[2] * U.shape[3], layers[i].Ci)):
+    top = _chain_top(ctx, layers, U, L)
+    if top is not None:
+        i, Z = top
         in_slope = layers[i - 1].slope if i > 0 else ctx.in_slope
         return ops.btlnk_bwd_chain(U, W, dz, slope, dW, db, dslope, ws, ctx.inputs[i], Z, in_slope)
     buf = ws.get(ops.btlnk_bwd_ws_bytes(B, K, L), U.device)
     return ops.btlnk_bwd(U, W, dz, slope, dW, db, dslope, buf), None
+
+
+def head_rides(ctx: Optional[ChainCtx], layers: List[LayerTensors], U: Tensor, L: int) -> bool:
+    return bool(HEAD_RIDES and _chain_top(ctx, layers, U, L) is not None and (U.numel() // U.shape[0]) % 16 == 0)
+
+
+def btlnk_head_backward(ctx: ChainCtx, layers: List[LayerTensors], U: Tensor, W: Tensor, part: Tensor, bias: Optional[Tensor],
+                        c: Tensor, slope: Optional[Tensor], dW: Tensor, db: Optional[Tensor], dslope: Optional[Tensor], ws: Workspace,
+                        acc: Optional[Tensor] = None):
+    i, Z = _chain_top(ctx, layers, U, W.shape[0])
+    in_slope = layers[i - 1].slope if i > 0 else ctx.in_slope
+    _, _, _, stats, dU, top_stats = ops.btlnk_bwd_chain_head(U, W, part, bias, c, slope, dW, db, dslope, ws, ctx.inputs[i], Z, in_slope,
+                                                             acc=acc)
+    return stats, dU, top_stats
 
 
 def chain_backward(ctx: ChainCtx, layers: List[LayerTensors], dU: Tensor, ws: Workspace,
diff --git a/coskad_amd/ops.py b/coskad_amd/ops.py
--- a/coskad_amd/ops.py
+++ b/coskad_amd/ops.py
@@ -180,7 +180,7 @@
 
 
 def layer_train_stats(x, A, Tm, in_slope, Wt, bt, gt, bet, rm_t, rv_t, nbt_t,
-                      Wr, br, gr, ber, rm_r, rv_r, nbt_r, ws, momentum: float = 0.1, Z: Optional[Tensor] = None):
+                      Wr, br, gr, ber, rm_r, rv_r, nbt_r, ws, momentum: float = 0.1, Z: Optional[Tensor] = None, ftabs=None):
     B, Ci, T, V = x.shape
     Co = Wt.shape[0]
     _chk(x, "x"); _chk(A, "A", (T, V, V)); _chk(Tm, "T", (V, T, T))
@@ -202,7 +202,13 @@
     args = (x, A, Tm, in_slope, Wt, bt, gt, bet, rm_t, rv_t, nbt_t, Wr, br, gr, ber, rm_r, rv_r, nbt_r, momentum, wfold, bias, stat, ws,
             ws.numel() * ws.element_size(), B, Ci, Co, T, V, _stream())
     note_raw_write()
-    if Z is None:
+    if ftabs is not None:
+        _chk(Z, "Z", tuple(x.shape))
+        tab_A, tab_T, tabs, ntab = _ftab_pointers(*ftabs, T, V)
+        call("coskad_layer_train_stats_z_ftab_f32", x, A, Tm, in_slope, Wt, bt, gt, bet, rm_t, rv_t, nbt_t, Wr, br, gr, ber, rm_r, rv_r,
+             nbt_r, momentum, wfold, bias, stat, ws, ws.numel() * ws.element_size(), B, Ci, Co, T, V, _stream(), Z, tab_A, tab_T, tabs,
+             ntab)
+    elif Z is None:
         call("coskad_layer_train_stats_f32", *args)
     else:
         call("coskad_layer_train_stats_z_f32", *args, Z)
@@ -290,17 +296,21 @@
     return _lib.lib().coskad_ftab_floats()
 
 
-def build_ftabs(As, Ts, tabs) -> None:
+def _ftab_pointers(As, Ts, tabs, T, V):
     n = len(As)
     if not (1 <= n <= 4) or len(Ts) != n or len(tabs) != n:
         raise ValueError("build_ftabs: 1..4 layers, equal list lengths")
-    T, V = As[0].shape[0], As[0].shape[1]
     nf = ftab_floats()
     for A, Tm, tab in zip(As, Ts, tabs):
         _chk(A, "A", (T, V, V)); _chk(Tm, "T", (V, T, T)); _chk(tab, "tab", (nf,))
     arr = ctypes.c_void_p * n
-    call("coskad_build_ftab_f32", arr(*[t.data_ptr() for t in As]), arr(*[t.data_ptr() for t in Ts]),
-         arr(*[t.data_ptr() for t in tabs]), n, T, V, _stream())
+    return arr(*[t.data_ptr() for t in As]), arr(*[t.data_ptr() for t in Ts]), arr(*[t.data_ptr() for t in tabs]), n
+
+
+def build_ftabs(As, Ts, tabs) -> None:
+    T, V = (As[0].shape[0], As[0].shape[1]) if len(As) else (0, 0)
+    pa, pt, ptab, n = _ftab_pointers(As, Ts, tabs, T, V)
+    call("coskad_build_ftab_f32", pa, pt, ptab, n, T, V, _stream())
 
 
 def layer_apply_next(Z, x, wfold, bias, Co, in_slope, out_slope, ftab_next, partials, T, V, out=None, Z_next=None):
@@ -545,6 +555,49 @@
     return dU, (stats, rows.value)
 
 
+def btlnk_fwd_parts(U: Tensor, W: Tensor, slope: Optional[Tensor]) -> Tensor:
+    B = U.shape[0]
+    K = U.numel() // B
+    L = W.shape[0]
+    _chk(U, "U"); _chk(W, "W", (L, K)); _chk(slope, "slope", (1,), optional=True)
+    part = torch.empty(_lib.lib().coskad_btlnk_fwd_ks(), B, 16, device=U.device, dtype=torch.float32)
+    call("coskad_btlnk_fwd_parts_f32", U, W, slope, part, _bytes(part), B, K, L, _stream())
+    return part
+
+
+def btlnk_bwd_chain_head(U, W, part, bias, c, slope, dW, db, dslope, ws, below_in, below_Z, below_in_slope, acc=None, need_score=False,
+                         upstream=1.0, dU=None, accumulate=False):
+    B, Ch, T, V = U.shape
+    TV = T * V
+    K = Ch * TV
+    L = W.shape[0]
+    Ci = below_in.shape[1]
+    KS = part.shape[0]
+    S = head_slots(L)
+    _chk(U, "U"); _chk(W, "W", (L, K)); _chk(part, "part", (KS, B, 16)); _chk(bias, "bias", (L,), optional=True); _chk(c, "c", (L,))
+    _chk(dW, "dW", (L, K)); _chk(db, "db", (L,), optional=True); _chk(dslope, "dslope", (1,), optional=True)
+    _chk(slope, "slope", (1,), optional=True); _chk(acc, "acc", (S,), optional=True)
+    _chk(below_in, "below_in", (B, Ci, T, V)); _chk(below_Z, "below_Z", (B, Ci, T, V)); _chk(below_in_slope, "below_in_slope", (1,), optional=True)
+    if not btlnk_bwd_chain_ok(K, TV, Ci):
+        raise ValueError(f"btlnk_bwd_chain_head: shape K={K} TV={TV} Ci={Ci} not supported")
+    lib = _lib.lib()
+    need = lib.coskad_btlnk_bwd_chain_ws_bytes(B, K, L, TV)
+    buf = ws.get(need, U.device)
+    chain = torch.empty(lib.coskad_btlnk_bwd_chain_floats(B, TV, Ci), device=U.device, dtype=torch.float32)
+    if dU is None:
+        dU = torch.empty_like(U)
+    z = torch.empty(B, L, device=U.device, dtype=torch.float32)
+    dz = torch.empty_like(z)
+    score = torch.empty(B, device=U.device, dtype=torch.float32) if need_score else None
+    stats = torch.empty(S, device=U.device, dtype=torch.float32)
+    hws = head_ws(B, U.device, L)
+    rows = ctypes.c_int(0)
+    call("coskad_btlnk_bwd_chain_head_f32", U, W, part, KS, bias, c, upstream, z, dz, score, stats, acc, hws, slope, dU, dW, db, dslope,
+         buf, _bytes(buf), 1 if accumulate else 0, B, K, L, below_in, below_Z, below_in_slope, Ci, TV, chain, _bytes(chain),
+         ctypes.byref(rows), _stream())
+    return z, dz, score, stats, dU, (chain, rows.value)
+
+
 def _cuda_f32(t: Tensor, name: str) -> None:
     if not t.is_cuda:
         raise _lib.CoskadHipError(f"{name}: expected a CUDA (ROCm) tensor, got device {t.device}; no CPU fallback")
diff --git a/coskad_amd/trainer.py b/coskad_amd/trainer.py
--- a/coskad_amd/trainer.py
+++ b/coskad_amd/trainer.py
@@ -449,6 +449,14 @@
 
     def backward(self, W, dy, U, slope, ctx, top_layers, last_slope_grad):
         return engine.btlnk_backward(ctx, top_layers or [], U, W, dy, slope, self.gW, self.gb, last_slope_grad, self.ws)
+
+    def forward_parts(self, U: Tensor, slope):
+        W = self.lin.weight
+        return ops.btlnk_fwd_parts(U, W, slope), W
+
+    def head_backward(self, W, part, c, acc, U, slope, ctx, top_layers, last_slope_grad):
+        return engine.btlnk_head_backward(ctx, top_layers, U, W, part, self.lin.bias, c, slope, self.gW, self.gb, last_slope_grad,
+                                          self.ws, acc=acc)
 
 
 class _MLPProjector(_LinearProjector):
@@ -599,10 +607,16 @@
     def _body(self, x: Tensor) -> Tensor:
         U, slope, saved_stack = self.stack.forward(x, self.ws)
         ctx, top_layers = self.stack.top(saved_stack)
-        z, saved = self.projector.forward(U, slope)
-        stats, dz = self._head(z)
-        dU, top_stats = self.projector.backward(saved, dz, U, slope, ctx if self.side is None else None, top_layers,
-                                                self.stack.last_slope_grad)
+        if (type(self.projector) is _LinearProjector and self.head == 'euclidean' and self.side is None
+                and engine.head_rides(ctx, top_layers or [], U, self.model.latent_dim)):
+            part, saved = self.projector.forward_parts(U, slope)
+            stats, dU, top_stats = self.projector.head_backward(saved, part, self.model.c, self.center_acc, U, slope, ctx, top_layers,
+                                                                self.stack.last_slope_grad)
+        else:
+            z, saved = self.projector.forward(U, slope)
+            stats, dz = self._head(z)
+            dU, top_stats = self.projector.backward(saved, dz, U, slope, ctx if self.side is None else None, top_layers,
+                                                    self.stack.last_slope_grad)
         work = None
         if self.world > 1 and self.tail_off is not None:
             work = dist.all_reduce(self.fp.grad[self.tail_off:], group=self.pg, async_op=True)
diff --git a/include/coskad_hip.h b/include/coskad_hip.h
--- a/include/coskad_hip.h
+++ b/include/coskad_hip.h
@@ -85,6 +85,16 @@
 int coskad_layer_apply_next_rows(int B, int Ci, int Co);
 int coskad_build_ftab_f32(const float* const* A, const float* const* Tm, float* const* tab, int n, int T, int V,
                           hipStream_t stream);
+int coskad_layer_train_stats_z_ftab_f32(const float* in, const float* A, const float* Tm, const float* in_slope,
+                                        const float* Wt, const float* bt, const float* gamma_t,
+                                        const float* beta_t, float* rmean_t, float* rvar_t, long long* nbt_t,
+                                        const float* Wr, const float* br, const float* gamma_r,
+                                        const float* beta_r, float* rmean_r, float* rvar_r, long long* nbt_r,
+                                        float momentum, float* wfold, float* bias, float* stat, void* ws,
+                                        size_t ws_bytes, int B, int Ci, int Co, int T, int V,
+                                        hipStream_t stream, float* Z, const float* const* tab_A, const float* const* tab_Tm,
+                                        float* const* tab, int ntab);
+
 int coskad_layer_apply_next_f32(const float* Z, const float* in, float* out, const float* wfold, const float* bias,
                                 const float* in_slope, const float* out_slope, const float* ftab_next, float* Z_next,
                                 float* partials, size_t partials_bytes, int B, int Ci, int Co, int T, int V,
@@ -239,6 +249,16 @@
                                float* db, float* dslope, void* ws, size_t ws_bytes, int accumulate, int B, int K, int L,
                                const float* below_in, const float* below_Z, const float* below_in_slope, int below_Ci, int TV,
                                float* stats_out, size_t stats_out_bytes, int* stats_rows, hipStream_t stream);
+
+int coskad_btlnk_fwd_ks(void);
+int coskad_btlnk_fwd_parts_f32(const float* U, const float* W, const float* slope, float* part, size_t part_bytes, int B, int K,
+                               int L, hipStream_t stream);
+int coskad_btlnk_bwd_chain_head_f32(const float* U, const float* W, const float* part, int KS, const float* bias, const float* c,
+                                    float upstream, float* z, float* dz, float* score, float* stats, float* acc, float* head_ws,
+                                    const float* slope, float* dU, float* dW, float* db, float* dslope, void* ws, size_t ws_bytes,
+                                    int accumulate, int B, int K, int L, const float* below_in, const float* below_Z,
+                                    const float* below_in_slope, int below_Ci, int TV, float* stats_out, size_t stats_out_bytes,
+                                    int* stats_rows, hipStream_t stream);
 
 
 int coskad_gather_transform_f32(const float* xy, const long long* index, const float* mats, float* out, int B, int N,
```

Result: faster. 3.075 million clips/s, median of 6 (+2.4%).
